# mazouziwissem/improving_yolov8_CBAM_SwinBlock

Measured on AMD Instinct MI355X. Metric: images/sec fwd+bwd YOLOv8s-CBAM-Swin bs=32 640x640, higher is better.
Workload: dtype bf16; 1 GPU; yolov8s.yaml (nc=1) forward + v8 loss + backward + clip + SGD-nesterov + EMA step, bs=32/GPU 640x640 (CBAM + 2x SwinBlock + SPPF5 + SPPF7); global_batch=32, imgsz=640, parallelism=dp1

## Files before the change

### improving_yolov8_cbam_swinblock_amd/_lib.py

```python
import ctypes
import os
import subprocess
import threading
from pathlib import Path

import torch

PKG_DIR = Path(__file__).resolve().parent
CSRC_DIR = PKG_DIR / "csrc"
LIB_PATH = Path(os.environ["YMI_LIB"]).resolve() if os.environ.get("YMI_LIB") else PKG_DIR / "libyolo_mi355.so"

YMI_F32, YMI_BF16 = 0, 1
ACT_NONE, ACT_SILU, ACT_GELU = 0, 1, 2

_c_i64 = ctypes.c_int64
_c_i32 = ctypes.c_int32
_c_f32 = ctypes.c_float
_vp = ctypes.c_void_p
_sz = ctypes.c_size_t


class YmiTensor(ctypes.Structure):
    _fields_ = [
        ("data", _vp),
        ("n", _c_i64),
        ("h", _c_i64),
        ("w", _c_i64),
        ("c", _c_i64),
        ("ld", _c_i64),
        ("dtype", _c_i32),
        ("_pad", _c_i32),
    ]


_TP = ctypes.POINTER(YmiTensor)

_SIGNATURES = {
    "ymi_version": (_c_i32, []),
    "ymi_last_error": (ctypes.c_char_p, []),
    "ymi_set_option": (_c_i32, [ctypes.c_char_p, _c_i64]),
    "ymi_get_option": (_c_i64, [ctypes.c_char_p]),
    "ymi_profile_begin": (_c_i32, [_c_i64]),
    "ymi_profile_end": (_c_i32, [ctypes.POINTER(ctypes.c_double), ctypes.POINTER(ctypes.c_double), ctypes.POINTER(_c_i64)]),
    "ymi_profile_end_ex": (_c_i32, [ctypes.POINTER(ctypes.c_double), ctypes.POINTER(ctypes.c_double), ctypes.POINTER(_c_i64),
                                    ctypes.POINTER(ctypes.c_double), ctypes.POINTER(ctypes.c_double)]),
    "ymi_nchw_to_nhwc": (_c_i32, [_vp, _c_i64, _c_i64, _c_i64, _c_i64, _TP, _vp]),
    "ymi_nhwc_to_nchw": (_c_i32, [_TP, _vp, _vp]),
    "ymi_copy": (_c_i32, [_TP, _TP, _vp]),
    "ymi_upsample2x": (_c_i32, [_TP, _TP, _vp]),
    "ymi_upsample2x_bwd": (_c_i32, [_TP, _TP, _vp]),
    "ymi_upsample2x_bwd_acc": (_c_i32, [_TP, _TP, _vp]),
    "ymi_add_inplace": (_c_i32, [_TP, _TP, _vp]),
    "ymi_pack_conv_weight_fwd": (_c_i32, [_vp, _c_i64, _c_i64, _c_i64, _c_i64, _c_i64, _c_i32, _vp, _vp]),
    "ymi_pack_conv_weight_dgrad": (_c_i32, [_vp, _c_i64, _c_i64, _c_i64, _c_i64, _c_i64, _c_i32, _vp, _vp]),
    "ymi_pack_conv_weight_dgrad_ex": (_c_i32, [_vp, _c_i64, _c_i64, _c_i64, _c_i64, _c_i64, _c_i64, _c_i32, _vp, _vp]),
    "ymi_conv_dgrad_pack_elems": (_c_i64, [_c_i64, _c_i64, _c_i64, _c_i64, _c_i64]),
    "ymi_pack_conv_weights_batch": (_c_i32, [_vp, _vp, _c_i32, _c_i32, _c_i32, _vp]),
    "ymi_pack_matrix": (_c_i32, [_vp, _c_i64, _c_i64, _c_i32, _c_i32, _vp, _vp]),
    "ymi_conv2d_fwd": (_c_i32, [_TP, _vp, _c_i64, _c_i64, _c_i64, _c_i64, _vp, _vp, _c_i32, _TP, _TP, _vp, ctypes.POINTER(_c_i64), _vp]),
    "ymi_conv2d_stat_blocks": (_c_i64, [_c_i64, _c_i64]),
    "ymi_conv2d_fwd_multi": (_c_i32, [_vp, _c_i32, _vp]),
    "ymi_conv2d_bwd_data_multi": (_c_i32, [_vp, _c_i32, _vp]),
    "ymi_bn_finalize_pair": (_c_i32, [_vp, _c_i64, _c_i64, _c_i64, _c_i64, _vp, _vp, _vp, _vp, _vp, _vp, _vp, _vp, _c_f32, _c_f32, _vp, _vp, _vp, _vp, _vp]),
    "ymi_bn_finalize": (_c_i32, [_vp, _c_i64, _c_i64, _c_i64, _vp, _vp, _vp, _vp, _c_f32, _c_f32, _vp, _vp, _vp, _vp, _vp]),
    "ymi_scale_shift_act": (_c_i32, [_TP, _vp, _vp, _c_i32, _TP, _TP, _vp]),
    "ymi_conv2d_bn_silu_fwd": (
        _c_i32,
        [_TP, _vp, _c_i64, _c_i64, _c_i64, _c_i64, _vp, _vp, _vp, _vp, _c_f32, _c_f32, _c_i32, _TP, _TP, _TP, _vp, _vp, _vp, _sz, _vp],
    ),
    "ymi_conv2d_bn_silu_fwd_acc_ok": (_c_i32, [_TP, _TP, _TP]),
    "ymi_conv2d_bn_silu_fwd_acc": (_c_i32, [_TP, _vp, _c_i64, _c_i64, _c_i64, _c_i64, _vp, _vp, _vp, _vp, _c_f32, _c_f32, _c_i32, _TP, _TP, _TP, _vp, _vp, _vp, _vp]),
    "ymi_bn_act_bwd": (_c_i32, [_TP, _TP, _vp, _vp, _vp, _vp, _c_i32, _TP, _vp, _vp, _vp, _sz, _vp]),
    "ymi_conv2d_bn_silu_fwd_pair": (
        _c_i32,
        [_TP, _vp, _c_i64, _c_i64, _c_i64, _c_i64, _c_i64, _vp, _vp, _vp, _vp, _vp, _vp, _vp, _vp, _c_f32, _c_f32, _c_i32, _TP, _TP, _vp, _vp, _vp, _sz, _vp],
    ),
    "ymi_first_conv_stat_blocks": (_c_i64, [_c_i64, _c_i64, _c_i64]),
    "ymi_first_conv_bn_act_fwd": (_c_i32, [_vp, _c_i64, _c_i64, _c_i64, _c_i64, _vp, _c_i64, _vp, _vp, _vp, _vp, _c_f32, _c_f32, _c_i32, _TP, _TP, _vp, _vp,
                                           _vp, _sz, _vp]),
    "ymi_first_conv_bwd_workspace": (_c_i64, [_c_i64, _c_i64, _c_i64, _c_i64]),
    "ymi_first_conv_bn_act_bwd": (_c_i32, [_TP, _vp, _c_i64, _c_i64, _vp, _vp, _vp, _vp, _c_i32, _TP, _vp, _vp, _vp, _vp, _sz, _vp, _vp]),
    "ymi_bn_act_bwd_pair": (_c_i32, [_TP, _TP, _vp, _vp, _vp, _vp, _c_i64, _vp, _vp, _c_i32, _TP, _vp, _vp, _vp, _sz, _vp]),
    "ymi_conv2d_bwd_data": (_c_i32, [_TP, _vp, _c_i64, _c_i64, _c_i64, _c_i64, _TP, _vp]),
    "ymi_conv2d_bwd_data_add": (_c_i32, [_TP, _vp, _c_i64, _c_i64, _c_i64, _c_i64, _TP, _TP, _TP, _vp]),
    "ymi_dwconv2d_fwd": (_c_i32, [_TP, _vp, _c_i64, _c_i64, _vp, _vp, _c_i32, _TP, _TP, _vp, ctypes.POINTER(_c_i64), _vp]),
    "ymi_dwconv2d_stat_blocks": (_c_i64, [_c_i64, _c_i64, _c_i64, _c_i64]),
    "ymi_dwconv2d_bn_act_fwd": (_c_i32, [_TP, _vp, _c_i64, _c_i64, _vp, _vp, _vp, _vp, _c_f32, _c_f32, _c_i32, _TP, _TP, _TP, _vp, _vp, _vp, _sz, _vp]),
    "ymi_dwconv2d_bwd_data": (_c_i32, [_TP, _vp, _c_i64, _c_i64, _TP, _TP, _vp]),
    "ymi_dwconv2d_bwd_weight": (_c_i32, [_TP, _TP, _c_i64, _c_i64, _vp, _vp, _sz, _vp]),
    "ymi_dwconv2d_bwd_weight_workspace": (_sz, [_c_i64, _c_i64, _c_i64, _c_i64, _c_i64]),
    "ymi_swin_mlp_fwd": (_c_i32, [_TP, _vp, _vp, _c_i64, _vp, _vp, _TP, _TP, _TP, _TP, _vp]),
    "ymi_swin_ln_mlp_supported": (_c_i32, [_c_i64, _c_i64, _c_i32]),
    "ymi_swin_ln_mlp_pack_elems": (_c_i64, [_c_i64, _c_i64]),
    "ymi_swin_ln_mlp_pre_elems": (_c_i64, [_c_i64, _c_i64]),
    "ymi_swin_ln_mlp_pack": (_c_i32, [_vp, _vp, _c_i64, _c_i64, _vp, _vp]),
    "ymi_swin_ln_mlp_fwd": (_c_i32, [_TP, _vp, _vp, _c_f32, _vp, _vp, _vp, _c_i64, _TP, _vp, _vp, _vp, _TP, _vp]),
    "ymi_swin_ln_mlp_bwd_data": (_c_i32, [_TP, _vp, _vp, _c_i64, _TP, _TP, _TP, _vp]),
    "ymi_swin_mlp_bwd_data": (_c_i32, [_TP, _vp, _TP, _TP, _vp, _TP, _TP, _TP, _vp]),
    "ymi_conv2d_bwd_weight": (_c_i32, [_TP, _TP, _c_i64, _c_i64, _c_i64, _c_i64, _c_i64, _vp, _vp, _vp, _sz, _vp]),
    "ymi_conv2d_bwd_weight_workspace": (_sz, [_c_i64, _c_i64, _c_i64, _c_i64, _c_i64]),
    "ymi_conv2d_bwd_weight_deferred": (_c_i32, [_TP, _TP, _c_i64, _c_i64, _c_i64, _c_i64, _c_i64, _vp, _vp, _vp, _sz, _vp, _vp]),
    "ymi_wgrad_hold": (_c_i32, [_c_i32]),
    "ymi_wgrad_reduce_batch": (_c_i32, [_vp, _c_i32, _vp, _vp]),
    "ymi_sppf_pool3_fwd": (_c_i32, [_TP, _c_i64, _TP, _TP, _TP, _vp]),
    "ymi_sppf_pool3_bwd_workspace": (_c_i64, [_c_i64, _c_i64, _c_i64, _c_i64, _c_i32]),
    "ymi_sppf_pool3_bwd": (_c_i32, [_TP, _TP, _TP, _c_i64, _TP, _TP, _TP, _TP, _TP, _vp, _c_i64, _vp]),
    "ymi_cbam_fwd": (_c_i32, [_TP, _vp, _vp, _c_i64, _vp, _c_i64, _TP, _vp, _vp, _vp, _vp, _vp, _vp, _vp]),
    "ymi_cbam_bwd": (_c_i32, [_TP, _TP, _vp, _vp, _c_i64, _vp, _c_i64, _vp, _vp, _vp, _vp, _vp, _vp, _TP, _vp, _vp, _vp, _vp, _sz, _vp]),
    "ymi_cbam_bwd_workspace": (_sz, [_c_i64, _c_i64, _c_i64, _c_i64, _c_i64]),
    "ymi_window_partition_index": (_c_i32, [_c_i64, _c_i64, _c_i64, _c_i64, _vp, _vp]),
    "ymi_window_partition": (_c_i32, [_TP, _c_i64, _TP, _vp]),
    "ymi_window_reverse": (_c_i32, [_TP, _c_i64, _TP, _vp]),
    "ymi_layernorm_fwd": (_c_i32, [_TP, _c_i64, _vp, _vp, _c_f32, _TP, _vp, _vp, _vp]),
    "ymi_layernorm_bwd": (_c_i32, [_TP, _c_i64, _TP, _vp, _vp, _vp, _TP, _c_i32, _vp, _vp, _vp, _sz, _vp]),
    "ymi_layernorm_bwd_add": (_c_i32, [_TP, _c_i64, _TP, _vp, _vp, _vp, _TP, _TP, _vp, _vp, _vp, _sz, _vp]),
    "ymi_window_attention_fwd": (_c_i32, [_TP, _c_i64, _c_i64, _TP, _vp, _vp]),
    "ymi_window_attention_bwd": (_c_i32, [_TP, _TP, _TP, _vp, _c_i64, _c_i64, _TP, _vp]),
    "ymi_psa_attention_fwd": (_c_i32, [_TP, _c_i64, _c_i64, _c_i64, _TP, _TP, _vp, _vp]),
    "ymi_psa_attention_bwd": (_c_i32, [_TP, _TP, _TP, _vp, _TP, _c_i64, _c_i64, _c_i64, _TP, _vp]),
    "ymi_colsum":(_c_i32, [_TP, _vp, _vp, _sz, _vp]),
    "ymi_gelu_bwd": (_c_i32, [_TP, _TP, _TP, _vp]),
    "ymi_detect_targets": (_c_i32, [_vp, _vp, _vp, _c_i64, _c_i64, _c_i64, ctypes.c_float, ctypes.c_float, _vp, _vp]),
    "ymi_detect_loss_sizes": (_c_i32, [_c_i64, _c_i64, _c_i64, ctypes.POINTER(ctypes.c_size_t), ctypes.POINTER(ctypes.c_size_t)]),
    "ymi_detect_loss_fwd": (_c_i32, [_c_i32, _TP, _TP, ctypes.POINTER(ctypes.c_float), _vp, _c_i64, _c_i32, ctypes.c_float, ctypes.c_float,
                                     _vp, _vp, _vp, _sz, _vp, _sz, _vp]),
    "ymi_detect_loss_bwd": (_c_i32, [_c_i32, _TP, _TP, ctypes.POINTER(ctypes.c_float), _vp, _sz, _vp, _vp, _TP, _TP, _vp]),
    "ymi_detect_decode": (_c_i32, [_c_i32, _TP, _TP, ctypes.POINTER(ctypes.c_float), _vp, _vp]),
    "ymi_depth_to_space2": (_c_i32, [_TP, _TP, _vp]),
    "ymi_space_to_depth2": (_c_i32, [_TP, _TP, _vp]),
    "ymi_detect_loss_fwd_assign": (_c_i32, [_c_i32, _TP, _TP, ctypes.POINTER(ctypes.c_float), _vp, _c_i64, _c_i32, ctypes.c_float, ctypes.c_float,
                                            _vp, _vp, _vp, _sz, _vp, _sz, _vp, _vp]),
    "ymi_detect_decode_seg": (_c_i32, [_c_i32, _TP, _TP, _TP, ctypes.POINTER(ctypes.c_float), _vp, _vp]),
    "ymi_mask_loss_sizes": (_c_i32, [_c_i64, _c_i64, _c_i64, _c_i32, ctypes.POINTER(ctypes.c_size_t)]),
    "ymi_mask_loss_fwd": (_c_i32, [_c_i32, _TP, _TP, _vp, _c_i32, _c_i64, _c_i64, _vp, _vp, _c_i64, _c_i32, _c_f32, _c_f32, _vp, _vp, _vp, _vp, _sz, _vp]),
    "ymi_mask_loss_bwd": (_c_i32, [_c_i32, _TP, _TP, _vp, _c_i32, _c_i64, _c_i64, _c_i64, _c_i32, _vp, _sz, _vp, _vp, _TP, _TP, _vp]),
    "ymi_detect_nms_sizes": (_c_i32, [_c_i64, _c_i64, _c_i64, _c_i64, _c_i64, ctypes.POINTER(ctypes.c_size_t)]),
    "ymi_detect_nms": (_c_i32, [_vp, _c_i64, _c_i64, _c_i64, _c_f32, _c_f32, _c_i32, _c_i32, ctypes.POINTER(_c_i32), _c_i32, _c_i64, _c_i64, _c_f32,
                                _vp, _vp, _vp, _sz, _vp]),
    "ymi_detect_nms_seg": (_c_i32, [_vp, _c_i64, _c_i64, _c_i64, _c_i64, _c_f32, _c_f32, _c_i32, _c_i32, ctypes.POINTER(_c_i32), _c_i32, _c_i64, _c_i64,
                                    _c_f32, _vp, _vp, _vp, _vp, _sz, _vp]),
    "ymi_process_mask": (_c_i32, [_TP, _vp, _vp, _vp, _c_i64, _c_i64, _c_i64, _c_i32, _vp, _vp, _vp]),
    "ymi_mask_overlap": (_c_i32, [_vp, _vp, _vp, _c_i64, _c_i64, _TP, _c_i64, _c_i64, _vp, _c_i32, _c_i64, _c_i64, _c_i64, _vp, _vp, _vp, _vp]),
    "ymi_scale_image": (_c_i32, [_vp, _c_i32, _c_i64, _c_i64, _c_i64, _vp, _c_i64, _c_i64, _c_i64, _c_i64, _c_f32, _c_i32, _c_i32, _c_i32, _vp]),
    "ymi_tta_merge": (_c_i32, [_c_i32, ctypes.POINTER(_vp), ctypes.POINTER(_c_i64), ctypes.POINTER(_c_i64), ctypes.POINTER(_c_i64), ctypes.POINTER(_c_f32),
                               ctypes.POINTER(_c_i32), ctypes.POINTER(_c_i64), ctypes.POINTER(_c_i64), _c_i64, _c_i64, _vp, _vp]),
    "ymi_letterbox_batch": (_c_i32, [_vp, _c_i64, _vp, _c_i64, _c_i64, _c_i32, _c_i32, _c_i32, _vp]),
    "ymi_scale_boxes": (_c_i32, [_vp, _c_i64, _vp, _vp, _c_i64, _c_i64, _c_i64, _c_i32, _c_i32, _vp, _c_i64, _vp]),
    "ymi_augment_batch": (_c_i32, [_vp, _vp, _c_i64, _vp, _c_i64, _c_i32, _c_i32, _c_i32, _vp]),
    "ymi_augment_boxes": (_c_i32, [_vp, _c_i64, _vp, _c_i64, _c_f32, _vp, _vp, _vp, _vp, _vp, _vp, _vp]),
    "ymi_val_match": (_c_i32, [_vp, _vp, _c_i64, _c_i64, _vp, _vp, _vp, _c_i64, _c_f32, _c_f32, _vp, ctypes.POINTER(_c_f32), _c_i32, _c_i32, _vp, _vp, _c_i64,
                              _c_f32, _c_f32, _vp]),
    "ymi_val_match_masks": (_c_i32, [_vp, _vp, _c_i64, _c_i64, _vp, _vp, _c_i64, _vp, _vp, _vp, _c_i64, ctypes.POINTER(_c_f32), _c_i32, _c_i32, _vp, _vp]),
    "ymi_opt_chunk_elems": (_c_i64, []),
    "ymi_opt_grad_norm": (_c_i32, [_vp, _vp, _c_i32, _c_i32, _c_i64, ctypes.POINTER(_vp), _vp, _vp, _c_i64, _c_i64, _vp, _c_i32, _vp]),
    "ymi_opt_update": (_c_i32, [_vp, _vp, _c_i32, _c_i32, _c_i64, ctypes.POINTER(_vp), _vp, _vp, _c_i32, _vp]),
    "ymi_opt_grad_accumulate": (_c_i32, [_vp, _vp, _c_i32, _c_i32, _c_i64, ctypes.POINTER(_vp), _vp]),
}

OPT_MAX_GRADS = 448


class LetterboxImage(ctypes.Structure):
    _fields_ = [("src", _vp), ("h", _c_i32), ("w", _c_i32), ("hs", _c_i32), ("ws", _c_i32), ("top", _c_i32), ("left", _c_i32)]


AUGMENT_MAX_SRC = 4
VALMATCH_CHUNK, VALMATCH_MAX_LEVELS, VALMATCH_MAX_DET = 1024, 16, 2048


class AugmentSource(ctypes.Structure):
    _fields_ = [("src", _vp), ("h", _c_i32), ("w", _c_i32), ("x1a", _c_i32), ("y1a", _c_i32), ("x2a", _c_i32), ("y2a", _c_i32), ("x1b", _c_i32),
                ("y1b", _c_i32)]


class AugmentImage(ctypes.Structure):
    _fields_ = [("s", AugmentSource * AUGMENT_MAX_SRC), ("A", ctypes.c_double * 6), ("lut", _vp), ("n_src", _c_i32), ("canvas_h", _c_i32),
                ("canvas_w", _c_i32), ("flip_ud", _c_i32), ("flip_lr", _c_i32), ("_pad", _c_i32)]


class AugmentLabelImage(ctypes.Structure):
    _fields_ = [("src_w", _c_f32 * AUGMENT_MAX_SRC), ("src_h", _c_f32 * AUGMENT_MAX_SRC), ("ratio_w", _c_f32 * AUGMENT_MAX_SRC),
                ("ratio_h", _c_f32 * AUGMENT_MAX_SRC), ("padw", _c_f32 * AUGMENT_MAX_SRC), ("padh", _c_f32 * AUGMENT_MAX_SRC), ("M", _c_f32 * 6),
                ("scale", _c_f32), ("size_w", _c_f32), ("size_h", _c_f32), ("canvas", _c_f32), ("flip_ud", _c_i32), ("flip_lr", _c_i32),
                ("row_start", _c_i32), ("row_end", _c_i32)]


class ConvProblem(ctypes.Structure):
    _fields_ = [("x", _TP), ("w_packed", _vp), ("cout", _c_i64), ("kh", _c_i64), ("kw", _c_i64), ("stride", _c_i64), ("scale", _vp), ("bias", _vp),
                ("act", _c_i32), ("_pad", _c_i32), ("residual", _TP), ("y", _TP), ("stat_partials", _vp), ("stat_blocks", _c_i64), ("stat_stride", _c_i64),
                ("stat_offset", _c_i64)]


class DgradProblem(ctypes.Structure):
    _fields_ = [("dy", _TP), ("w_dgrad_packed", _vp), ("cin", _c_i64), ("k", _c_i64), ("add1", _TP), ("add2", _TP), ("dx", _TP)]


class WgradPending(ctypes.Structure):
    _fields_ = [("slab", _vp), ("dw", _vp), ("elems", _c_i64), ("splits", _c_i32), ("ng", _c_i32), ("cin", _c_i32), ("cout_real", _c_i32),
                ("cin_real", _c_i32), ("ntaps", _c_i32), ("lanes", _c_i32), ("first_block", _c_i32), ("blocks", _c_i32), ("slab_bf16", _c_i32),
                ("bias_slab", _vp), ("dbias", _vp)]


class OptEntry(ctypes.Structure):
    _fields_ = [("param", _vp), ("momentum", _vp), ("ema", _vp), ("numel", _c_i64), ("group", _c_i32), ("_pad", _c_i32), ("second", _vp), ("acc", _vp)]


class OptState(ctypes.Structure):
    _fields_ = [("clip", _c_f32), ("norm", _c_f32), ("ema_d", _c_f32), ("ema_1md", _c_f32), ("updates", _c_i64), ("steps", _c_i64), ("inv_bc1", _c_f32),
                ("bc2_sqrt", _c_f32), ("c0", _c_f32), ("c1", _c_f32), ("c2", _c_f32), ("c3", _c_f32), ("mu_product", ctypes.c_double)]


assert ctypes.sizeof(OptState) == 64

_lib = None
_lock = threading.Lock()


def build(verbose=False):
    jobs = str(min(8, os.cpu_count() or 1))
    proc = subprocess.run(["make", "-C", str(CSRC_DIR), "-j", jobs], capture_output=True, text=True)
    if proc.returncode != 0:
        raise RuntimeError(f"building libyolo_mi355.so failed:\n{proc.stdout[-4000:]}\n{proc.stderr[-4000:]}")
    if verbose:
        print(proc.stdout[-2000:])
    return LIB_PATH


def lib():
    global _lib
    if _lib is None:
        with _lock:
            if _lib is None:
                if not LIB_PATH.exists():
                    raise RuntimeError(
                        f"{LIB_PATH} is missing: build it with improving_yolov8_cbam_swinblock_amd._lib.build() "
                        "(make -C csrc); this package has no CPU or PyTorch fallback"
                    )
                handle = ctypes.CDLL(str(LIB_PATH))
                missing = []
                for name, (res, args) in _SIGNATURES.items():
                    try:
                        fn = getattr(handle, name)
                    except AttributeError:
                        missing.append(name)
                        continue
                    fn.restype = res
                    fn.argtypes = args
                if missing:
                    raise RuntimeError(f"{LIB_PATH} is stale, missing symbols {missing}: rebuild with make -C csrc")
                _lib = handle
    return _lib


def exported_symbols():
    return list(_SIGNATURES)


def check(rc, what=""):
    if rc != 0:
        msg = lib().ymi_last_error().decode("utf-8", "replace")
        raise RuntimeError(f"libyolo_mi355 {what} failed ({rc}): {msg}")


def ymi_dtype(dt):
    if dt == torch.float32:
        return YMI_F32
    if dt == torch.bfloat16:
        return YMI_BF16
    raise TypeError(f"libyolo_mi355 computes in float32 or bfloat16, got {dt}")


def chunk_elems(dt):
    return 8 if dt == torch.bfloat16 else 4


def is_nhwc(t):
    if t.dim() != 4:
        return False
    n, c, h, w = t.shape
    sn, sc, sh, sw = t.stride()
    if c > 1 and sc != 1:
        return False
    ld = sw if w > 1 else (sh if h > 1 else (sn if n > 1 else c))
    if w > 1 and h > 1 and sh != w * ld:
        return False
    if (h > 1 or w > 1) and n > 1 and sn != h * w * ld:
        return False
    return ld >= c


def as_ymi(t):
    if not t.is_cuda:
        raise RuntimeError("libyolo_mi355 kernels need tensors on the MI355X (cuda) device; there is no CPU path")
    if t.dim() == 4:
        if not is_nhwc(t):
            raise RuntimeError(f"expected NHWC memory for a logical NCHW tensor, got shape {tuple(t.shape)} strides {t.stride()}")
        n, c, h, w = t.shape
        sn, sc, sh, sw = t.stride()
        ld = sw if w > 1 else (sh if h > 1 else (sn if n > 1 else c))
        return YmiTensor(t.data_ptr(), n, h, w, c, ld, ymi_dtype(t.dtype), 0)
    if t.dim() == 2:
        rows, c = t.shape
        if c > 1 and t.stride(1) != 1:
            raise RuntimeError("token matrix must have unit channel stride")
        ld = t.stride(0) if rows > 1 else c
        return YmiTensor(t.data_ptr(), 1, 1, rows, c, ld, ymi_dtype(t.dtype), 0)
    raise RuntimeError(f"unsupported tensor rank {t.dim()}")


def stream_ptr():
    return ctypes.c_void_p(torch.cuda.current_stream().cuda_stream)


def ptr(t):
    return ctypes.c_void_p(t.data_ptr()) if t is not None else None


def empty_nhwc(n, c, h, w, dtype, device, ld=None):
    ld = c if ld is None else ld
    buf = torch.empty((n, h, w, ld), dtype=dtype, device=device)
    return buf.permute(0, 3, 1, 2)[:, :c]


_workspaces = {}


def workspace(nbytes, device, tag="default"):
    if os.environ.get("YMI_WS_NOCACHE") == "1":
        return torch.empty(max(int(nbytes), 256), dtype=torch.uint8, device=device)
    key = (device.index, torch.cuda.current_stream().cuda_stream, tag)
    buf = _workspaces.get(key)
    if buf is None or buf.numel() < nbytes:
        buf = torch.empty(max(int(nbytes), 1 << 20), dtype=torch.uint8, device=device)
        _workspaces[key] = buf
    return buf


def live_workspaces(device):
    return tuple(buf for (idx, _, _), buf in _workspaces.items() if idx == device.index)


def set_option(name, value):
    check(lib().ymi_set_option(name.encode(), int(value)), "set_option")


def get_option(name):
    v = lib().ymi_get_option(name.encode())
    if v < 0:
        raise RuntimeError(f"unknown option {name!r}")
    return int(v)
```

### improving_yolov8_cbam_swinblock_amd/csrc/common.h

```cpp
#pragma once
#include <hip/hip_runtime.h>
#include <stdint.h>
#include <stdio.h>

#include <type_traits>

#include "../../include/ymi.h"

typedef __bf16 bf16_t;
typedef __attribute__((ext_vector_type(8))) __bf16 bf16x8;
typedef __attribute__((ext_vector_type(4))) __bf16 bf16x4;
typedef __attribute__((ext_vector_type(4))) float f32x4;
typedef __attribute__((ext_vector_type(2))) float f32x2;
typedef __attribute__((ext_vector_type(4))) uint32_t u32x4;
typedef __attribute__((ext_vector_type(2))) uint32_t u32x2;

typedef const __attribute__((address_space(1))) void* gptr_t;
typedef __attribute__((address_space(3))) void* lptr_t;

#define YMI_WAVE 64

void ymi_set_error(const char* fmt, ...);
#define YMI_CHECK_ARG(cond, ...)          \
    do {                                  \
// ... 4 lines not shown
    } while (0)
#define YMI_CHECK_LAUNCH(what)                                                   \
    do {                                                                         \
        hipError_t e_ = hipGetLastError();                                       \
        if (e_ != hipSuccess) {                                                  \
            ymi_set_error("%s: launch failed: %s", what, hipGetErrorString(e_)); \
            return YMI_ELAUNCH;                                                  \
        }                                                                        \
    } while (0)

static inline bool ymi_tensor_ok(const ymi_tensor* t) {
    return t && t->data && t->n > 0 && t->h > 0 && t->w > 0 && t->c > 0 && t->ld >= t->c && (t->dtype == YMI_F32 || t->dtype == YMI_BF16);
}
static inline int64_t ymi_pixels(const ymi_tensor* t) { return t->n * t->h * t->w; }
static inline int ymi_stat_fixed_point_shift(int64_t count) {
    int lg = 0;
    while (((int64_t)1 << lg) < count) ++lg;
    const int sh = 37 - lg;
    return sh < 8 ? 8 : sh > 40 ? 40 : sh;
}
constexpr int BN_STAGE_ROWS = 64;
static inline size_t ymi_esize(int dtype) { return dtype == YMI_BF16 ? 2 : 4; }
static inline bool vec4_ok(const ymi_tensor* t) {
    return t->c % 4 == 0 && t->ld % 4 == 0 && ((uintptr_t)t->data % (4 * ymi_esize(t->dtype))) == 0;
}
static inline bool ymi_same_shape(const ymi_tensor* a, const ymi_tensor* b) {
    return a->n == b->n && a->h == b->h && a->w == b->w && a->c == b->c;
}
enum YmiOpt {
    OPT_EW_PPT,
    OPT_EW_CAP,
    OPT_RED_CAP,
    OPT_XCD_SHIFT,
    OPT_ATTN_TILED,
    OPT_WGRAD_BLOCKS,
    OPT_WGRAD_BLOCKS128,
    OPT_IGEMM_TILE_BM,
    OPT_IGEMM_TILE_BN,
    OPT_BN_TAIL,
    OPT_WGRAD_PATCH,
    OPT_COUNT
};
int ymi_opt(int id);
static inline int ew_ppt() { return ymi_opt(OPT_EW_PPT); }
static inline int ew_cap() { return ymi_opt(OPT_EW_CAP); }
static inline int64_t ew_capped(int64_t gb) {
    if (gb > ew_cap()) gb = ew_cap();
    return (gb + 7) / 8 * 8;
}
static inline int64_t ew_blocks(int64_t P, int rows) {
    int64_t gb = (P + (int64_t)rows * ew_ppt() - 1) / ((int64_t)rows * ew_ppt());
    if (gb < 1024) gb = (P + rows - 1) / rows < 1024 ? (P + rows - 1) / rows : 1024;
    return ew_capped(gb);
}
template <typename T> struct TypeTag {
    typedef T type;
};
template <int ACT> using ActTag = std::integral_constant<int, ACT>;
template <typename F> static inline void dispatch_dtype(int dtype, F&& f) {
    if (dtype == YMI_BF16) f(TypeTag<bf16_t>{});
    else f(TypeTag<float>{});
}
template <typename F> static inline void dispatch_dtype_act(int dtype, int act, F&& f) {
    dispatch_dtype(dtype, [&](auto t) {
        if (act == YMI_ACT_SILU) f(t, ActTag<YMI_ACT_SILU>{});
        else if (act == YMI_ACT_GELU) f(t, ActTag<YMI_ACT_GELU>{});
        else f(t, ActTag<YMI_ACT_NONE>{});
    });
}
const void* ymi_zero_page();

template <typename T> struct ElemTraits;
template <> struct ElemTraits<float> {
    static constexpr int CH = 4;
    static constexpr int DT = YMI_F32;
};
template <> struct ElemTraits<bf16_t> {
    static constexpr int CH = 8;
    static constexpr int DT = YMI_BF16;
};

__device__ __forceinline__ float to_f32(float v) { return v; }
__device__ __forceinline__ float to_f32(bf16_t v) { return (float)v; }
template <typename T> __device__ __forceinline__ T from_f32(float v);
template <> __device__ __forceinline__ float from_f32<float>(float v) { return v; }
template <> __device__ __forceinline__ bf16_t from_f32<bf16_t>(float v) { return (bf16_t)v; }

template <typename T, int G> struct Pack;
template <> struct Pack<float, 4> {
    static __device__ __forceinline__ void load(const float* p, float (&v)[4]) {
        f32x4 t = *reinterpret_cast<const f32x4*>(p);
        v[0] = t[0]; v[1] = t[1]; v[2] = t[2]; v[3] = t[3];
    }
    static __device__ __forceinline__ void store(float* p, const float (&v)[4]) {
        f32x4 t = {v[0], v[1], v[2], v[3]};
        *reinterpret_cast<f32x4*>(p) = t;
    }
};
template <> struct Pack<bf16_t, 4> {
    static __device__ __forceinline__ void load(const bf16_t* p, float (&v)[4]) {
        bf16x4 t = *reinterpret_cast<const bf16x4*>(p);
        v[0] = (float)t[0]; v[1] = (float)t[1]; v[2] = (float)t[2]; v[3] = (float)t[3];
    }
    static __device__ __forceinline__ void store(bf16_t* p, const float (&v)[4]) {
        bf16x4 t = {(bf16_t)v[0], (bf16_t)v[1], (bf16_t)v[2], (bf16_t)v[3]};
        *reinterpret_cast<bf16x4*>(p) = t;
    }
};
template <> struct Pack<bf16_t, 8> {
    static __device__ __forceinline__ void load(const bf16_t* p, float (&v)[8]) {
        bf16x8 t = *reinterpret_cast<const bf16x8*>(p);
#pragma unroll
        for (int i = 0; i < 8; ++i) v[i] = (float)t[i];
    }
    static __device__ __forceinline__ void store(bf16_t* p, const float (&v)[8]) {
        bf16x8 t;
#pragma unroll
        for (int i = 0; i < 8; ++i) t[i] = (bf16_t)v[i];
        *reinterpret_cast<bf16x8*>(p) = t;
    }
};

template <typename T> struct Raw4;
template <> struct Raw4<bf16_t> {
    typedef bf16x4 type;
    static __device__ __forceinline__ void to_f32(const bf16x4& r, float (&v)[4]) {
#pragma unroll
        for (int i = 0; i < 4; ++i) v[i] = (float)r[i];
    }
};
template <> struct Raw4<float> {
    typedef f32x4 type;
    static __device__ __forceinline__ void to_f32(const f32x4& r, float (&v)[4]) {
#pragma unroll
        for (int i = 0; i < 4; ++i) v[i] = r[i];
    }
};

__host__ __device__ __forceinline__ int64_t ymi_xcd_span(int64_t P) { return (((P + 63) >> 6) + 7) >> 3 << 6; }
struct XcdRange {
    int64_t lo, hi;
    int bi, nbx;
};
int64_t ymi_xcd_span_arg(int64_t P);
__device__ __forceinline__ XcdRange xcd_range(int64_t P, int64_t span_arg) {
    const int id = blockIdx.x, x = ((id & 7) + (int)(span_arg >> 56)) & 7;
    const int64_t span = span_arg & ((1ll << 56) - 1);
    XcdRange r;
    r.lo = x * span;
    r.hi = r.lo + span < P ? r.lo + span : P;
    if (r.lo > P) r.lo = P;
    r.bi = id >> 3;
    r.nbx = gridDim.x >> 3;
    return r;
}

__device__ __forceinline__ int xcd_unit(int flat, int total) { return (total & 7) ? flat : (flat & 7) * (total >> 3) + (flat >> 3); }
__device__ __forceinline__ int flat_block_id() { return blockIdx.x + gridDim.x * (blockIdx.y + gridDim.y * blockIdx.z); }

template <int U, typename T, typename F>
__device__ __forceinline__ void pixel_walk(const T* ap, int64_t lda, const T* bp, int64_t ldb, bool two, int coff, int64_t p, int64_t step, int64_t end, F&& use) {
    typedef typename Raw4<T>::type R4;
    R4 ra[U], rb[U];
    bool have = p + (U - 1) * step < end;
    if (have) {
#pragma unroll
        for (int u = 0; u < U; ++u) {
            ra[u] = *reinterpret_cast<const R4*>(ap + (p + u * step) * lda + coff);
            if (two) rb[u] = *reinterpret_cast<const R4*>(bp + (p + u * step) * ldb + coff);
        }
    }
    while (have) {
        float va[U][4], vb[U][4] = {};
#pragma unroll
        for (int u = 0; u < U; ++u) {
            Raw4<T>::to_f32(ra[u], va[u]);
            if (two) Raw4<T>::to_f32(rb[u], vb[u]);
        }
        const int64_t pc = p;
        p += U * step;
        have = p + (U - 1) * step < end;
        if (have) {
#pragma unroll
            for (int u = 0; u < U; ++u) {
                ra[u] = *reinterpret_cast<const R4*>(ap + (p + u * step) * lda + coff);
                if (two) rb[u] = *reinterpret_cast<const R4*>(bp + (p + u * step) * ldb + coff);
            }
        }
#pragma unroll
        for (int u = 0; u < U; ++u) use(va[u], vb[u], pc + u * step);
    }
    for (; p < end; p += step) {
        float va[4], vb[4] = {0.f, 0.f, 0.f, 0.f};
        Pack<T, 4>::load(ap + p * lda + coff, va);
        if (two) Pack<T, 4>::load(bp + p * ldb + coff, vb);
        use(va, vb, p);
    }
}

__device__ __forceinline__ float fast_exp(float x) { return __builtin_amdgcn_exp2f(x * 1.44269504088896340736f); }
__device__ __forceinline__ float sigmoidf_(float x) { return __builtin_amdgcn_rcpf(1.0f + fast_exp(-x)); }
__device__ __forceinline__ float silu_f(float x) { return x * sigmoidf_(x); }
__device__ __forceinline__ float silu_grad_f(float x) {
    float s = sigmoidf_(x);
    return s * (1.0f + x * (1.0f - s));
}
__device__ __forceinline__ float erf_as(float z, float* e2 = nullptr) {
    const float az = fabsf(z);
    const float t = __builtin_amdgcn_rcpf(1.0f + 0.3275911f * az);
    const float e = fast_exp(-az * az);
    float p = 1.061405429f;
    p = p * t - 1.453152027f;
    p = p * t + 1.421413741f;
    p = p * t - 0.284496736f;
    p = p * t + 0.254829592f;
    if (e2) *e2 = e;
    return copysignf(1.0f - p * t * e, z);
}
__device__ __forceinline__ float gelu_f(float x) { return 0.5f * x * (1.0f + erf_as(x * 0.70710678118654752440f)); }
__device__ __forceinline__ float gelu_grad_f(float x) {
    const float c = 0.39894228040143267794f;
    float e;
    const float er = erf_as(x * 0.70710678118654752440f, &e);
    return 0.5f * (1.0f + er) + x * c * e;
}
template <int ACT> __device__ __forceinline__ float apply_act(float x) {
    if (ACT == YMI_ACT_SILU) return silu_f(x);
    if (ACT == YMI_ACT_GELU) return gelu_f(x);
    return x;
}
__device__ __forceinline__ float apply_act_rt(float x, int act) {
    return act == YMI_ACT_SILU ? silu_f(x) : act == YMI_ACT_GELU ? gelu_f(x) : x;
}
template <int ACT> __device__ __forceinline__ float act_grad(float x) {
    if (ACT == YMI_ACT_SILU) return silu_grad_f(x);
    if (ACT == YMI_ACT_GELU) return gelu_grad_f(x);
    return 1.0f;
}
__device__ __forceinline__ float act_grad_rt(float x, int act) {
    return act == YMI_ACT_SILU ? silu_grad_f(x) : act == YMI_ACT_GELU ? gelu_grad_f(x) : 1.0f;
}

__device__ __forceinline__ float unit_of_byte(uint32_t u) {
    const float f = (float)u, rc = 1.0f / 255.0f;
    const float q = f * rc;
    const float r = __builtin_fmaf(-q, 255.0f, f);
    return __builtin_fmaf(r, rc, q);
}

struct Tap {
    int i0, i1;
    float l0, l1;
};
__device__ __forceinline__ Tap tap_of(int dst, float scale, int in) {
    float s = ((float)dst + 0.5f) * scale - 0.5f;
    s = s < 0.0f ? 0.0f : s;
    Tap t;
    t.i0 = (int)s;
    t.i0 = t.i0 > in - 1 ? in - 1 : t.i0;
    t.i1 = t.i0 + (t.i0 < in - 1 ? 1 : 0);
    t.l1 = s - (float)t.i0;
    t.l0 = 1.0f - t.l1;
    return t;
}

__device__ __forceinline__ void st_wt(float* p, float v) { __hip_atomic_store(p, v, __ATOMIC_RELAXED, __HIP_MEMORY_SCOPE_AGENT); }
__device__ __forceinline__ void st_wt2(float* p, float a, float b) {
    const uint64_t v = (uint64_t)__builtin_bit_cast(uint32_t, a) | ((uint64_t)__builtin_bit_cast(uint32_t, b) << 32);
    __hip_atomic_store(reinterpret_cast<uint64_t*>(p), v, __ATOMIC_RELAXED, __HIP_MEMORY_SCOPE_AGENT);
}
__device__ __forceinline__ void st_wt(double* p, double v) { __hip_atomic_store(p, v, __ATOMIC_RELAXED, __HIP_MEMORY_SCOPE_AGENT); }
__device__ __forceinline__ float ld_wt(const float* p) { return __hip_atomic_load(p, __ATOMIC_RELAXED, __HIP_MEMORY_SCOPE_AGENT); }
__device__ __forceinline__ double ld_wt(const double* p) { return __hip_atomic_load(p, __ATOMIC_RELAXED, __HIP_MEMORY_SCOPE_AGENT); }
__device__ __forceinline__ void ld_wt2(const float* p, float& a, float& b) {
    const uint64_t v = __hip_atomic_load(reinterpret_cast<const uint64_t*>(p), __ATOMIC_RELAXED, __HIP_MEMORY_SCOPE_AGENT);
    a = __builtin_bit_cast(float, (uint32_t)v);
    b = __builtin_bit_cast(float, (uint32_t)(v >> 32));
}
__device__ __forceinline__ bool ticket_is_last(unsigned* counter, unsigned last, int* flag) {
    asm volatile("s_waitcnt vmcnt(0)" ::: "memory");
    __syncthreads();
    if (threadIdx.x == 0) {
        const unsigned t = __hip_atomic_fetch_add(counter, 1u, __ATOMIC_RELAXED, __HIP_MEMORY_SCOPE_AGENT);
        if (t == last) __hip_atomic_store(counter, 0u, __ATOMIC_RELAXED, __HIP_MEMORY_SCOPE_AGENT);
        *flag = t == last;
    }
    __syncthreads();
    return *flag != 0;
}
struct GammaBeta2 {
    const float* gamma;
    const float* beta;
    int split;
};
struct BnCoefArgs {
    const float* gamma;
    const float* beta;
    const float* mean;
    const float* inv;
    float inv_count;
    float* coef;
    GammaBeta2 g2;
};
struct BnFinal {
    const float* part;
    int blocks, C;
    float* out0;
    float* out1;
    BnCoefArgs bn;
};
__device__ __forceinline__ void bn_affine_of(const float* gamma, const float* beta, const GammaBeta2& g2, int c, float& ga, float& be) {
    const bool second = g2.split > 0 && c >= g2.split;
    const float* gp = second ? g2.gamma : gamma;
    const float* bp = second ? g2.beta : beta;
    const int pc = second ? c - g2.split : c;
    ga = gp ? gp[pc] : 1.0f;
    be = bp ? bp[pc] : 0.0f;
}
struct BnChan {
    float ga, be, inv, mean;
};
__device__ __forceinline__ void bn_chan_fetch(const BnCoefArgs& bn, int c, BnChan& p) {
    bn_affine_of(bn.gamma, bn.beta, bn.g2, c, p.ga, p.be);
    p.inv = bn.inv[c];
    p.mean = bn.mean[c];
}
__device__ __forceinline__ void bn_coef_write(const BnCoefArgs& bn, int C, int c, const BnChan& p, float s0, float s1) {
    const float ga = p.ga, be = p.be;
    const float p0 = p.inv, p1 = -p.mean * p0;
    const float k1 = s0 * bn.inv_count, k2 = s1 * bn.inv_count;
    bn.coef[0 * C + c] = p0 * ga;
    bn.coef[1 * C + c] = p1 * ga + be;
    bn.coef[2 * C + c] = ga * p0;
    bn.coef[3 * C + c] = ga * p0 * p0 * k2;
    bn.coef[4 * C + c] = ga * p0 * (k1 + p1 * k2);
}
struct BnStat {
    double mean, var;
    float inv;
};
__device__ __forceinline__ BnStat bn_stat_of(double sum, double sumsq, double count, float eps) {
    BnStat s;
    s.mean = sum / count;
    s.var = sumsq / count - s.mean * s.mean;
    if (s.var < 0.0) s.var = 0.0;
    s.inv = (float)(1.0 / sqrt(s.var + (double)eps));
    return s;
}
constexpr int BN_FINAL_RED = 2 * 32 * 33;
template <int NT, bool PREFETCH = true> __device__ __forceinline__ void bn_final_block(const BnFinal& f, int w, double* red) {
    static_assert(NT == 1024 || NT == 256, "32 channels x 32 or 8 thread rows");
    constexpr int SPT = 1024 / NT;
    const int cl = threadIdx.x & 31, grp = threadIdx.x >> 5;
    const int c = w * 32 + cl, C = f.C;
    BnChan p{1.0f, 0.0f, 0.f, 0.f};
    if (PREFETCH && grp == 0 && c < C && f.bn.coef) bn_chan_fetch(f.bn, c, p);
    int es = 0;
#pragma unroll
    do {
        const int slice = grp * SPT + es;
        double s0 = 0.0, s1 = 0.0;
        if (c < C) {
            float a0 = 0.f, a1 = 0.f, b0 = 0.f, b1 = 0.f, c0 = 0.f, c1 = 0.f, d0 = 0.f, d1 = 0.f;
            int b = slice;
            for (; b + 96 < f.blocks; b += 128) {
                a0 += f.part[((int64_t)b * 2 + 0) * C + c];
                a1 += f.part[((int64_t)b * 2 + 1) * C + c];
                b0 += f.part[((int64_t)(b + 32) * 2 + 0) * C + c];
                b1 += f.part[((int64_t)(b + 32) * 2 + 1) * C + c];
                c0 += f.part[((int64_t)(b + 64) * 2 + 0) * C + c];
                c1 += f.part[((int64_t)(b + 64) * 2 + 1) * C + c];
                d0 += f.part[((int64_t)(b + 96) * 2 + 0) * C + c];
                d1 += f.part[((int64_t)(b + 96) * 2 + 1) * C + c];
            }
            for (; b < f.blocks; b += 32) {
                a0 += f.part[((int64_t)b * 2 + 0) * C + c];
                a1 += f.part[((int64_t)b * 2 + 1) * C + c];
            }
            s0 = ((double)a0 + (double)b0) + ((double)c0 + (double)d0);
            s1 = ((double)a1 + (double)b1) + ((double)c1 + (double)d1);
        }
        red[(0 * 32 + slice) * 33 + cl] = s0;
        red[(1 * 32 + slice) * 33 + cl] = s1;
    } while (++es < SPT);
    __syncthreads();
    if (grp == 0 && c < C) {
        double a0 = 0.0, a1 = 0.0;
#pragma unroll
        for (int q = 0; q < 32; ++q) {
            a0 += red[(0 * 32 + q) * 33 + cl];
            a1 += red[(1 * 32 + q) * 33 + cl];
        }
        if (f.out0) f.out0[c] = (float)a0;
        if (f.out1) f.out1[c] = (float)a1;
        if (f.bn.coef) {
            if (!PREFETCH) bn_chan_fetch(f.bn, c, p);
            bn_coef_write(f.bn, C, c, p, (float)a0, (float)a1);
        }
    }
}
struct BnRider {
    BnFinal f;
    int nwg;
};
bool ymi_wgrad_issue_held(const BnFinal* f, hipStream_t stream);

bool ymi_prof_enabled();
int ymi_prof_start(hipStream_t stream, int family, double flop, double bytes, double peak_tflops);
void ymi_prof_stop(hipStream_t stream, int idx);
struct IgemmArgs;
int ymi_launch_igemm(const IgemmArgs& a, int dtype, bool stats, int* host_blocks, hipStream_t stream);
int ymi_conv2d_fwd_statacc(const ymi_tensor* x, const void* w_packed, int64_t cout, int64_t kh, int64_t kw, int64_t stride, const ymi_tensor* y,
                           long long* stat_acc, void* stream);

int ymi_chan_reduce_final(const float* part, int blocks, int C, float* out0, float* out1, hipStream_t stream);
int ymi_bn_bwd_final(const float* part, int blocks, int C, const float* gamma, const float* beta, const float* mean, const float* inv, float inv_count,
                     float* dgamma, float* dbeta, float* coef, hipStream_t stream);

ymi_wgrad_pending ymi_wgrad_record(const void* slab, float* dw, int64_t elems, int splits, int ng, int cin, int cout_real, int cin_real, int ntaps,
                                   bool slab_bf16, const float* bias_slab, float* dbias);

unsigned* ymi_ticket_slot();

template <int N> __device__ __forceinline__ void wait_vmcnt_barrier() {
    asm volatile("s_waitcnt vmcnt(%0)\n\ts_barrier" ::"n"(N) : "memory");
}

constexpr int tr_swz_mode(int row_bytes) { return row_bytes >= 256 ? 1 : row_bytes == 64 ? 2 : 0; }
template <int SW> __device__ __forceinline__ int tr_swz(int row) {
    return SW == 1 ? ((row & 3) | (((row >> 3) & 1) << 2)) : SW == 2 ? ((row >> 3) & 1) : (((row >> 1) & 1) | (((row >> 3) & 1) << 1));
}
struct TrFragAddr {
    lptr_t lo, hi;
};
template <int SW> __device__ __forceinline__ TrFragAddr tr_frag_addr(const char* img, int rowb, int c0, int lane) {
    const int g = lane >> 4, i = lane & 15, q = i >> 2, p = i & 3;
    const int r_lo = 8 * g + q, r_hi = r_lo + 4;
    const int u = (c0 >> 2) + p;
    const int u_lo = u ^ (tr_swz<SW>(r_lo) << 2), u_hi = u ^ (tr_swz<SW>(r_hi) << 2);
    return TrFragAddr{(lptr_t)(img + r_lo * rowb + u_lo * 8), (lptr_t)(img + r_hi * rowb + u_hi * 8)};
}

template <int CTRL> __device__ __forceinline__ float dpp_add(float v) {
    return v + __builtin_bit_cast(float, __builtin_amdgcn_update_dpp(0, __builtin_bit_cast(int, v), CTRL, 0xF, 0xF, true));
}
__device__ __forceinline__ float row16_sum(float v) {
    v = dpp_add<0xB1>(v);
    v = dpp_add<0x4E>(v);
    v = dpp_add<0x141>(v);
    v = dpp_add<0x140>(v);
    return v;
}
__device__ __forceinline__ uint32_t pack_bf16x2(float a, float b) {
    typedef __attribute__((ext_vector_type(2))) __bf16 bf16x2;
    const bf16x2 v = {(bf16_t)a, (bf16_t)b};
    return __builtin_bit_cast(uint32_t, v);
}

__device__ __forceinline__ float wave_sum(float v) {
#pragma unroll
    for (int o = 32; o > 0; o >>= 1) v += __shfl_xor(v, o, 64);
    return v;
}
__device__ __forceinline__ float wave_max(float v) {
#pragma unroll
    for (int o = 32; o > 0; o >>= 1) v = fmaxf(v, __shfl_xor(v, o, 64));
    return v;
}
```

### improving_yolov8_cbam_swinblock_amd/csrc/reduce_bwd.hip

```cpp
#include <stdlib.h>

#include "common.h"

struct RV {
    const void* p;
    int64_t ld;
};

struct ReduceTail {
    unsigned* tickets;
    int ncls;
    double* xrows;
    float* out0;
    float* out1;
    BnCoefArgs bn;
};
constexpr int RED_U = 4;
constexpr int APPLY_U = 4;
template <typename T, int FN, int ACT>
__global__ void chan_reduce_kernel(RV a, RV b, int64_t P, int64_t span, int C, int TG, const float* __restrict__ gamma, const float* __restrict__ beta,
                                   const float* __restrict__ mean, const float* __restrict__ inv, float* __restrict__ part, GammaBeta2 g2, ReduceTail tail) {
    extern __shared__ float red[];
    const int rows = 256 / TG;
    const int tx = threadIdx.x % TG, ty = threadIdx.x / TG;
    const int c0 = blockIdx.y * 1024;
    const int groups = ((C - c0 < 1024) ? C - c0 : 1024) / 4;
    const XcdRange xr = xcd_range(P, span);
    const int64_t per = (xr.hi - xr.lo + xr.nbx - 1) / xr.nbx;
    const int64_t p0 = (xr.lo + xr.bi * per < xr.hi) ? xr.lo + xr.bi * per : xr.hi, p1 = (p0 + per < xr.hi) ? p0 + per : xr.hi;
    const T* ap = reinterpret_cast<const T*>(a.p) + c0;
    const T* bp = reinterpret_cast<const T*>(b.p) + c0;
    float s0[4] = {0.f, 0.f, 0.f, 0.f}, s1[4] = {0.f, 0.f, 0.f, 0.f};
    if (tx < groups) {
        float g[4], be[4], mu[4], iv[4];
#pragma unroll
        for (int r = 0; r < 4; ++r) {
            const int c = c0 + tx * 4 + r;
            g[r] = 1.0f;
            be[r] = 0.0f;
            if (FN == 1) bn_affine_of(gamma, beta, g2, c, g[r], be[r]);
            mu[r] = (FN == 1) ? mean[c] : 0.0f;
            iv[r] = (FN == 1) ? inv[c] : 1.0f;
        }
        auto accum = [&](const float (&va)[4], const float (&vb)[4], int64_t p) {
            if (FN == 0) {
#pragma unroll
                for (int r = 0; r < 4; ++r) s0[r] += va[r];
            } else if (FN == 1) {
#pragma unroll
                for (int r = 0; r < 4; ++r) {
                    const float xh = (vb[r] - mu[r]) * iv[r];
                    const float dz = va[r] * act_grad<ACT>(xh * g[r] + be[r]);
                    s0[r] += dz;
                    s1[r] += dz * xh;
                }
            } else {
                const float m = mean[p], rs = inv[p];
#pragma unroll
                for (int r = 0; r < 4; ++r) {
                    s0[r] += va[r];
                    s1[r] += va[r] * (vb[r] - m) * rs;
                }
            }
        };
        pixel_walk<RED_U>(ap, a.ld, bp, b.ld, FN != 0, tx * 4, p0 + ty, (int64_t)rows, p1, accum);
    }
    float* my = red + ((size_t)ty * TG + tx) * 8;
#pragma unroll
    for (int r = 0; r < 4; ++r) {
        my[r] = s0[r];
        my[4 + r] = s1[r];
    }
    __syncthreads();
    if (ty == 0 && tx < groups) {
        for (int q = 1; q < rows; ++q) {
            const float* o = red + ((size_t)q * TG + tx) * 8;
#pragma unroll
            for (int r = 0; r < 4; ++r) {
                s0[r] += o[r];
                s1[r] += o[4 + r];
            }
        }
        float* r0 = part + ((int64_t)blockIdx.x * 2 + 0) * C + c0 + tx * 4;
        float* r1 = part + ((int64_t)blockIdx.x * 2 + 1) * C + c0 + tx * 4;
        if (tail.tickets) {
            st_wt2(r0, s0[0], s0[1]);
            st_wt2(r0 + 2, s0[2], s0[3]);
            st_wt2(r1, s1[0], s1[1]);
            st_wt2(r1 + 2, s1[2], s1[3]);
        } else {
#pragma unroll
            for (int r = 0; r < 4; ++r) {
                r0[r] = s0[r];
                r1[r] = s1[r];
            }
        }
    }
    if (tail.tickets == nullptr) return;
    int* flag = reinterpret_cast<int*>(red);
    const int NC = tail.ncls;
    const int xg = blockIdx.x % NC, nbx = gridDim.x / NC;
    if (!ticket_is_last(&tail.tickets[xg], (unsigned)nbx - 1u, flag)) return;
    for (int col = threadIdx.x * 2; col < 2 * C; col += 512) {
        const float* src = part + (int64_t)xg * 2 * C + col;
        const int64_t rs = (int64_t)NC * 2 * C;
        double a0 = 0.0, a1 = 0.0;
        int j = 0;
        for (; j + 15 < nbx; j += 16) {
            float x[16], y[16];
#pragma unroll
            for (int u = 0; u < 16; ++u) ld_wt2(src + (int64_t)(j + u) * rs, x[u], y[u]);
#pragma unroll
            for (int u = 0; u < 16; ++u) {
                a0 += (double)x[u];
                a1 += (double)y[u];
            }
        }
        for (; j < nbx; ++j) {
            float x, y;
            ld_wt2(src + (int64_t)j * rs, x, y);
            a0 += (double)x;
            a1 += (double)y;
        }
        st_wt(&tail.xrows[(int64_t)xg * 2 * C + col], a0);
        st_wt(&tail.xrows[(int64_t)xg * 2 * C + col + 1], a1);
    }
    if (!ticket_is_last(&tail.tickets[32], (unsigned)NC - 1u, flag)) return;
    for (int c = threadIdx.x; c < C; c += 256) {
        double sa = 0.0, sb = 0.0;
        for (int x0 = 0; x0 < NC; x0 += 8) {
            double v0[8], v1[8];
#pragma unroll
            for (int x = 0; x < 8; ++x) {
                v0[x] = ld_wt(&tail.xrows[((int64_t)(x0 + x) * 2 + 0) * C + c]);
                v1[x] = ld_wt(&tail.xrows[((int64_t)(x0 + x) * 2 + 1) * C + c]);
            }
#pragma unroll
            for (int x = 0; x < 8; ++x) {
                sa += v0[x];
                sb += v1[x];
            }
        }
        if (tail.out0) tail.out0[c] = (float)sa;
        if (tail.out1) tail.out1[c] = (float)sb;
        if (tail.bn.coef) {
            BnChan p;
            bn_chan_fetch(tail.bn, c, p);
            bn_coef_write(tail.bn, C, c, p, (float)sa, (float)sb);
        }
    }
}

__global__ __launch_bounds__(1024) void chan_reduce_final_kernel(BnFinal f) {
    __shared__ double red[BN_FINAL_RED];
    bn_final_block<1024>(f, (int)blockIdx.x, red);
}
static int launch_final(const BnFinal& f, hipStream_t stream, const char* what) {
    hipLaunchKernelGGL(chan_reduce_final_kernel, dim3((f.C + 31) / 32), dim3(1024), 0, stream, f);
    YMI_CHECK_LAUNCH(what);
    return YMI_OK;
}

static bool bn_tail_on() { return ymi_opt(OPT_BN_TAIL) != 0; }

static int pow2_ge(int v) {
    int p = 1;
    while (p < v) p <<= 1;
    return p;
}

static int reduce_blocks(int64_t P, int C) {
    const int tg = pow2_ge(C / 4) > 256 ? 256 : pow2_ge(C / 4);
    int64_t ppb = (int64_t)(256 / tg) * 4;
    if (ppb < 16) ppb = 16;
    if (ppb > 64) ppb = 64;
    int64_t b = (P + ppb - 1) / ppb;
    const int rcap = ymi_opt(OPT_RED_CAP);
    if (b > rcap) b = rcap;
    if (b < 1) b = 1;
    return (int)((b + 7) / 8 * 8);
}

template <int FN>
static int launch_chan_reduce(const ymi_tensor* a, const ymi_tensor* b, const float* gamma, const float* beta, const float* mean,
                              const float* inv, int act, float* part, int* blocks_out, hipStream_t stream, const char* what,
                              GammaBeta2 g2 = GammaBeta2{nullptr, nullptr, 0}, ReduceTail tail = ReduceTail{}) {
    const int64_t P = ymi_pixels(a);
    const int C = (int)a->c;
    YMI_CHECK_ARG(C % 4 == 0 && a->ld % 4 == 0 && (!b || (b->ld % 4 == 0)), "%s: channels must be a multiple of 4", what);
    const int TG = pow2_ge(C / 4) > 256 ? 256 : pow2_ge(C / 4);
    const int crows = (C + 1023) / 1024;
    const int blocks = reduce_blocks(P, C);
    YMI_CHECK_ARG(!tail.tickets || crows == 1, "%s: the in-kernel final pass covers at most 1024 channels", what);
    const size_t lds = (size_t)256 * 8 * sizeof(float);
    RV ra{a->data, a->ld}, rb{b ? b->data : nullptr, b ? b->ld : 0};
    dispatch_dtype_act(a->dtype, act, [&](auto t, auto ac) {
        typedef typename decltype(t)::type T;
        constexpr int ACT = FN == 1 ? decltype(ac)::value : YMI_ACT_NONE;
        hipLaunchKernelGGL((chan_reduce_kernel<T, FN, ACT>), dim3(blocks, crows), dim3(256), lds, stream, ra, rb, P, ymi_xcd_span_arg(P), C, TG, gamma, beta, mean,
                           inv, part, g2, tail);
    });
    YMI_CHECK_LAUNCH(what);
    *blocks_out = blocks;
    return YMI_OK;
}

int ymi_chan_reduce_final(const float* part, int blocks, int C, float* out0, float* out1, hipStream_t stream) {
    return launch_final(BnFinal{part, blocks, C, out0, out1, BnCoefArgs{}}, stream, "chan_reduce_final");
}

int ymi_bn_bwd_final(const float* part, int blocks, int C, const float* gamma, const float* beta, const float* mean, const float* inv, float inv_count,
                     float* dgamma, float* dbeta, float* coef, hipStream_t stream) {
    return launch_final(BnFinal{part, blocks, C, dbeta, dgamma, BnCoefArgs{gamma, beta, mean, inv, inv_count, coef, GammaBeta2{nullptr, nullptr, 0}}}, stream,
                        "bn_bwd_final");
}

extern "C" int ymi_colsum(const ymi_tensor* x, float* out, void* workspace, size_t workspace_bytes, void* stream) {
    YMI_CHECK_ARG(ymi_tensor_ok(x) && out && workspace, "colsum: args");
    const size_t need = (size_t)reduce_blocks(ymi_pixels(x), (int)x->c) * 2 * x->c * sizeof(float);
    if (workspace_bytes < need) {
        ymi_set_error("colsum: workspace %zu < %zu", workspace_bytes, need);
        return YMI_EWORKSPACE;
    }
    int blocks = 0;
    int rc = launch_chan_reduce<0>(x, nullptr, nullptr, nullptr, nullptr, nullptr, 0, (float*)workspace, &blocks, (hipStream_t)stream, "colsum");
    if (rc) return rc;
    return ymi_chan_reduce_final((const float*)workspace, blocks, (int)x->c, out, nullptr, (hipStream_t)stream);
}

int ymi_ln_param_grads(const ymi_tensor* dy, const ymi_tensor* x, const float* mean, const float* rstd, float* dgamma, float* dbeta,
                       void* workspace, size_t workspace_bytes, hipStream_t stream) {
    const size_t need = (size_t)reduce_blocks(ymi_pixels(dy), (int)dy->c) * 2 * dy->c * sizeof(float);
    if (workspace_bytes < need) {
        ymi_set_error("layernorm_bwd: workspace %zu < %zu", workspace_bytes, need);
        return YMI_EWORKSPACE;
    }
    int blocks = 0;
    int rc = launch_chan_reduce<2>(dy, x, nullptr, nullptr, mean, rstd, 0, (float*)workspace, &blocks, stream, "layernorm_bwd(param)");
    if (rc) return rc;
    return ymi_chan_reduce_final((const float*)workspace, blocks, (int)dy->c, dbeta, dgamma, stream);
}

template <typename T, bool FIXED, int ACT>
__global__ __launch_bounds__(256) void bn_act_bwd_apply_kernel(RV dout, RV raw, RV draw, int64_t Pall, int64_t span, int C, const float* __restrict__ coef) {
    constexpr int G = 4;
    const int groups = C / G;
    const T* dp = reinterpret_cast<const T*>(dout.p);
    const T* rp = reinterpret_cast<const T*>(raw.p);
    T* op = reinterpret_cast<T*>(const_cast<void*>(draw.p));
    if constexpr (FIXED) {
        const int g = threadIdx.x % groups, rows = 256 / groups;
        if ((int)threadIdx.x >= rows * groups) return;
        float a0[G], a1[G], c0[G], c1[G], c2[G];
#pragma unroll
        for (int r = 0; r < G; ++r) {
            const int c = g * G + r;
            a0[r] = coef[c];
            a1[r] = coef[C + c];
            c0[r] = coef[2 * C + c];
            c1[r] = coef[3 * C + c];
            c2[r] = coef[4 * C + c];
        }
        auto one = [&](const float (&d)[G], const float (&x)[G], int64_t p) {
            float o[G];
#pragma unroll
            for (int r = 0; r < G; ++r) {
                const float dz = d[r] * act_grad<ACT>(x[r] * a0[r] + a1[r]);
                o[r] = dz * c0[r] - (x[r] * c1[r] + c2[r]);
            }
            Pack<T, G>::store(op + p * draw.ld + g * G, o);
        };
        const XcdRange xr = xcd_range(Pall, span);
        const int64_t step = (int64_t)xr.nbx * rows;
        pixel_walk<APPLY_U>(dp, dout.ld, rp, raw.ld, true, g * G, xr.lo + (int64_t)xr.bi * rows + threadIdx.x / groups, step, xr.hi, one);
    } else {
        const uint32_t total = (uint32_t)(Pall * groups), ugroups = (uint32_t)groups;
        for (uint32_t i = blockIdx.x * blockDim.x + threadIdx.x; i < total; i += gridDim.x * blockDim.x) {
            const uint32_t pu = i / ugroups;
            const int g = (int)(i - pu * ugroups);
            const int64_t p = pu;
            float d[G], x[G], o[G];
            Pack<T, G>::load(dp + p * dout.ld + g * G, d);
            Pack<T, G>::load(rp + p * raw.ld + g * G, x);
#pragma unroll
            for (int r = 0; r < G; ++r) {
                const int c = g * G + r;
                const float dz = d[r] * act_grad<ACT>(x[r] * coef[c] + coef[C + c]);
                o[r] = dz * coef[2 * C + c] - (x[r] * coef[3 * C + c] + coef[4 * C + c]);
            }
            Pack<T, G>::store(op + p * draw.ld + g * G, o);
        }
    }
}

static int launch_bn_apply(const ymi_tensor* dout, const ymi_tensor* raw, const ymi_tensor* draw, int act, const float* coef, hipStream_t s) {
    const int64_t P = ymi_pixels(dout);
    const int C = (int)dout->c;
    const int groups = C / 4;
    const bool fixed = groups <= 256;
    const int64_t total = P * groups;
    YMI_CHECK_ARG(total < (1ll << 31), "bn_act_bwd: tensor too large for 32-bit indexing");
    const dim3 gb((unsigned)(fixed ? ew_blocks(P, 256 / groups) : ew_capped((total + 255) / 256)));
    const int64_t span = ymi_xcd_span_arg(P);
    RV a{dout->data, dout->ld}, b{raw->data, raw->ld}, o{draw->data, draw->ld};
    dispatch_dtype_act(dout->dtype, act, [&](auto t, auto ac) {
        typedef typename decltype(t)::type T;
        constexpr int ACT = decltype(ac)::value;
        if (fixed) hipLaunchKernelGGL((bn_act_bwd_apply_kernel<T, true, ACT>), gb, dim3(256), 0, s, a, b, o, P, span, C, coef);
        else hipLaunchKernelGGL((bn_act_bwd_apply_kernel<T, false, ACT>), gb, dim3(256), 0, s, a, b, o, P, span, C, coef);
    });
    YMI_CHECK_LAUNCH("bn_act_bwd(apply)");
    return YMI_OK;
}

static int bn_act_bwd_impl(const ymi_tensor* dout, const ymi_tensor* raw, const float* gamma, const float* save_mean,
                           const float* save_invstd, const float* beta, GammaBeta2 g2, int32_t act, const ymi_tensor* draw, float* dgamma,
                           float* dbeta, void* workspace, size_t workspace_bytes, void* stream);
extern "C" int ymi_bn_act_bwd(const ymi_tensor* dout, const ymi_tensor* raw, const float* gamma, const float* save_mean,
                              const float* save_invstd, const float* beta, int32_t act, const ymi_tensor* draw, float* dgamma,
                              float* dbeta, void* workspace, size_t workspace_bytes, void* stream) {
    return bn_act_bwd_impl(dout, raw, gamma, save_mean, save_invstd, beta, GammaBeta2{nullptr, nullptr, 0}, act, draw, dgamma, dbeta, workspace, workspace_bytes, stream);
}
extern "C" int ymi_bn_act_bwd_pair(const ymi_tensor* dout, const ymi_tensor* raw, const float* gamma, const float* beta, const float* gamma2,
                                   const float* beta2, int64_t split, const float* save_mean, const float* save_invstd, int32_t act,
                                   const ymi_tensor* draw, float* dgamma, float* dbeta, void* workspace, size_t workspace_bytes, void* stream) {
    YMI_CHECK_ARG(dout && split > 0 && split < dout->c && split % 4 == 0 && gamma2 && beta2, "bn_act_bwd_pair: split");
    return bn_act_bwd_impl(dout, raw, gamma, save_mean, save_invstd, beta, GammaBeta2{gamma2, beta2, (int)split}, act, draw, dgamma, dbeta, workspace, workspace_bytes, stream);
}
static int bn_act_bwd_impl(const ymi_tensor* dout, const ymi_tensor* raw, const float* gamma, const float* save_mean,
                           const float* save_invstd, const float* beta, GammaBeta2 g2, int32_t act, const ymi_tensor* draw, float* dgamma,
                           float* dbeta, void* workspace, size_t workspace_bytes, void* stream) {
    YMI_CHECK_ARG(ymi_tensor_ok(dout) && ymi_tensor_ok(raw) && ymi_tensor_ok(draw) && ymi_same_shape(dout, raw) && ymi_same_shape(dout, draw),
                  "bn_act_bwd: shapes");
    YMI_CHECK_ARG(dout->dtype == raw->dtype && raw->dtype == draw->dtype, "bn_act_bwd: dtypes");
    YMI_CHECK_ARG(save_mean && save_invstd && dgamma && dbeta && workspace, "bn_act_bwd: null argument");
    YMI_CHECK_ARG(draw->ld % 4 == 0, "bn_act_bwd: draw ld");
    const int64_t P = ymi_pixels(dout);
    const int C = (int)dout->c;
    const int rblocks = reduce_blocks(P, C);
    const size_t need = ((size_t)rblocks * 2 * C + 6 * (size_t)C) * sizeof(float) + 64 * (size_t)C * sizeof(double);
    if (workspace_bytes < need) {
        ymi_set_error("bn_act_bwd: workspace %zu < %zu", workspace_bytes, need);
        return YMI_EWORKSPACE;
    }
    hipStream_t s = (hipStream_t)stream;
    int blocks = 0;
    float* coef = (float*)workspace + (size_t)rblocks * 2 * C;
    double* xrows = reinterpret_cast<double*>(coef + 6 * (size_t)C);
    const BnCoefArgs bn{gamma, beta, save_mean, save_invstd, 1.0f / (float)P, coef, g2};
    if (bn_tail_on() && C <= 1024) {
        unsigned* tickets = ymi_ticket_slot();
        YMI_CHECK_ARG(tickets, "bn_act_bwd: ticket counters");
        int rc = launch_chan_reduce<1>(dout, raw, gamma, beta, save_mean, save_invstd, act, (float*)workspace, &blocks, s, "bn_act_bwd(reduce)", g2,
                                       ReduceTail{tickets, rblocks % 32 == 0 ? 32 : 8, xrows, dbeta, dgamma, bn});
        if (rc) return rc;
        return launch_bn_apply(dout, raw, draw, act, coef, s);
    }
    int rc = launch_chan_reduce<1>(dout, raw, gamma, beta, save_mean, save_invstd, act, (float*)workspace, &blocks, s, "bn_act_bwd(reduce)", g2);
    if (rc) return rc;
    const BnFinal f{(const float*)workspace, blocks, C, dbeta, dgamma, bn};
    if (C <= 1024 && ymi_wgrad_issue_held(&f, s)) YMI_CHECK_LAUNCH("bn_act_bwd(final, riding)");
    else if ((rc = launch_final(f, s, "bn_act_bwd(final)")) != YMI_OK) return rc;
    return launch_bn_apply(dout, raw, draw, act, coef, s);
}

template <typename T>
__global__ void gelu_bwd_kernel(RV pre, RV dy, RV dx, int64_t P, int C) {
    const int groups = C / 4;
    const uint32_t total = (uint32_t)(P * groups), ugroups = (uint32_t)groups;
    const T* pp = reinterpret_cast<const T*>(pre.p);
    const T* dp = reinterpret_cast<const T*>(dy.p);
    T* op = reinterpret_cast<T*>(const_cast<void*>(dx.p));
    for (uint32_t i = blockIdx.x * blockDim.x + threadIdx.x; i < total; i += gridDim.x * blockDim.x) {
        const uint32_t pu = i / ugroups;
        const int g = (int)(i - pu * ugroups);
        const int64_t p = pu;
        float a[4], d[4];
        Pack<T, 4>::load(pp + p * pre.ld + g * 4, a);
        Pack<T, 4>::load(dp + p * dy.ld + g * 4, d);
#pragma unroll
        for (int r = 0; r < 4; ++r) d[r] *= gelu_grad_f(a[r]);
        Pack<T, 4>::store(op + p * dx.ld + g * 4, d);
    }
}

extern "C" int ymi_gelu_bwd(const ymi_tensor* pre, const ymi_tensor* dy, const ymi_tensor* dx, void* stream) {
    YMI_CHECK_ARG(ymi_tensor_ok(pre) && ymi_tensor_ok(dy) && ymi_tensor_ok(dx) && ymi_same_shape(pre, dy) && ymi_same_shape(pre, dx), "gelu_bwd: shapes");
    YMI_CHECK_ARG(pre->dtype == dy->dtype && dy->dtype == dx->dtype && pre->c % 4 == 0 && pre->ld % 4 == 0 && dy->ld % 4 == 0 && dx->ld % 4 == 0, "gelu_bwd: dtype/alignment");
    const int64_t P = ymi_pixels(pre), total = P * (pre->c / 4);
    YMI_CHECK_ARG(total < (1ll << 31), "gelu_bwd: tensor too large for 32-bit indexing");
    int64_t gb = (total + 255) / 256;
    if (gb > 4096) gb = 4096;
    RV a{pre->data, pre->ld}, b{dy->data, dy->ld}, o{dx->data, dx->ld};
    dispatch_dtype(pre->dtype, [&](auto t) {
        hipLaunchKernelGGL(gelu_bwd_kernel<typename decltype(t)::type>, dim3((unsigned)gb), dim3(256), 0, (hipStream_t)stream, a, b, o, P, (int)pre->c);
    });
    YMI_CHECK_LAUNCH("gelu_bwd");
    return YMI_OK;
}
```

### improving_yolov8_cbam_swinblock_amd/csrc/wgrad.hip

```cpp
#include <stdlib.h>

#include <mutex>
#include <type_traits>

#include "common.h"

struct WgradArgs {
    const void* x;
    const void* dy;
    void* slab;
    int slab_bf16;
    float* bias_slab;
    const void* zero;
    int64_t ldx, ldy;
    int Mpix, H, W, Ho, Wo;
    int stride, pad, KW;
    int CoutP, Cin, NG;
    int pix_per_split;
    int nx, ny, splits, xcd_map;
    int pw_shift;
    uint32_t x_bytes, y_bytes;
    uint32_t wo_mul, wo_shr, ho_mul, ho_shr;
};

// ... 4 lines not shown
constexpr int WG_NS = 2;
constexpr int WG_WAVES = 5;

template <typename T, int BM> constexpr size_t wgrad_lds_bytes() { return (size_t)WG_NS * WG_BK * (BM + WG_BN) * sizeof(T); }

__device__ __forceinline__ void wg_buffer_to_lds(const void* base, uint32_t bytes, lptr_t dst, uint32_t voff, uint32_t soff) {
#if defined(__HIP_DEVICE_COMPILE__)
    __builtin_amdgcn_raw_ptr_buffer_load_lds(__builtin_amdgcn_make_buffer_rsrc(const_cast<void*>(base), 0, bytes, 0x00020000), dst, 16, voff, soff, 0, 0);
#endif
}
__device__ __forceinline__ void wg_global_to_lds(const void* src, lptr_t dst) {
#if defined(__HIP_DEVICE_COMPILE__)
    __builtin_amdgcn_global_load_lds((gptr_t)src, dst, 16, 0, 0);
#endif
}
template <typename T> struct WFrag;

template <> struct WFrag<bf16_t> {
    static __device__ __forceinline__ void read2(bf16x8& f, const TrFragAddr& ad) {
        typedef __attribute__((ext_vector_type(2))) uint32_t u2;
        u2 lo, hi;
        asm volatile("ds_read_b64_tr_b16 %0, %1" : "=v"(lo) : "v"((uint32_t)(uintptr_t)ad.lo));
        asm volatile("ds_read_b64_tr_b16 %0, %1" : "=v"(hi) : "v"((uint32_t)(uintptr_t)ad.hi));
        const u32x4 v = {lo[0], lo[1], hi[0], hi[1]};
        f = __builtin_bit_cast(bf16x8, v);
    }
    template <int BM, int TR, int TC, bool BIAS>
    static __device__ __forceinline__ void step(const char* Ys, const char* Xs, int r0, int c0, int lane, f32x4 (&acc)[TR][TC], bool bias, f32x4 (&accb)[BIAS ? TR : 1]) {
        static_assert(WG_BK == 32, "one 32-deep sub-step");
        bf16x8 af[TR], bfr[TC];
        TrFragAddr ay[TR], ax[TC];
#pragma unroll
        for (int t = 0; t < TR; ++t) ay[t] = tr_frag_addr<tr_swz_mode(BM * 2)>(Ys, BM * 2, r0 + t * 16, lane);
#pragma unroll
        for (int t = 0; t < TC; ++t) ax[t] = tr_frag_addr<tr_swz_mode(WG_BN * 2)>(Xs, WG_BN * 2, c0 + t * 16, lane);
        __builtin_amdgcn_sched_barrier(0);
#pragma unroll
        for (int t = 0; t < TC; ++t) read2(bfr[t], ax[t]);
#pragma unroll
        for (int t = 0; t < TR; ++t) read2(af[t], ay[t]);
#pragma unroll
        for (int a = 0; a < TR; ++a) {
            __builtin_amdgcn_sched_barrier(0);
            if (a == 0) asm volatile("s_waitcnt lgkmcnt(%0)" ::"n"(2 * (TR - 1)) : "memory");
            else if (a == 1) asm volatile("s_waitcnt lgkmcnt(%0)" ::"n"(TR > 2 ? 2 * (TR - 2) : 0) : "memory");
            else if (a == 2) asm volatile("s_waitcnt lgkmcnt(%0)" ::"n"(TR > 3 ? 2 * (TR - 3) : 0) : "memory");
            else asm volatile("s_waitcnt lgkmcnt(0)" ::: "memory");
            asm volatile("" : "+v"(af[a]));
            if (a == 0) {
#pragma unroll
                for (int b = 0; b < TC; ++b) asm volatile("" : "+v"(bfr[b]));
            }
#pragma unroll
            for (int b = 0; b < TC; ++b)
                acc[a][b] = __builtin_amdgcn_mfma_f32_16x16x32_bf16(bfr[b], af[a], acc[a][b], 0, 0, 0);
            if (BIAS && bias) {
                typedef __attribute__((ext_vector_type(8))) short s16x8;
                const s16x8 one8 = {0x3F80, 0x3F80, 0x3F80, 0x3F80, 0x3F80, 0x3F80, 0x3F80, 0x3F80};
                const bf16x8 ones = __builtin_bit_cast(bf16x8, one8);
                if constexpr (BIAS) accb[a] = __builtin_amdgcn_mfma_f32_16x16x32_bf16(ones, af[a], accb[a], 0, 0, 0);
            }
        }
        __builtin_amdgcn_sched_barrier(0);
    }
};
template <> struct WFrag<float> {
    template <int BM, int TR, int TC, bool BIAS>
    static __device__ __forceinline__ void step(const char* Ys, const char* Xs, int r0, int c0, int lane, f32x4 (&acc)[TR][TC], bool bias, f32x4 (&accb)[BIAS ? TR : 1]) {
        const int kq = lane >> 4, i = lane & 15;
#pragma unroll
        for (int ks = 0; ks < WG_BK / 4; ++ks) {
            float af[TR], bfr[TC];
#pragma unroll
            for (int t = 0; t < TR; ++t) af[t] = *reinterpret_cast<const float*>(Ys + ((4 * ks + kq) * BM + r0 + t * 16 + i) * 4);
#pragma unroll
            for (int t = 0; t < TC; ++t) bfr[t] = *reinterpret_cast<const float*>(Xs + ((4 * ks + kq) * WG_BN + c0 + t * 16 + i) * 4);
#pragma unroll
            for (int a = 0; a < TR; ++a)
#pragma unroll
                for (int b = 0; b < TC; ++b) acc[a][b] = __builtin_amdgcn_mfma_f32_16x16x4f32(bfr[b], af[a], acc[a][b], 0, 0, 0);
            if (BIAS && bias) {
#pragma unroll
                for (int a = 0; a < (BIAS ? TR : 1); ++a) accb[a] = __builtin_amdgcn_mfma_f32_16x16x4f32(1.0f, af[a], accb[a], 0, 0, 0);
            }
        }
    }
};

template <typename T, int BM> struct WgTile {
    static constexpr int NT = 256;
    static constexpr int CH = ElemTraits<T>::CH, ES = (int)sizeof(T);
    static constexpr int YCW = BM * ES / 16, XCW = WG_BN * ES / 16;
    static constexpr int YT = WG_BK * YCW < NT ? WG_BK * YCW : NT;
    static constexpr int NY = (WG_BK * YCW + NT - 1) / NT, NX = WG_BK * XCW / NT;
    static constexpr int WCOLS = WG_BN / 64, WROWS = (NT / 64) / WCOLS;
    static constexpr int WM = BM / WROWS, TR = WM / 16, TC = 4;
    static constexpr int YBYTES = WG_BK * BM * ES, XBYTES = WG_BK * WG_BN * ES, STAGE = YBYTES + XBYTES;
    static_assert(NY >= 1 && NX >= 1, "tile too small");
    static constexpr bool SWZ = std::is_same<T, bf16_t>::value;
    static_assert(NT / XCW >= 16 || !SWZ, "bf16: a block-wide load covers >= 16 rows, so a thread's rows share the row bits the swizzle uses");
    int yrow0, ych;
    bool y_cok, x_cok;
    int xrow0, ci, dh, dw;
    __device__ __forceinline__ WgTile(const WgradArgs& a, int tid, int j0, int co0) {
        const int ytid = tid % YT;
        yrow0 = ytid / YCW;
        const int ycc = SWZ ? ((ytid % YCW) ^ (tr_swz<tr_swz_mode(YCW * 16)>(yrow0) << 1)) : (ytid % YCW);
        ych = co0 + ycc * CH;
        y_cok = ych < a.CoutP;
        xrow0 = tid / XCW;
        const int xcc = SWZ ? ((tid % XCW) ^ (tr_swz<tr_swz_mode(XCW * 16)>(xrow0) << 1)) : (tid % XCW);
        const int j = j0 + xcc * CH;
        x_cok = j < a.NG;
        const int tap = x_cok ? j / a.Cin : 0;
        ci = x_cok ? j - tap * a.Cin : 0;
        dh = tap / a.KW - a.pad;
        dw = tap % a.KW - a.pad;
    }
    __device__ __forceinline__ int y_row(int i) const { return yrow0 + i * (NT / YCW); }
    __device__ __forceinline__ int x_row(int i) const { return xrow0 + i * (NT / XCW); }
    static __device__ __forceinline__ lptr_t y_slot(char* Ys, int i, int wave) { return (lptr_t)(Ys + (i * NT + (wave * 64) % YT) * 16); }
    static __device__ __forceinline__ lptr_t x_slot(char* Xs, int i, int wave) { return (lptr_t)(Xs + (i * NT + wave * 64) * 16); }
};

template <typename T, int BM> struct WgRasterWalk {
    using G = WgTile<T, BM>;
    const WgradArgs& a;
    const G& ld;
    const int wave, m_end;
    const int s_ = a.stride, ldx32 = (int)a.ldx, ldy32 = (int)a.ldy;
    const int q_ = WG_BK / a.Wo, r_ = WG_BK - q_ * a.Wo;
    const uint32_t d_step = (uint32_t)((q_ * s_ * a.W + r_ * s_) * ldx32);
    const uint32_t d_wwrap = (uint32_t)((s_ * a.W - a.Wo * s_) * ldx32);
    const uint32_t d_hwrap = (uint32_t)((a.H * a.W - a.Ho * s_ * a.W) * ldx32);
    const uint32_t y_step = (uint32_t)(WG_BK * ldy32);
    const int ws_lim = a.Wo * s_, hs_lim = a.Ho * s_;
    int x_ws[G::NX], x_hs[G::NX];
    uint32_t x_off[G::NX], y_off[G::NY];
    __device__ __forceinline__ WgRasterWalk(const WgradArgs& a_, const G& ld_, int wave_, int m_begin)
        : a(a_), ld(ld_), wave(wave_), m_end(min(a_.Mpix, m_begin + a_.pix_per_split)) {
#pragma unroll
        for (int i = 0; i < G::NX; ++i) {
            const int m = m_begin + ld.x_row(i);
            const int t = wg_fast_div(m, a.wo_mul, a.wo_shr);
            const int wo = m - t * a.Wo;
            const int n = wg_fast_div(t, a.ho_mul, a.ho_shr);
            const int ho = t - n * a.Ho;
            x_ws[i] = wo * s_;
            x_hs[i] = ho * s_;
            x_off[i] = (uint32_t)(((n * a.H + ho * s_ + ld.dh) * a.W + wo * s_ + ld.dw) * ldx32 + ld.ci);
        }
#pragma unroll
        for (int i = 0; i < G::NY; ++i) y_off[i] = (uint32_t)((m_begin + ld.y_row(i)) * ldy32 + ld.ych);
    }
    __device__ __forceinline__ void issue(char* Ys, int mk) {
        const T* __restrict__ xg = reinterpret_cast<const T*>(a.x);
        const T* __restrict__ yg = reinterpret_cast<const T*>(a.dy);
        const T* zero = reinterpret_cast<const T*>(a.zero);
        char* Xs = Ys + G::YBYTES;
        const int left = m_end - mk;
#pragma unroll
        for (int i = 0; i < G::NY; ++i) {
            const bool ok = ld.y_cok && ld.y_row(i) < left;
            const T* src = ok ? yg + y_off[i] : zero;
            wg_global_to_lds(src, ld.y_slot(Ys, i, wave));
            y_off[i] += y_step;
        }
#pragma unroll
        for (int i = 0; i < G::NX; ++i) {
            const bool ok = ld.x_cok && ld.x_row(i) < left && (unsigned)(x_hs[i] + ld.dh) < (unsigned)a.H && (unsigned)(x_ws[i] + ld.dw) < (unsigned)a.W;
            const T* src = ok ? xg + x_off[i] : zero;
            wg_global_to_lds(src, ld.x_slot(Xs, i, wave));
            x_ws[i] += r_ * s_;
            x_hs[i] += q_ * s_;
            x_off[i] += d_step;
            if (x_ws[i] >= ws_lim) {
                x_ws[i] -= ws_lim;
                x_hs[i] += s_;
                x_off[i] += d_wwrap;
            }
            while (x_hs[i] >= hs_lim) {
                x_hs[i] -= hs_lim;
                x_off[i] += d_hwrap;
            }
        }
    }
};

template <typename T, int BM> struct WgPatchWalk {
    using G = WgTile<T, BM>;
    static constexpr uint32_t OOR = 0x80000000u;
    static constexpr int ES = G::ES;
    const WgradArgs& a;
    const int wave;
    const int s_ = a.stride, ldx32 = (int)a.ldx, ldy32 = (int)a.ldy;
    const int pw = 1 << a.pw_shift, ph = WG_BK >> a.pw_shift;
    const uint32_t xbias = (uint32_t)((a.W + 1) * ldx32 * ES);
    uint32_t pvx[G::NX], pvy[G::NY];
    int pch[G::NX], pcw[G::NX];
    int p_wo, p_ho;
    uint32_t p_sx, p_sy;
    __device__ __forceinline__ WgPatchWalk(const WgradArgs& a_, const G& ld, int wave_, int m_begin) : a(a_), wave(wave_) {
#pragma unroll
        for (int i = 0; i < G::NX; ++i) {
            const int row = ld.x_row(i);
            const int pr = row >> a.pw_shift, pc = row & (pw - 1);
            pch[i] = pr * s_ + ld.dh;
            pcw[i] = pc * s_ + ld.dw;
            pvx[i] = ld.x_cok ? (uint32_t)(((pch[i] * a.W + pcw[i]) * ldx32 + ld.ci) * ES) + xbias : OOR;
        }
#pragma unroll
        for (int i = 0; i < G::NY; ++i) {
            const int row = ld.y_row(i);
            const int pr = row >> a.pw_shift, pc = row & (pw - 1);
            pvy[i] = ld.y_cok ? (uint32_t)(((pr * a.Wo + pc) * ldy32 + ld.ych) * ES) : OOR;
        }
        const int pidx = __builtin_amdgcn_readfirstlane(m_begin / WG_BK);
        const int npw = a.Wo >> a.pw_shift, nph = a.Ho / ph;
        const int t = pidx / npw, wp = pidx - t * npw;
        const int n = t / nph, hp = t - n * nph;
        p_wo = wp * pw;
        p_ho = hp * ph;
        p_sx = (uint32_t)(((n * a.H + p_ho * s_) * a.W + p_wo * s_) * ldx32 * ES);
        p_sy = (uint32_t)(((n * a.Ho + p_ho) * a.Wo + p_wo) * ldy32 * ES);
    }
    __device__ __forceinline__ void issue(char* Ys, int) {
        char* Xs = Ys + G::YBYTES;
        const char* xbase = reinterpret_cast<const char*>(a.x) - xbias;
        const uint32_t sx = __builtin_amdgcn_readfirstlane(p_sx), sy = __builtin_amdgcn_readfirstlane(p_sy);
#pragma unroll
        for (int i = 0; i < G::NY; ++i) wg_buffer_to_lds(a.dy, a.y_bytes, G::y_slot(Ys, i, wave), pvy[i], sy);
        const int hs0 = __builtin_amdgcn_readfirstlane(p_ho * s_), ws0 = __builtin_amdgcn_readfirstlane(p_wo * s_);
#pragma unroll
        for (int i = 0; i < G::NX; ++i) {
            const bool ok = (unsigned)(hs0 + pch[i]) < (unsigned)a.H && (unsigned)(ws0 + pcw[i]) < (unsigned)a.W;
            wg_buffer_to_lds(xbase, a.x_bytes + xbias, G::x_slot(Xs, i, wave), ok ? pvx[i] : OOR, sx);
        }
        p_wo += pw;
        p_sx += (uint32_t)(pw * s_ * ldx32 * ES);
        p_sy += (uint32_t)(pw * ldy32 * ES);
        if (p_wo == a.Wo) {
            p_wo = 0;
            p_ho += ph;
            p_sx += (uint32_t)((ph * s_ * a.W - a.Wo * s_) * ldx32 * ES);
            p_sy += (uint32_t)((ph * a.Wo - a.Wo) * ldy32 * ES);
            if (p_ho == a.Ho) {
                p_ho = 0;
                p_sx += (uint32_t)((a.H * a.W - a.Ho * s_ * a.W) * ldx32 * ES);
            }
        }
    }
};

template <typename S, int TR> struct SlabStage {
    static constexpr int ES = (int)sizeof(S);
    static constexpr int SROW = 64 * ES + 16;
    static constexpr int CPR = 64 * ES / 16;
    static constexpr int RPI = 64 / CPR;
    static constexpr int RP = TR < 4 / ES ? TR : 4 / ES;
    static constexpr int BYTES = RP * 16 * SROW;
    static_assert(TR % RP == 0, "whole passes");
};
template <typename S, int TR, int TC>
__device__ __forceinline__ void wg_store_slab_staged(char* ring, int wave, int lane, const f32x4 (&acc)[TR][TC], S* slab, int row0, int col0, int CoutP, int NG) {
    using St = SlabStage<S, TR>;
    constexpr int ES = St::ES, SROW = St::SROW, RP = St::RP;
    static_assert(TC * 16 == 64, "a wave's tile is 64 columns wide");
    __syncthreads();
    asm volatile("" : "+v"(lane));
    char* st = ring + wave * St::BYTES;
    const int l15 = lane & 15, l4 = lane >> 4;
    const int srow = lane / St::CPR, sch = lane % St::CPR;
    const int col = col0 + sch * (16 / ES);
#pragma unroll
    for (int r0 = 0; r0 < TR; r0 += RP) {
#pragma unroll
        for (int rr = 0; rr < RP; ++rr)
#pragma unroll
            for (int c = 0; c < TC; ++c) {
                char* p = st + (rr * 16 + l15) * SROW + (c * 16 + 4 * l4) * ES;
                if constexpr (std::is_same<S, float>::value) {
                    *reinterpret_cast<f32x4*>(p) = acc[r0 + rr][c];
                } else {
                    const bf16x4 v = {(bf16_t)acc[r0 + rr][c][0], (bf16_t)acc[r0 + rr][c][1], (bf16_t)acc[r0 + rr][c][2], (bf16_t)acc[r0 + rr][c][3]};
                    *reinterpret_cast<bf16x4*>(p) = v;
                }
            }
        __builtin_amdgcn_fence(__ATOMIC_RELEASE, "wavefront");
        __builtin_amdgcn_wave_barrier();
        __builtin_amdgcn_fence(__ATOMIC_ACQUIRE, "wavefront");
#pragma unroll
        for (int k = 0; k < RP * 16 / St::RPI; ++k) {
            const int row = k * St::RPI + srow;
            const u32x4 u = *reinterpret_cast<const u32x4*>(st + row * SROW + sch * 16);
            const int co = row0 + r0 * 16 + row;
            if (co < CoutP && col < NG) *reinterpret_cast<u32x4*>(slab + (int64_t)co * NG + col) = u;
        }
        __builtin_amdgcn_fence(__ATOMIC_RELEASE, "wavefront");
        __builtin_amdgcn_wave_barrier();
        __builtin_amdgcn_fence(__ATOMIC_ACQUIRE, "wavefront");
    }
}

template <typename T, int BM, bool BIAS, bool PATCH>
__global__ __launch_bounds__(256, (BM == 128 ? 3 : WG_WAVES)) void wgrad_kernel(WgradArgs a, BnRider rider) {
    using G = WgTile<T, BM>;
    constexpr int NT = G::NT, TR = G::TR, TC = G::TC, WM = G::WM, STAGE = G::STAGE, NS = WG_NS;
    constexpr int LDS = (int)wgrad_lds_bytes<T, BM>();
    static_assert(LDS == NS * STAGE, "the launcher's LDS bytes are the ring");
    static_assert(LDS >= (NT / 64) * SlabStage<bf16_t, TR>::BYTES && LDS >= (NT / 64) * SlabStage<float, TR>::BYTES, "the staged slab stores use the ring");
    static_assert(LDS >= BN_FINAL_RED * (int)sizeof(double), "a rider workgroup sums its slices in the ring");
    extern __shared__ __attribute__((aligned(16))) char smem[];

    const int tid = threadIdx.x, lane = tid & 63;
    const int wave = __builtin_amdgcn_readfirstlane(tid >> 6);
    const int wr = wave / G::WCOLS, wc = wave % G::WCOLS;
    int bx, by, bz;
    if (rider.nwg && (int)blockIdx.x < rider.nwg) {
        if ((int)blockIdx.x * 32 < rider.f.C) bn_final_block<NT, false>(rider.f, (int)blockIdx.x, reinterpret_cast<double*>(smem));
        return;
    }
    if (a.xcd_map) {
        const int id = (int)blockIdx.x - rider.nwg, xcd = id & 7, seq = id >> 3, nxy = a.nx * a.ny;
        const int zi = seq / nxy, t = seq - zi * nxy;
        const int spx = (a.splits + 7) >> 3;
        bz = xcd * spx + zi;
        if (zi >= spx || bz >= a.splits) return;
        by = t / a.nx;
        bx = t - by * a.nx;
    } else {
        bx = blockIdx.x; by = blockIdx.y; bz = blockIdx.z;
    }
    const int j0 = bx * WG_BN, co0 = by * BM;
    const int m_begin = bz * a.pix_per_split;
    const int m_end = min(a.Mpix, m_begin + a.pix_per_split);
    const G ld(a, tid, j0, co0);
    typename std::conditional<PATCH, WgPatchWalk<T, BM>, WgRasterWalk<T, BM>>::type walk(a, ld, wave, m_begin);

    f32x4 acc[TR][TC];
#pragma unroll
    for (int r = 0; r < TR; ++r)
#pragma unroll
        for (int c = 0; c < TC; ++c) acc[r][c] = f32x4{0.f, 0.f, 0.f, 0.f};

    const bool do_bias = BIAS && bx == 0 && wc == 0;
    f32x4 accb[BIAS ? TR : 1];
#pragma unroll
    for (int r = 0; r < (BIAS ? TR : 1); ++r) accb[r] = f32x4{0.f, 0.f, 0.f, 0.f};
    const int nk = (m_end - m_begin + WG_BK - 1) / WG_BK;
    constexpr int LPT = G::NY + G::NX;
#pragma unroll
    for (int s = 0; s < NS - 1; ++s)
        if (s < nk) walk.issue(smem + s * STAGE, m_begin + s * WG_BK);
    for (int kt = 0; kt < nk; ++kt) {
        if (kt + NS - 2 < nk) wait_vmcnt_barrier<LPT * (NS - 2)>();
        else wait_vmcnt_barrier<0>();
        if (kt + NS - 1 < nk) walk.issue(smem + ((kt + NS - 1) % NS) * STAGE, m_begin + (kt + NS - 1) * WG_BK);
        const char* Ys = smem + (kt % NS) * STAGE;
        WFrag<T>::template step<BM, TR, TC, BIAS>(Ys, Ys + G::YBYTES, wr * WM, wc * 64, lane, acc, do_bias, accb);
    }

    const int64_t slab_off = (int64_t)bz * a.CoutP * a.NG;
    const int row0 = co0 + wr * WM, col0 = j0 + wc * 64;
    const int l15 = lane & 15, l4 = lane >> 4;
    if (BIAS && do_bias && l4 == 0) {
#pragma unroll
        for (int r = 0; r < (BIAS ? TR : 1); ++r) {
            const int co = row0 + r * 16 + l15;
            if (co < a.CoutP) a.bias_slab[(int64_t)bz * a.CoutP + co] = accb[r][0];
        }
    }
    if constexpr (std::is_same<T, bf16_t>::value) {
        if (a.slab_bf16) wg_store_slab_staged<bf16_t>(smem, wave, lane, acc, reinterpret_cast<bf16_t*>(a.slab) + slab_off, row0, col0, a.CoutP, a.NG);
        else wg_store_slab_staged<float>(smem, wave, lane, acc, reinterpret_cast<float*>(a.slab) + slab_off, row0, col0, a.CoutP, a.NG);
    } else {
#pragma unroll
        for (int r = 0; r < TR; ++r) {
            const int co = row0 + r * 16 + l15;
#pragma unroll
            for (int c = 0; c < TC; ++c) {
                const int col = col0 + c * 16 + 4 * l4;
                if (co < a.CoutP && col < a.NG) *reinterpret_cast<f32x4*>(reinterpret_cast<float*>(a.slab) + slab_off + (int64_t)co * a.NG + col) = acc[r][c];
            }
        }
    }
}


template <typename S> __device__ __forceinline__ float wg_split_sum(const S* __restrict__ p, int64_t e, int64_t stride, int splits) {
    float s0 = 0.f, s1 = 0.f, s2 = 0.f, s3 = 0.f;
    int k = 0;
    for (; k + 3 < splits; k += 4) {
        s0 += (float)p[e + (int64_t)k * stride];
        s1 += (float)p[e + (int64_t)(k + 1) * stride];
        s2 += (float)p[e + (int64_t)(k + 2) * stride];
        s3 += (float)p[e + (int64_t)(k + 3) * stride];
    }
    for (; k < splits; ++k) s0 += (float)p[e + (int64_t)k * stride];
    return (s0 + s1) + (s2 + s3);
}

template <bool BF>
__global__ void wgrad_reduce_kernel(const void* __restrict__ slab, int splits, int CoutP, int NG, int Cin, int cout_real, int cin_real, int ntaps,
                                    float* __restrict__ dw) {
    typedef typename std::conditional<BF, bf16_t, float>::type S;
    const uint32_t total = (uint32_t)cout_real * (uint32_t)ntaps * (uint32_t)cin_real;
    const int64_t sstride = (int64_t)CoutP * NG;
    for (uint32_t idx = blockIdx.x * blockDim.x + threadIdx.x; idx < total; idx += gridDim.x * blockDim.x) {
        const uint32_t t = idx / (uint32_t)cin_real;
        const uint32_t ci = idx - t * (uint32_t)cin_real;
        const uint32_t co = t / (uint32_t)ntaps;
        const uint32_t tap = t - co * (uint32_t)ntaps;
        const int64_t e = (int64_t)co * NG + tap * Cin + ci;
        dw[((int64_t)co * cin_real + ci) * ntaps + tap] = wg_split_sum(reinterpret_cast<const S*>(slab), e, sstride, splits);
    }
}

__device__ __forceinline__ void bias_slab_sum(const float* __restrict__ bs, int splits, int coutp, float* __restrict__ db, int tid, int nthr) {
    for (int co = tid; co < coutp; co += nthr) db[co] = wg_split_sum(bs, co, coutp, splits);
}
__global__ void wgrad_bias_reduce_kernel(const float* __restrict__ bs, int splits, int coutp, float* __restrict__ db) {
    bias_slab_sum(bs, splits, coutp, db, (int)(blockIdx.x * blockDim.x + threadIdx.x), (int)(gridDim.x * blockDim.x));
}
template <bool BF> __device__ __forceinline__ void reduce_batch_body(const ymi_wgrad_pending& e, f32x4* red) {
    if (e.bias_slab && (int)blockIdx.x == e.first_block) bias_slab_sum(e.bias_slab, e.splits, (int)(e.elems / e.ng), e.dbias, (int)threadIdx.x, 256);
    constexpr int EPT = BF ? 8 : 4, Q = EPT / 4;
    const int SL = e.lanes, OUTS = 256 / SL;
    const int ol = threadIdx.x % OUTS, lane = threadIdx.x / OUTS;
    const int64_t el = ((int64_t)((int)blockIdx.x - e.first_block) * OUTS + ol) * EPT;
    f32x4 s0[Q], s1[Q], s2[Q], s3[Q];
#pragma unroll
    for (int q = 0; q < Q; ++q) s0[q] = s1[q] = s2[q] = s3[q] = f32x4{0.f, 0.f, 0.f, 0.f};
    auto add_split = [&](f32x4 (&acc)[Q], int k) {
        const int64_t off = el + (int64_t)k * e.elems;
        if constexpr (BF) {
            const bf16x8 v = *reinterpret_cast<const bf16x8*>(reinterpret_cast<const bf16_t*>(e.slab) + off);
            acc[0] += f32x4{(float)v[0], (float)v[1], (float)v[2], (float)v[3]};
            acc[1] += f32x4{(float)v[4], (float)v[5], (float)v[6], (float)v[7]};
        } else {
            acc[0] += *reinterpret_cast<const f32x4*>(reinterpret_cast<const float*>(e.slab) + off);
        }
    };
    if (el < e.elems) {
        int k = lane;
        for (; k + 3 * SL < e.splits; k += 4 * SL) {
            add_split(s0, k);
            add_split(s1, k + SL);
            add_split(s2, k + 2 * SL);
            add_split(s3, k + 3 * SL);
        }
        for (; k < e.splits; k += SL) add_split(s0, k);
    }
#pragma unroll
    for (int q = 0; q < Q; ++q) red[(q * SL + lane) * OUTS + ol] = (s0[q] + s1[q]) + (s2[q] + s3[q]);
    __syncthreads();
    if (lane == 0 && el < e.elems) {
#pragma unroll
        for (int q = 0; q < Q; ++q) {
            f32x4 s = {0.f, 0.f, 0.f, 0.f};
            for (int c = 0; c < SL; ++c) s += red[(q * SL + c) * OUTS + ol];
            const uint32_t eu = (uint32_t)el + 4u * q;
            const int co = (int)(eu / (uint32_t)e.ng), col = (int)(eu - (uint32_t)co * (uint32_t)e.ng);
            const int tap = (int)((uint32_t)col / (uint32_t)e.cin), ci = col - tap * e.cin;
            if (co < e.cout_real) {
#pragma unroll
                for (int r = 0; r < 4; ++r)
                    if (ci + r < e.cin_real) e.dw[((int64_t)co * e.cin_real + ci + r) * e.ntaps + tap] = s[r];
            }
        }
    }
}
__global__ __launch_bounds__(256) void wgrad_reduce_batch_kernel(const ymi_wgrad_pending* __restrict__ tab, int n) {
    __shared__ f32x4 red[512];
    int lo = 0, hi = n - 1;
    while (lo < hi) {
        const int mid = (lo + hi + 1) >> 1;
        if (tab[mid].first_block <= (int)blockIdx.x) lo = mid;
        else hi = mid - 1;
    }
    const ymi_wgrad_pending e = tab[lo];
    if (e.slab_bf16) reduce_batch_body<true>(e, red);
    else reduce_batch_body<false>(e, red);
}

static void wg_find_divisor(int d, uint32_t* mul, uint32_t* shr) {
    int lg = 0;
    while ((1 << lg) < d) ++lg;
    *mul = (uint32_t)((((uint64_t)1 << 32) * (((uint64_t)1 << lg) - (uint64_t)d)) / (uint64_t)d + 1);
    *shr = (uint32_t)lg;
}

struct WgradPlan {
    int splits, pix_per_split;
    size_t slab_bytes;
};
static int wgrad_bm(int64_t coutp, bool bf16) {
    if (!bf16) return 64;
    if (coutp <= 32) return 32;
    return (coutp >= 128 && coutp % 128 == 0) || coutp >= 256 ? 128 : 64;
}
static WgradPlan wgrad_plan(int64_t mpix, int64_t coutp, int64_t ng, int bm, size_t slab_esize) {
    const int64_t tiles = ((ng + WG_BN - 1) / WG_BN) * ((coutp + bm - 1) / bm);
    const int target64 = ymi_opt(OPT_WGRAD_BLOCKS);
    const int target128 = ymi_opt(OPT_WGRAD_BLOCKS128);
    const int target = bm == 128 ? target128 : target64;
    int64_t s = (target + tiles - 1) / tiles;
    const int64_t smax = (mpix + 255) / 256;
    if (s > smax) s = smax;
    if (s < 1) s = 1;
    if (s >= 8) s = (s + 7) / 8 * 8 <= smax ? (s + 7) / 8 * 8 : s / 8 * 8;
    int64_t pps = (mpix + s - 1) / s;
    pps = (pps + WG_BK - 1) / WG_BK * WG_BK;
    s = (mpix + pps - 1) / pps;
    WgradPlan p;
    p.splits = (int)s;
    p.pix_per_split = (int)pps;
    p.slab_bytes = ((size_t)s * coutp * ng * slab_esize + 255) / 256 * 256;
    return p;
}

static int64_t pad_to(int64_t v, int64_t m) { return (v + m - 1) / m * m; }
constexpr int64_t WG_BIAS_ROWS = 2048 * 2 + 1;

extern "C" size_t ymi_conv2d_bwd_weight_workspace(int64_t m_rows, int64_t cout, int64_t cin, int64_t kh, int64_t kw) {
    const int64_t coutp = pad_to(cout, 8), cinp = pad_to(cin, 8);
    WgradPlan p = wgrad_plan(m_rows, coutp, kh * kw * cinp, 64, 4);
    const WgradPlan p128 = wgrad_plan(m_rows, coutp, kh * kw * cinp, 128, 4);
    if (p128.slab_bytes > p.slab_bytes) p = p128;
    return p.slab_bytes + (size_t)WG_BIAS_ROWS * coutp * sizeof(float) + 256;
}

static int wgrad_impl(const ymi_tensor* x, const ymi_tensor* dy, int64_t cout_real, int64_t cin_real, int64_t kh, int64_t kw, int64_t stride,
                      float* dw_oihw, float* dbias, void* workspace, size_t workspace_bytes, ymi_wgrad_pending* pending, void* stream);

struct WgradLaunch {
    WgradArgs a;
    dim3 grid;
    int bm;
    bool bf16;
    hipStream_t s;
    double flop, bytes;
};
template <typename T, int BM> static void wgrad_launch_tile(const WgradArgs& a, const BnRider& r, dim3 grid, hipStream_t s) {
    constexpr size_t lds = wgrad_lds_bytes<T, BM>();
    static_assert(lds <= 64 * 1024, "a larger ring needs hipFuncAttributeMaxDynamicSharedMemorySize");
    void (*kernel)(WgradArgs, BnRider) = a.bias_slab ? wgrad_kernel<T, BM, true, false> : wgrad_kernel<T, BM, false, false>;
    if constexpr (std::is_same<T, bf16_t>::value) {
        if (a.pw_shift >= 0) kernel = a.bias_slab ? wgrad_kernel<T, BM, true, true> : wgrad_kernel<T, BM, false, true>;
    }
    hipLaunchKernelGGL(kernel, grid, dim3(256), lds, s, a, r);
}
static void wgrad_launch(const WgradLaunch& h, const BnFinal* rider) {
    BnRider r{};
    dim3 grid = h.grid;
    if (rider && h.a.xcd_map) {
        r.f = *rider;
        r.nwg = ((rider->C + 31) / 32 + 7) / 8 * 8;
        grid.x += (unsigned)r.nwg;
    }
    int prof = -1;
    if (ymi_prof_enabled()) prof = ymi_prof_start(h.s, 1, h.flop, h.bytes, h.bf16 ? 2500.0 : 157.3);
    if (!h.bf16) wgrad_launch_tile<float, 64>(h.a, r, grid, h.s);
    else if (h.bm == 128) wgrad_launch_tile<bf16_t, 128>(h.a, r, grid, h.s);
    else if (h.bm == 32) wgrad_launch_tile<bf16_t, 32>(h.a, r, grid, h.s);
    else wgrad_launch_tile<bf16_t, 64>(h.a, r, grid, h.s);
    ymi_prof_stop(h.s, prof);
}
static struct WgradHeld {
    std::mutex mu;
    bool on = false;
    bool valid = false;
    WgradLaunch launch;
    int device = 0;
} g_held;
static int wgrad_current_device() {
    int d = 0;
    (void)hipGetDevice(&d);
    return d;
}
static void wgrad_flush_held_locked(const BnFinal* rider = nullptr) {
    if (!g_held.valid) return;
    g_held.valid = false;
    const int cur = wgrad_current_device();
    if (cur != g_held.device) (void)hipSetDevice(g_held.device);
    wgrad_launch(g_held.launch, rider);
    if (cur != g_held.device) (void)hipSetDevice(cur);
}
bool ymi_wgrad_issue_held(const BnFinal* f, hipStream_t stream) {
    std::lock_guard<std::mutex> lk(g_held.mu);
    if (!g_held.valid || g_held.launch.s != stream || g_held.device != wgrad_current_device()) return false;
    wgrad_flush_held_locked(f);
    return true;
}
extern "C" int ymi_wgrad_hold(int32_t mode) {
    std::lock_guard<std::mutex> lk(g_held.mu);
    if (mode == 2) {
        g_held.valid = false;
        return YMI_OK;
    }
    YMI_CHECK_ARG(mode == 0 || mode == 1, "wgrad_hold: mode 0, 1 or 2");
    if (mode == 0) wgrad_flush_held_locked();
    g_held.on = mode == 1;
    return hipGetLastError() == hipSuccess ? YMI_OK : YMI_ELAUNCH;
}

extern "C" int ymi_conv2d_bwd_weight(const ymi_tensor* x, const ymi_tensor* dy, int64_t cout_real, int64_t cin_real, int64_t kh, int64_t kw,
                                     int64_t stride, float* dw_oihw, float* dbias, void* workspace, size_t workspace_bytes, void* stream) {
    return wgrad_impl(x, dy, cout_real, cin_real, kh, kw, stride, dw_oihw, dbias, workspace, workspace_bytes, nullptr, stream);
}

extern "C" int ymi_conv2d_bwd_weight_deferred(const ymi_tensor* x, const ymi_tensor* dy, int64_t cout_real, int64_t cin_real, int64_t kh, int64_t kw,
                                              int64_t stride, float* dw_oihw, float* dbias, void* workspace, size_t workspace_bytes,
                                              ymi_wgrad_pending* pending, void* stream) {
    YMI_CHECK_ARG(pending, "conv2d_bwd_weight_deferred: null pending record");
    return wgrad_impl(x, dy, cout_real, cin_real, kh, kw, stride, dw_oihw, dbias, workspace, workspace_bytes, pending, stream);
}

ymi_wgrad_pending ymi_wgrad_record(const void* slab, float* dw, int64_t elems, int splits, int ng, int cin, int cout_real, int cin_real, int ntaps,
                                   bool slab_bf16, const float* bias_slab, float* dbias) {
    const int lanes = splits > 128 ? 32 : splits > 32 ? 16 : splits > 8 ? 8 : 4;
    const int outs = 256 / lanes, ept = slab_bf16 ? 8 : 4;
    return ymi_wgrad_pending{slab, dw, elems, splits, ng, cin, cout_real, cin_real, ntaps, lanes, 0, (int32_t)((elems / ept + outs - 1) / outs), slab_bf16 ? 1 : 0,
                             bias_slab, dbias};
}

constexpr int WG_TABLE_CHUNK = 48;
static_assert(sizeof(ymi_wgrad_pending) == 80, "ymi_wgrad_pending layout (mirrored in _lib.py)");
struct WgradTableChunk {
    ymi_wgrad_pending e[WG_TABLE_CHUNK];
};
__global__ void wgrad_table_write_kernel(WgradTableChunk c, int n, ymi_wgrad_pending* __restrict__ table) {
    const int i = threadIdx.x;
    if (i < n) table[i] = c.e[i];
}

extern "C" int ymi_wgrad_reduce_batch(const ymi_wgrad_pending* host_records, int32_t n, ymi_wgrad_pending* device_table, void* stream) {
    YMI_CHECK_ARG(host_records && device_table && n > 0, "wgrad_reduce_batch: args");
    hipStream_t s = (hipStream_t)stream;
    {
        std::lock_guard<std::mutex> lk(g_held.mu);
        wgrad_flush_held_locked();
    }
    int64_t total = 0;
    for (int base = 0; base < n; base += WG_TABLE_CHUNK) {
        WgradTableChunk c{};
        const int m = n - base < WG_TABLE_CHUNK ? n - base : WG_TABLE_CHUNK;
        for (int i = 0; i < m; ++i) {
            c.e[i] = host_records[base + i];
            YMI_CHECK_ARG(c.e[i].slab && c.e[i].dw && c.e[i].blocks > 0 && (c.e[i].lanes == 4 || c.e[i].lanes == 8 || c.e[i].lanes == 16 || c.e[i].lanes == 32),
                          "wgrad_reduce_batch: record %d", base + i);
            c.e[i].first_block = (int32_t)total;
            total += c.e[i].blocks;
        }
        hipLaunchKernelGGL(wgrad_table_write_kernel, dim3(1), dim3(64), 0, s, c, m, device_table + base);
    }
    YMI_CHECK_ARG(total < (1ll << 31), "wgrad_reduce_batch: too many workgroups");
    hipLaunchKernelGGL(wgrad_reduce_batch_kernel, dim3((unsigned)total), dim3(256), 0, s, (const ymi_wgrad_pending*)device_table, (int)n);
    YMI_CHECK_LAUNCH("wgrad_reduce_batch");
    return YMI_OK;
}

static int wgrad_impl(const ymi_tensor* x, const ymi_tensor* dy, int64_t cout_real, int64_t cin_real, int64_t kh, int64_t kw, int64_t stride,
                      float* dw_oihw, float* dbias, void* workspace, size_t workspace_bytes, ymi_wgrad_pending* pending, void* stream) {
    YMI_CHECK_ARG(ymi_tensor_ok(x) && ymi_tensor_ok(dy) && dw_oihw && workspace, "conv2d_bwd_weight: bad argument");
    YMI_CHECK_ARG(x->dtype == dy->dtype, "conv2d_bwd_weight: dtype mismatch");
    const int ch = x->dtype == YMI_BF16 ? 8 : 4;
    YMI_CHECK_ARG(x->c % ch == 0 && x->ld % ch == 0 && dy->c % ch == 0 && dy->ld % ch == 0, "conv2d_bwd_weight: channels must be multiples of %d", ch);
    YMI_CHECK_ARG(kh == kw && (kh == 1 || kh == 3) && (stride == 1 || stride == 2), "conv2d_bwd_weight: k in {1,3}, stride in {1,2}");
    const int64_t pad = kh / 2;
    YMI_CHECK_ARG(dy->n == x->n && dy->h == (x->h + 2 * pad - kh) / stride + 1 && dy->w == (x->w + 2 * pad - kw) / stride + 1, "conv2d_bwd_weight: shapes");
    YMI_CHECK_ARG(cout_real <= dy->c && cin_real <= x->c, "conv2d_bwd_weight: real channel counts");
    YMI_CHECK_ARG(ymi_pixels(x) * x->ld < (1ll << 31) && ymi_pixels(dy) * dy->ld < (1ll << 31), "conv2d_bwd_weight: too large");
    const int64_t mpix = ymi_pixels(dy);
    const int64_t ng = kh * kw * x->c;
    const bool bf16 = x->dtype == YMI_BF16;
    const int bm = wgrad_bm(dy->c, bf16), bn = WG_BN;
    WgradPlan p = wgrad_plan(mpix, dy->c, ng, bm, bf16 ? 2 : 4);
    const bool slab_bf16 = bf16 && p.splits >= 16;
    if (bf16 && !slab_bf16) p = wgrad_plan(mpix, dy->c, ng, bm, 4);
    size_t need = p.slab_bytes + (dbias ? (size_t)WG_BIAS_ROWS * dy->c * sizeof(float) : 0);
    if (workspace_bytes < need) {
        ymi_set_error("conv2d_bwd_weight: workspace %zu < %zu bytes", workspace_bytes, need);
        return YMI_EWORKSPACE;
    }
    WgradArgs a{};
    a.x = x->data; a.dy = dy->data; a.slab = workspace; a.slab_bf16 = slab_bf16 ? 1 : 0; a.zero = ymi_zero_page();
    a.bias_slab = dbias ? reinterpret_cast<float*>(reinterpret_cast<char*>(workspace) + p.slab_bytes) : nullptr;
    YMI_CHECK_ARG(!dbias || p.splits <= WG_BIAS_ROWS, "conv2d_bwd_weight: too many splits for the bias partials");
    a.ldx = x->ld; a.ldy = dy->ld;
    a.Mpix = (int)mpix; a.H = (int)x->h; a.W = (int)x->w; a.Ho = (int)dy->h; a.Wo = (int)dy->w;
    a.stride = (int)stride; a.pad = (int)pad; a.KW = (int)kw;
    a.CoutP = (int)dy->c; a.Cin = (int)x->c; a.NG = (int)ng; a.pix_per_split = p.pix_per_split;
    wg_find_divisor(a.Wo, &a.wo_mul, &a.wo_shr);
    wg_find_divisor(a.Ho, &a.ho_mul, &a.ho_shr);
    a.nx = (int)((ng + bn - 1) / bn); a.ny = (int)((dy->c + bm - 1) / bm); a.splits = p.splits;
    a.pw_shift = -1;
    {
        const int64_t xb = ymi_pixels(x) * x->ld * ymi_esize(x->dtype), yb = ymi_pixels(dy) * dy->ld * ymi_esize(dy->dtype);
        const int64_t margin = (x->w + 2) * x->ld * (int64_t)ymi_esize(x->dtype);
        if (bf16 && ymi_opt(OPT_WGRAD_PATCH) && xb + margin < (1ll << 31) && yb < (1ll << 31) && mpix % WG_BK == 0) {
            for (int sh = 5; sh >= 0; --sh) {
                const int pw = 1 << sh, ph = WG_BK >> sh;
                if (dy->w % pw == 0 && dy->h % ph == 0) {
                    a.pw_shift = sh;
                    break;
                }
            }
            a.x_bytes = (uint32_t)xb;
            a.y_bytes = (uint32_t)yb;
        }
    }
    a.xcd_map = p.splits >= 8 ? 1 : 0;
    dim3 grid((unsigned)a.nx, (unsigned)a.ny, (unsigned)p.splits);
    if (a.xcd_map) grid = dim3((unsigned)(8 * ((p.splits + 7) / 8) * a.nx * a.ny), 1, 1);
    hipStream_t s = (hipStream_t)stream;
    const double es = (double)ymi_esize(x->dtype);
    WgradLaunch h{a, grid, bm, bf16, s, 2.0 * (double)mpix * (double)dy->c * (double)ng,
                  ((double)ymi_pixels(x) * x->c + (double)mpix * dy->c) * es + (double)dy->c * ng * 4.0};
    {
        std::lock_guard<std::mutex> lk(g_held.mu);
        wgrad_flush_held_locked();
        if (pending && g_held.on && a.xcd_map) {
            g_held.launch = h;
            g_held.device = wgrad_current_device();
            g_held.valid = true;
        } else {
            wgrad_launch(h, nullptr);
        }
    }
    YMI_CHECK_LAUNCH("wgrad");
    if (pending) {
        *pending = ymi_wgrad_record(a.slab, dw_oihw, (int64_t)a.CoutP * a.NG, p.splits, a.NG, a.Cin, (int)cout_real, (int)cin_real, (int)(kh * kw), slab_bf16,
                                    a.bias_slab, dbias);
    } else {
        const int64_t total = cout_real * kh * kw * cin_real;
        int64_t gb = (total + 255) / 256;
        if (gb > 2048) gb = 2048;
        hipLaunchKernelGGL(slab_bf16 ? wgrad_reduce_kernel<true> : wgrad_reduce_kernel<false>, dim3((unsigned)gb), dim3(256), 0, s, (const void*)a.slab, p.splits,
                           a.CoutP, a.NG, a.Cin, (int)cout_real, (int)cin_real, (int)(kh * kw), dw_oihw);
    }
    YMI_CHECK_LAUNCH("wgrad_reduce");
    if (dbias && !pending) {
        hipLaunchKernelGGL(wgrad_bias_reduce_kernel, dim3((unsigned)((dy->c + 255) / 256)), dim3(256), 0, s, (const float*)a.bias_slab, p.splits, (int)dy->c, dbias);
        YMI_CHECK_LAUNCH("wgrad_bias_reduce");
    }
    return YMI_OK;
}
```

### improving_yolov8_cbam_swinblock_amd/ops/base.py

```python
import ctypes
import os

import torch

from .. import _lib
from .._lib import ACT_GELU, ACT_NONE, ACT_SILU, ConvProblem, DgradProblem, as_ymi, check, chunk_elems, empty_nhwc, is_nhwc, ptr, stream_ptr, workspace, ymi_dtype

_byref = ctypes.byref


def L():
    return _lib.lib()


HOOKS = {
    "fused_swin_mlp": True,
    "detect_pair": True,
    "detect_multi": True,
    "first_conv": True,
    "stat_atomics": True,
    "wgrad_rider": True,
}


def compute_dtype(x):
    if torch.is_autocast_enabled("cuda") if hasattr(torch, "is_autocast_enabled") else False:
        dt = torch.get_autocast_dtype("cuda")
        if dt != torch.bfloat16:
            raise RuntimeError(f"libyolo_mi355 supports bfloat16 autocast only (got {dt}); fp16 has no kernels here")
        return dt
    return x.dtype if x.dtype in (torch.float32, torch.bfloat16) else torch.float32


def round_up(v, m):
    return (v + m - 1) // m * m


def _dense_ok(t, dtype):
    ch = chunk_elems(dtype)
    if t.dtype != dtype or not is_nhwc(t):
        return False
    n, c, h, w = t.shape
    ld = as_ymi(t).ld
    return c % ch == 0 and ld % ch == 0 and t.data_ptr() % 16 == 0


class _ToInternal(torch.autograd.Function):

    @staticmethod
    def forward(ctx, x, dtype):
        n, c, h, w = x.shape
        cp = round_up(c, chunk_elems(dtype))
        src = x.detach()
        if src.dtype != torch.float32 or not src.is_contiguous():
            src = src.float().contiguous()
        out = empty_nhwc(n, cp, h, w, dtype, x.device)
        check(L().ymi_nchw_to_nhwc(ptr(src), n, c, h, w, _byref(as_ymi(out)), stream_ptr()), "nchw_to_nhwc")
        ctx.c = c
        ctx.in_dtype = x.dtype
        return out

    @staticmethod
    def backward(ctx, g):
        g = grad_nhwc(g, g.dtype if g.dtype in (torch.float32, torch.bfloat16) else torch.float32)
        n, cp, h, w = g.shape
        full = torch.empty((n, cp, h, w), dtype=torch.float32, device=g.device)
        check(L().ymi_nhwc_to_nchw(_byref(as_ymi(g)), ptr(full), stream_ptr()), "nhwc_to_nchw")
        return full[:, : ctx.c].to(ctx.in_dtype), None


def to_internal(x, dtype=None):
    dtype = dtype or compute_dtype(x)
    if not x.is_cuda:
        raise RuntimeError("improving_yolov8_cbam_swinblock_amd runs on the MI355X only: move the input to 'cuda' (no CPU path)")
    if _dense_ok(x, dtype):
        return x
    return _ToInternal.apply(x, dtype)


def grad_nhwc(g, dtype):
    if g.dtype != dtype:
        g = g.to(dtype)
    if g.dim() == 4:
        if not _dense_ok(g, dtype):
            n, c, h, w = g.shape
            buf = empty_nhwc(n, c, h, w, dtype, g.device)
            buf.copy_(g)
            g = buf
    elif g.dim() == 2:
        if g.stride(1) != 1 or g.stride(0) % 4 != 0 or g.data_ptr() % 16 != 0:
            g = g.contiguous()
    return g


def to_nchw_float(x):
    n, c, h, w = x.shape
    out = torch.empty((n, c, h, w), dtype=torch.float32, device=x.device)
    check(L().ymi_nhwc_to_nchw(_byref(as_ymi(x.detach())), ptr(out), stream_ptr()), "nhwc_to_nchw")
    return out


def _as4d(w):
    return w if w.dim() == 4 else w.view(w.shape[0], w.shape[1], 1, 1)


def _conv_out_hw(h, w, k, s):
    p = k // 2
    return (h + 2 * p - k) // s + 1, (w + 2 * p - k) // s + 1


class RunState:

    def __init__(self):
        self.model = None
        self.arena = None
        self.defer = False
        self.records, self.keep, self.owners, self.bias = [], [], [], []
        self.task = None
        self.table = None
        self.side = False
        self.side_pending, self.side_keep = False, []
        self.side_streams = {}
        self.grad_views = None
        self.riders = False
        self.padded = {}


RUN = RunState()


def _note_use(*params):
    m = RUN.model
    epoch = (id(m), m.epoch) if m is not None else None
    for w in params:
        if w is None:
            continue
        st = getattr(w, "_ymi_use", None)
        if st is None or (epoch is not None and st[0] != epoch):
            w._ymi_use = [epoch, 1]
        else:
            st[1] += 1


def _stat_acc(cout, device):
    n = 8 * cout
    m = RUN.model
    if m is not None:
        m.need += n
        if m.acc is not None and m.acc.device == device and m.cursor + n <= m.acc.numel():
            m.cursor += n
            return m.acc[m.cursor - n : m.cursor]
    return torch.zeros(n, dtype=torch.int64, device=device)


def _count_batch(bn):
    if bn.num_batches_tracked is None:
        return
    if RUN.model is not None:
        RUN.model.counters.append(bn.num_batches_tracked)
    else:
        bn.num_batches_tracked.add_(1)


def _deferred_twice(params):
    for p in params:
        st = getattr(p, "_ymi_use", None) if p is not None else None
        if st is not None and st[1] > 1:
            return True
    return False


def _in_backward():
    try:
        return torch._C._current_graph_task_id() != -1
    except AttributeError:
        return False


class GradJoin:

    __slots__ = ("n", "seen", "pending", "out", "dst")

    def __init__(self, n):
        self.n, self.seen, self.pending = int(n), 0, []
        self.dst = None
        self.out = None

    def arrive(self):
        self.seen += 1
        if self.seen < self.n:
            return None
        out, self.pending, self.seen = self.pending, [], 0
        return out

    def deposit(self, g):
        self.pending.append(g)


def mark_join(t, consumers, force=False):
    if (consumers > 1 or force) and torch.is_grad_enabled() and t.requires_grad:
        t._ymi_join = GradJoin(consumers)
    return t


def join_of(t):
    return getattr(t, "_ymi_join", None) if torch.is_grad_enabled() else None


def _accumulate(total, adds):
    for a in adds:
        a = grad_nhwc(a, total.dtype) if a.dim() == 4 else a.to(total.dtype)
        check(L().ymi_add_inplace(_byref(as_ymi(a)), _byref(as_ymi(total)), stream_ptr()), "add_inplace")
    return total


def _join_plain(join, g):
    if join is None:
        return g
    adds = join.arrive()
    if adds is None:
        join.deposit(g)
        return None
    if not adds:
        return g
    total = empty_nhwc(*g.shape, g.dtype, g.device) if g.dim() == 4 else torch.empty_like(g)
    total.copy_(g)
    return _accumulate(total, adds)


def _prep_adds(adds, dtype):
    out = []
    for a in adds or ():
        if a.dtype != dtype:
            a = a.to(dtype)
        a = grad_nhwc(a, dtype)
        out.append(a)
    return out


class OutSlot:

    def __init__(self, buf, off, lazy=None):
        self.buf, self.off, self.lazy = buf, int(off), lazy

    def view(self, n, c, h, w, dtype):
        if self.buf is None and self.lazy is not None:
            self.buf = self.lazy.get(n, h, w, dtype)
        b = self.buf
        if b.dtype != dtype or b.shape[0] != n or b.shape[2] != h or b.shape[3] != w or self.off + c > b.shape[1]:
            raise RuntimeError(f"output slot [{self.off}:{self.off + c}] of {tuple(b.shape)} {b.dtype} does not fit a {(n, c, h, w)} {dtype} result")
        return b[:, self.off : self.off + c]


class LazyConcatBuffer:

    def __init__(self, channels, device):
        self.channels, self.device, self.buf = int(channels), device, None

    def get(self, n, h, w, dtype):
        if self.buf is None:
            self.buf = empty_nhwc(n, self.channels, h, w, dtype, self.device)
        return self.buf


class _GradBuffer:

    def __init__(self, shape, device):
        self.shape, self.device, self.buf = tuple(shape), device, None

    def get(self, dtype):
        if self.buf is None:
            n, c, h, w = self.shape
            self.buf = empty_nhwc(n, c, h, w, dtype, self.device)
        return self.buf if self.buf.dtype == dtype else None


class _GradSlot:
    __slots__ = ("gb", "lo", "hi")

    def __init__(self, gb, lo, hi):
        self.gb, self.lo, self.hi = gb, lo, hi

    def view(self, dtype):
        b = self.gb.get(dtype)
        return None if b is None else b[:, self.lo : self.hi]
```

### improving_yolov8_cbam_swinblock_amd/ops/conv.py

```python
import ctypes
from collections import namedtuple
from dataclasses import make_dataclass

import torch

from .. import _lib
from .._lib import ACT_NONE, ACT_SILU, ConvProblem, DgradProblem, as_ymi, check, chunk_elems, empty_nhwc, is_nhwc, ptr, stream_ptr, workspace
from .base import (
    HOOKS, RUN, L, _GradBuffer, _GradSlot, _accumulate, _as4d, _byref, _conv_out_hw, _count_batch, _deferred_twice, _dense_ok, _in_backward,
    _join_plain, _note_use, _prep_adds, _stat_acc, compute_dtype, grad_nhwc, join_of, mark_join, round_up,
)
from .weights import (
    _adoptable, _defer_wgrad, _new_dw, _wgrad_maybe_async, pack_conv_dgrad, pack_conv_dgrad_pair, pack_conv_fwd, pack_conv_fwd_pair,
)

DgradJob = namedtuple("DgradJob", "dy ty wd cin k stride fused rest dx dxv")
FwdProblem = make_dataclass("FwdProblem", ["x", "wp", "cout", "k", "y", ("bias", object, None), ("part", object, None), ("pstride", int, 0), ("poff", int, 0),
                                           ("blocks", int, 0)])


def _dgrad_prepare(dy, weight4, k, stride, in_shape, dtype, adds=None, out=None, packed=None):
    shape = tuple(in_shape)
    cp = shape[1]
    ty = as_ymi(dy)
    if packed is not None:
        wd, cin = packed
    else:
        cin = weight4.shape[1]
        wd = pack_conv_dgrad(weight4, ty.c, stride, dtype)
    dx = out if (out is not None and tuple(out.shape) == shape and cp == cin) else None
    if dx is None:
        dx = empty_nhwc(*shape, dtype, dy.device) if len(shape) == 4 else torch.empty(shape, dtype=dtype, device=dy.device)
    dxv = dx
    if cp != cin:
        dx.zero_()
        dxv = dx[:, :cin]
    adds = _prep_adds(adds, dtype)
    sparse = k == 1 and stride > 1
    if sparse and cp == cin:
        dx.zero_()
    fused = adds[:2] if (cp == cin and not sparse) else []
    return DgradJob(dy, ty, wd, cin, k, stride, fused, adds[len(fused):], dx, dxv)


def _dgrad_finish(job):
    if job.rest:
        _accumulate(job.dxv, job.rest)
    return job.dx


def _dgrad(dy, weight4, k, stride, in_shape, dtype, adds=None, out=None, packed=None):
    return _dgrad_launch(_dgrad_prepare(dy, weight4, k, stride, in_shape, dtype, adds, out, packed))


def _dgrad_launch(j):
    a1 = _byref(as_ymi(j.fused[0])) if len(j.fused) > 0 else None
    a2 = _byref(as_ymi(j.fused[1])) if len(j.fused) > 1 else None
    check(L().ymi_conv2d_bwd_data_add(_byref(j.ty), ptr(j.wd), j.cin, j.k, j.k, j.stride, a1, a2, _byref(as_ymi(j.dxv)), stream_ptr()), "conv2d_bwd_data")
    return _dgrad_finish(j)


def _width_class(c, dtype):
    cpt = int(c) // chunk_elems(dtype)
    return (cpt % 4 == 0, cpt % 8 == 0)


def _launch_grouped(items, key, struct, fill, entry, what):
    groups = {}
    for it in items:
        groups.setdefault(key(it), []).append(it)
    done = []
    for g in groups.values():
        for s in range(0, len(g), 8):
            chunk = g[s : s + 8]
            arr = (struct * len(chunk))()
            keep = [fill(q, it) for q, it in zip(arr, chunk)]
            check(entry(arr, len(chunk), stream_ptr()), what)
            done += zip(chunk, arr)
    return done


def _fill_dgrad(q, j):
    ts = [j.ty, as_ymi(j.dxv)] + [as_ymi(a) for a in j.fused]
    for name, t in zip(("dy", "dx", "add1", "add2"), ts):
        setattr(q, name, ctypes.pointer(t))
    q.w_dgrad_packed, q.cin, q.k = j.wd.data_ptr(), j.cin, j.k
    return ts


def _fill_fwd(q, p):
    ts = [as_ymi(p.x), as_ymi(p.y)]
    q.x, q.y = ctypes.pointer(ts[0]), ctypes.pointer(ts[1])
    q.w_packed, q.cout, q.kh, q.kw, q.stride, q.act = p.wp.data_ptr(), p.cout, p.k, p.k, 1, ACT_NONE
    if p.bias is not None:
        q.bias = p.bias.data_ptr()
    if p.part is not None:
        q.stat_partials, q.stat_stride, q.stat_offset = p.part.data_ptr(), p.pstride, p.poff
    return ts


def _dgrad_multi(jobs, dtype):
    if any(j.stride != 1 for j in jobs):
        raise RuntimeError("_dgrad_multi: stride 1 only")
    _launch_grouped(jobs, lambda j: _width_class(j.ty.c, dtype), DgradProblem, _fill_dgrad, L().ymi_conv2d_bwd_data_multi, "conv2d_bwd_data_multi")
    return [_dgrad_finish(j) for j in jobs]


def _conv_fwd_multi(problems, dtype):
    for p, q in _launch_grouped(problems, lambda p: (_width_class(p.x.shape[1], dtype), p.part is not None), ConvProblem, _fill_fwd,
                                L().ymi_conv2d_fwd_multi, "conv2d_fwd_multi"):
        p.blocks = int(q.stat_blocks)


def _dgrad_joined_prepare(join, dy, weight4, k, stride, in_shape, dtype, packed=None):
    adds = join.arrive() if join is not None else []
    out = None
    if adds is not None and join is not None and join.dst is not None:
        cand = join.dst.view(dtype)
        join.dst = None
        if cand is not None and tuple(cand.shape) == tuple(in_shape) and _dense_ok(cand, dtype) and not (k == 1 and stride > 1):
            out = cand
    elif adds is not None and join is not None and join.out is not None:
        out, join.out = join.out, None
        if len(adds) < 2 and _dense_ok(out, dtype) and tuple(out.shape) == tuple(in_shape) and not (k == 1 and stride > 1):
            adds = list(adds) + [out]
        else:
            out = None
    return _dgrad_prepare(dy, weight4, k, stride, in_shape, dtype, adds, out, packed), adds is None


def _dgrad_joined_finish(join, dx, deposit):
    if deposit:
        join.deposit(dx)
        return None
    return dx


def _dgrad_joined(join, dy, weight4, k, stride, in_shape, dtype, packed=None):
    job, deposit = _dgrad_joined_prepare(join, dy, weight4, k, stride, in_shape, dtype, packed)
    return _dgrad_joined_finish(join, _dgrad_launch(job), deposit)


def _stat_ws_bytes(m, o):
    return (L().ymi_conv2d_stat_blocks(m, o) * 2 * o + 2 * o) * 4


def _bn_act_bwd(dout, raw, stats, act, gamma, beta, second=None):
    o, dev = raw.shape[1], raw.device
    draw = empty_nhwc(*raw.shape, raw.dtype, dev)
    dgamma = torch.empty(o, dtype=torch.float32, device=dev)
    dbeta = torch.empty(o, dtype=torch.float32, device=dev)
    ws = workspace(2048 * 2 * o * 4 + 256, dev, "bnbwd")
    if second is None:
        check(L().ymi_bn_act_bwd(_byref(as_ymi(dout)), _byref(as_ymi(raw)), ptr(gamma), ptr(stats[0]), ptr(stats[1]), ptr(beta), act,
                                 _byref(as_ymi(draw)), ptr(dgamma), ptr(dbeta), ptr(ws), ws.numel(), stream_ptr()), "bn_act_bwd")
    else:
        gamma_b, beta_b, oa = second
        check(L().ymi_bn_act_bwd_pair(_byref(as_ymi(dout)), _byref(as_ymi(raw)), ptr(gamma), ptr(beta), ptr(gamma_b), ptr(beta_b), oa, ptr(stats[0]), ptr(stats[1]),
                                      act, _byref(as_ymi(draw)), ptr(dgamma), ptr(dbeta), ptr(ws), ws.numel(), stream_ptr()), "bn_act_bwd_pair")
    return draw, dgamma, dbeta


class _ConvBnAct(torch.autograd.Function):

    @staticmethod
    def forward(ctx, x, weight, gamma, beta, running_mean, running_var, stride, eps, momentum, act, residual, slot=None, join=None, res_join=None):
        dtype = x.dtype
        o, i, k, _ = weight.shape
        n, cp, h, w = x.shape
        ho, wo = _conv_out_hw(h, w, k, stride)
        dev = x.device
        _note_use(weight)
        wp = pack_conv_fwd(weight, cp, dtype)
        raw = empty_nhwc(n, o, ho, wo, dtype, dev)
        out = slot.view(n, o, ho, wo, dtype) if slot is not None else empty_nhwc(n, o, ho, wo, dtype, dev)
        stats = torch.empty((2, o), dtype=torch.float32, device=dev)
        ws = workspace(_stat_ws_bytes(n * ho * wo, o), dev, "conv")
        res = residual
        tres = _byref(as_ymi(res)) if res is not None else None
        if (HOOKS["stat_atomics"] and o % 4 == 0 and L().ymi_conv2d_bn_silu_fwd_acc_ok(_byref(as_ymi(raw)), _byref(as_ymi(out)), tres)
                and all(t is None or t.data_ptr() % 16 == 0 for t in (gamma, beta, running_mean, running_var))):
            acc = _stat_acc(o, dev)
            check(
                L().ymi_conv2d_bn_silu_fwd_acc(
                    _byref(as_ymi(x)), ptr(wp), o, k, k, stride, ptr(gamma), ptr(beta), ptr(running_mean), ptr(running_var),
                    momentum, eps, act, tres, _byref(as_ymi(raw)), _byref(as_ymi(out)), ptr(stats[0]), ptr(stats[1]), ptr(acc), stream_ptr(),
                ),
                "conv2d_bn_silu_fwd_acc",
            )
        else:
            check(
                L().ymi_conv2d_bn_silu_fwd(
                    _byref(as_ymi(x)), ptr(wp), o, k, k, stride, ptr(gamma), ptr(beta), ptr(running_mean), ptr(running_var),
                    momentum, eps, act, tres, _byref(as_ymi(raw)), _byref(as_ymi(out)), ptr(stats[0]), ptr(stats[1]), ptr(ws), ws.numel(), stream_ptr(),
                ),
                "conv2d_bn_silu_fwd",
            )
        ctx.save_for_backward(x, weight, gamma, beta, raw, stats)
        ctx.cfg = (stride, act, i, residual is not None)
        ctx.joins = (join, res_join)
        return out

    @staticmethod
    def backward(ctx, dout):
        x, weight, gamma, beta, raw, stats = ctx.saved_tensors
        stride, act, cin, has_res = ctx.cfg
        dtype = x.dtype
        o, _, k, _ = weight.shape
        dout = grad_nhwc(dout, dtype)
        draw, dgamma, dbeta = _bn_act_bwd(dout, raw, stats, act, gamma, beta)
        join, res_join = ctx.joins
        dres = _join_plain(res_join, dout) if (has_res and ctx.needs_input_grad[10]) else None
        dx = None
        if ctx.needs_input_grad[0]:
            dx = _dgrad_joined(join, draw, weight, k, stride, x.shape, dtype)
        dw = None
        if ctx.needs_input_grad[1]:
            dw, _ = _wgrad_maybe_async(x, draw, o, cin, k, stride, False, (weight,))
        return dx, dw, dgamma, dbeta, None, None, None, None, None, None, dres, None, None, None


def conv_bn_act(x, weight, bn, stride, act=ACT_SILU, residual=None, slot=None):
    if bn.momentum is None:
        raise RuntimeError("BatchNorm with cumulative moving average (momentum=None) is not supported")
    if torch.is_grad_enabled() and weight.shape[0] % chunk_elems(x.dtype) != 0 and (x.requires_grad or weight.requires_grad):
        raise NotImplementedError(f"training a Conv with {weight.shape[0]} output channels in {x.dtype}: the backward kernels need channel counts in "
                                  f"whole 16-byte chunks (multiples of {chunk_elems(x.dtype)}); every standard YOLOv8 width is - use float32 for this width")
    out = _ConvBnAct.apply(x, weight, bn.weight, bn.bias, bn.running_mean, bn.running_var, int(stride), float(bn.eps), float(bn.momentum), int(act), residual, slot,
                           join_of(x), join_of(residual) if residual is not None else None)
    _count_batch(bn)
    return out


class _FirstConvBnAct(torch.autograd.Function):

    @staticmethod
    def forward(ctx, img, weight, gamma, beta, running_mean, running_var, eps, momentum, act):
        n, c, h, w = img.shape
        o = weight.shape[0]
        dt = torch.bfloat16
        dev = img.device
        ho, wo = _conv_out_hw(h, w, 3, 2)
        _note_use(weight)
        x4 = torch.empty((n, h, w, 4), dtype=dt, device=dev).permute(0, 3, 1, 2)
        out = empty_nhwc(n, o, ho, wo, dt, dev)
        stats = torch.empty((2, o), dtype=torch.float32, device=dev)
        need = (2 * o + (L().ymi_first_conv_stat_blocks(n, h, w) + 64) * 2 * o) * 4
        ws = workspace(need, dev, "conv")
        check(
            L().ymi_first_conv_bn_act_fwd(ptr(img), n, c, h, w, ptr(weight.detach()), o, ptr(gamma), ptr(beta), ptr(running_mean), ptr(running_var), momentum, eps,
                                          act, _byref(as_ymi(x4)), _byref(as_ymi(out)), ptr(stats[0]), ptr(stats[1]), ptr(ws), ws.numel(), stream_ptr()),
            "first_conv_bn_act_fwd",
        )
        ctx.save_for_backward(x4, weight, gamma, beta, stats)
        ctx.act = act
        return out

    @staticmethod
    def backward(ctx, dout):
        x4, weight, gamma, beta, stats = ctx.saved_tensors
        o, cin, k, _ = weight.shape
        dev = x4.device
        dout = grad_nhwc(dout, torch.bfloat16)
        dgamma = torch.empty(o, dtype=torch.float32, device=dev)
        dbeta = torch.empty(o, dtype=torch.float32, device=dev)
        n, _, h, w = x4.shape
        need = int(L().ymi_first_conv_bwd_workspace(n, h, w, o))
        defer = (ctx.needs_input_grad[1] and RUN.defer and _in_backward() and _adoptable((weight,)) and not _deferred_twice((weight,)))
        dw = _new_dw(o, cin, k, dev, (weight,), None)
        ws = torch.empty(need, dtype=torch.uint8, device=dev) if defer else workspace(need, dev, "firstconv")
        rec = _lib.WgradPending() if defer else None
        if defer:
            _defer_wgrad(rec, (ws, x4, dout), weight)
        check(
            L().ymi_first_conv_bn_act_bwd(_byref(as_ymi(x4)), ptr(weight.detach()), cin, o, ptr(gamma), ptr(beta), ptr(stats[0]), ptr(stats[1]), ctx.act,
                                          _byref(as_ymi(dout)), ptr(dgamma), ptr(dbeta), ptr(dw), ptr(ws), ws.numel(), _byref(rec) if defer else None, stream_ptr()),
            "first_conv_bn_act_bwd",
        )
        return None, (dw if ctx.needs_input_grad[1] else None), dgamma, dbeta, None, None, None, None, None


def first_conv_ok(x, conv, residual, slot):
    return (residual is None and slot is None and torch.is_tensor(x) and x.is_cuda and x.dim() == 4 and x.dtype == torch.float32 and x.is_contiguous()
            and x.shape[1] <= 4 and not x.requires_grad and conv.kernel_size == (3, 3) and conv.stride == (2, 2) and conv.in_channels == x.shape[1]
            and conv.out_channels in (16, 32, 48, 64) and x.shape[2] % 2 == 0 and x.shape[3] % 4 == 0 and x.data_ptr() % 16 == 0 and compute_dtype(x) == torch.bfloat16
            and HOOKS["first_conv"])


def first_conv_bn_act(img, weight, bn, act=ACT_SILU):
    if bn.momentum is None:
        raise RuntimeError("BatchNorm with cumulative moving average (momentum=None) is not supported")
    out = _FirstConvBnAct.apply(img, weight, bn.weight, bn.bias, bn.running_mean, bn.running_var, float(bn.eps), float(bn.momentum), int(act))
    _count_batch(bn)
    return out


class _ChanSplit2(torch.autograd.Function):

    @staticmethod
    def forward(ctx, t, c):
        ctx.c, ctx.shape = c, tuple(t.shape)
        ctx.gb = _ChanSplit2.last = _GradBuffer(t.shape, t.device)
        return t[:, :c], t[:, c:]

    @staticmethod
    def backward(ctx, ga, gb):
        c = ctx.c
        buf = ctx.gb.buf
        ctx.gb.buf = None
        n, ctot, h, w = ctx.shape
        g0 = ga if ga is not None else gb
        if buf is None or buf.dtype != g0.dtype:
            buf = empty_nhwc(n, ctot, h, w, g0.dtype, g0.device)
        for g, dst in ((ga, buf[:, :c]), (gb, buf[:, c:])):
            if g is None:
                dst.zero_()
            elif not (g.data_ptr() == dst.data_ptr() and g.stride() == dst.stride() and g.dtype == dst.dtype):
                check(L().ymi_copy(_byref(as_ymi(grad_nhwc(g, buf.dtype))), _byref(as_ymi(dst)), stream_ptr()), "copy")
        return buf, None


def chan_split2(t, c):
    a, b = _ChanSplit2.apply(t, int(c))
    if torch.is_grad_enabled() and t.requires_grad:
        gb, _ChanSplit2.last = getattr(_ChanSplit2, "last", None), None
        if gb is not None:
            for v, lo, hi in ((a, 0, int(c)), (b, int(c), t.shape[1])):
                mark_join(v, 1, force=True)
                j = join_of(v)
                if j is not None:
                    j.dst = _GradSlot(gb, lo, hi)
    return a, b


class _ConvBnActPair(torch.autograd.Function):

    @staticmethod
    def forward(ctx, x, wa, ga, ba, rma, rva, wb, gb, bb, rmb, rvb, stride, eps, momentum, act, join):
        dtype = x.dtype
        oa, i, k, _ = wa.shape
        ob = wb.shape[0]
        o = oa + ob
        n, cp, h, w = x.shape
        ho, wo = _conv_out_hw(h, w, k, stride)
        dev = x.device
        _note_use(wa, wb)
        wp = pack_conv_fwd_pair(wa, wb, cp, dtype)
        raw = empty_nhwc(n, o, ho, wo, dtype, dev)
        out = empty_nhwc(n, o, ho, wo, dtype, dev)
        stats = torch.empty((2, o), dtype=torch.float32, device=dev)
        ws = workspace(_stat_ws_bytes(n * ho * wo, o), dev, "conv")
        check(
            L().ymi_conv2d_bn_silu_fwd_pair(
                _byref(as_ymi(x)), ptr(wp), o, oa, k, k, stride, ptr(ga), ptr(ba), ptr(rma), ptr(rva), ptr(gb), ptr(bb), ptr(rmb), ptr(rvb),
                momentum, eps, act, _byref(as_ymi(raw)), _byref(as_ymi(out)), ptr(stats[0]), ptr(stats[1]), ptr(ws), ws.numel(), stream_ptr(),
            ),
            "conv2d_bn_silu_fwd_pair",
        )
        ctx.save_for_backward(x, wa, wb, ga, ba, gb, bb, raw, stats)
        ctx.cfg = (stride, act, i)
        ctx.join = join
        return out

    @staticmethod
    def backward(ctx, dout):
        x, wa, wb, ga, ba, gb, bb, raw, stats = ctx.saved_tensors
        stride, act, cin = ctx.cfg
        dtype = x.dtype
        oa, _, k, _ = wa.shape
        o = oa + wb.shape[0]
        dout = grad_nhwc(dout, dtype)
        draw, dgamma, dbeta = _bn_act_bwd(dout, raw, stats, act, ga, ba, (gb, bb, oa))
        dx = None
        if ctx.needs_input_grad[0]:
            wd = pack_conv_dgrad_pair(wa, wb, stride, dtype)
            dx = _dgrad_joined(ctx.join, draw, None, k, stride, x.shape, dtype, packed=(wd, cin))
        nig = ctx.needs_input_grad
        dwa = dwb = None
        if nig[1] or nig[6]:
            dw, _ = _wgrad_maybe_async(x, draw, o, cin, k, stride, False, (wa, wb), pair_rows=oa)
            dwa, dwb = (dw[:oa] if nig[1] else None), (dw[oa:] if nig[6] else None)
        return (dx, dwa, dgamma[:oa], dbeta[:oa], None, None, dwb, dgamma[oa:], dbeta[oa:], None, None, None, None, None, None, None)


def conv_bn_act_pair(x, conv_a, bn_a, conv_b, bn_b, act=ACT_SILU):
    wa, wb = conv_a.weight, conv_b.weight
    if wa.shape[1:] != wb.shape[1:] or conv_a.stride != conv_b.stride:
        raise RuntimeError("conv_bn_act_pair: the two convolutions must share kernel size, stride and input width")
    if bn_a.momentum is None or bn_b.momentum is None or bn_a.eps != bn_b.eps or bn_a.momentum != bn_b.momentum:
        raise RuntimeError("conv_bn_act_pair: the two BatchNorms must share eps and momentum (initialize_weights sets them alike)")
    ch = chunk_elems(x.dtype)
    if wa.shape[0] % ch or wb.shape[0] % ch:
        raise NotImplementedError(f"conv_bn_act_pair: output widths {wa.shape[0]} / {wb.shape[0]} must be multiples of {ch} in {x.dtype}")
    out = _ConvBnActPair.apply(x, wa, bn_a.weight, bn_a.bias, bn_a.running_mean, bn_a.running_var, wb, bn_b.weight, bn_b.bias, bn_b.running_mean,
                               bn_b.running_var, int(conv_a.stride[0]), float(bn_a.eps), float(bn_a.momentum), int(act), join_of(x))
    _count_batch(bn_a)
    _count_batch(bn_b)
    return out


_Level = namedtuple("_Level", """x
    a0_w a0_gamma a0_beta a0_mean a0_var
    b0_w b0_gamma b0_beta b0_mean b0_var
    a1_w a1_gamma a1_beta a1_mean a1_var
    b1_w b1_gamma b1_beta b1_mean b1_var
    oa_w oa_bias ob_w ob_bias""")
_SAVED_ARGS = "x a0_w b0_w a0_gamma a0_beta b0_gamma b0_beta a1_w b1_w a1_gamma a1_beta b1_gamma b1_beta oa_w ob_w".split()
_Saved = namedtuple("_Saved", _SAVED_ARGS + "raw1 st1 h1 raw2 st2 h2".split())
_Geo = namedtuple("_Geo", "n cp h w c2 c3 o m ws_off stat_bytes")


def _per_level(rec, flat, nl):
    n = len(rec._fields)
    return [rec._make(flat[l * n : (l + 1) * n]) for l in range(nl)]


def _detect_args(xs, levels):
    t = []
    for x, (a0, b0, a1, b1, oa, ob) in zip(xs, levels):
        t.append(x)
        for m in (a0, b0, a1, b1):
            t += [m.conv.weight, m.bn.weight, m.bn.bias, m.bn.running_mean, m.bn.running_var]
        t += [oa.weight, oa.bias, ob.weight, ob.bias]
    return t


def _detect_grads(per_level):
    return (None,) + tuple(g for d in per_level for g in _Level(**{**dict.fromkeys(_Level._fields), **d}))


class _DetectTrain(torch.autograd.Function):

    @staticmethod
    def forward(ctx, meta, *t):
        nl, eps, momentum, joins, ncpad = meta
        lv = _per_level(_Level, t, nl)
        dtype, dev = lv[0].x.dtype, lv[0].x.device
        lib = L()
        geo = []
        need = 0
        for v in lv:
            n, cp, h, w = v.x.shape
            c2, c3 = v.a0_w.shape[0], v.b0_w.shape[0]
            g = _Geo(n, cp, h, w, c2, c3, c2 + c3, n * h * w, need, _stat_ws_bytes(n * h * w, c2 + c3))
            geo.append(g)
            need += 2 * g.stat_bytes
            _note_use(v.a0_w, v.b0_w, v.a1_w, v.b1_w, v.oa_w, v.ob_w)
        ws = workspace(need, dev, "detect").view(torch.float32)

        def region(g, stage):
            base, o = (g.ws_off + stage * g.stat_bytes) // 4, g.o
            return ws[base : base + o], ws[base + o : base + 2 * o], ws[base + 2 * o : base + g.stat_bytes // 4]

        def bn_stage(probs_of_level, stage, raws, bns):
            _conv_fwd_multi([p for ps in probs_of_level for p in ps], dtype)
            outs, stats = [], []
            for g, ps, raw, bn in zip(geo, probs_of_level, raws, bns):
                blocks = ps[0].blocks
                if any(p.blocks != blocks for p in ps):
                    raise RuntimeError("_DetectTrain: the convolutions of one BatchNorm group ran with different row tiles")
                scale, shift, part = region(g, stage)
                st = torch.empty((2, g.o), dtype=torch.float32, device=dev)
                out = empty_nhwc(g.n, g.o, g.h, g.w, dtype, dev)
                check(lib.ymi_bn_finalize_pair(ptr(part), blocks, g.m, g.o, g.c2, *map(ptr, bn), momentum, eps, ptr(scale), ptr(shift), ptr(st[0]), ptr(st[1]),
                                               stream_ptr()), "bn_finalize_pair")
                check(lib.ymi_scale_shift_act(_byref(as_ymi(raw)), ptr(scale), ptr(shift), ACT_SILU, None, _byref(as_ymi(out)), stream_ptr()), "scale_shift_act")
                outs.append(out)
                stats.append(st)
            return outs, stats

        raw1 = [empty_nhwc(g.n, g.o, g.h, g.w, dtype, dev) for g in geo]
        probs = [[FwdProblem(v.x, pack_conv_fwd_pair(v.a0_w, v.b0_w, g.cp, dtype), g.o, v.a0_w.shape[2], r, part=region(g, 0)[2], pstride=g.o)]
                 for v, g, r in zip(lv, geo, raw1)]
        h1, st1 = bn_stage(probs, 0, raw1, [(v.a0_gamma, v.a0_beta, v.a0_mean, v.a0_var, v.b0_gamma, v.b0_beta, v.b0_mean, v.b0_var) for v in lv])
        raw2 = [empty_nhwc(g.n, g.o, g.h, g.w, dtype, dev) for g in geo]
        probs = []
        for v, g, hh, r in zip(lv, geo, h1, raw2):
            c2, c3 = g.c2, g.c3
            part = region(g, 1)[2]
            probs.append([FwdProblem(hh[:, :c2], pack_conv_fwd(v.a1_w, c2, dtype), c2, v.a1_w.shape[2], r[:, :c2], part=part, pstride=g.o, poff=0),
                          FwdProblem(hh[:, c2:], pack_conv_fwd(v.b1_w, c3, dtype), c3, v.b1_w.shape[2], r[:, c2:], part=part, pstride=g.o, poff=c2)])
        h2, st2 = bn_stage(probs, 1, raw2, [(v.a1_gamma, v.a1_beta, v.a1_mean, v.a1_var, v.b1_gamma, v.b1_beta, v.b1_mean, v.b1_var) for v in lv])
        outs, probs = [], []
        for v, g, hh in zip(lv, geo, h2):
            c2, c3 = g.c2, g.c3
            ob, nc = v.oa_w.shape[0], v.ob_w.shape[0]
            box = empty_nhwc(g.n, ob, g.h, g.w, dtype, dev)
            cls = empty_nhwc(g.n, ncpad, g.h, g.w, dtype, dev)
            probs += [FwdProblem(hh[:, :c2], pack_conv_fwd(v.oa_w, c2, dtype), ob, 1, box, bias=v.oa_bias),
                      FwdProblem(hh[:, c2:], pack_conv_fwd(v.ob_w, c3, dtype), nc, 1, cls[:, :nc] if ncpad != nc else cls, bias=v.ob_bias)]
            outs += [box, cls]
        _conv_fwd_multi(probs, dtype)
        saved = []
        for v, r1, s1, a1, r2, s2, a2 in zip(lv, raw1, st1, h1, raw2, st2, h2):
            saved += _Saved(*[getattr(v, f) for f in _SAVED_ARGS], r1, s1, a1, r2, s2, a2)
        ctx.save_for_backward(*saved)
        ctx.bias_params = [(v.oa_bias if v.oa_bias.requires_grad else None, v.ob_bias if v.ob_bias.requires_grad else None) for v in lv]
        ctx.meta = (nl, joins, ncpad, geo)
        return tuple(outs)

    @staticmethod
    def backward(ctx, *gout):
        nl, joins, ncpad, geo = ctx.meta
        sv = _per_level(_Saved, ctx.saved_tensors, nl)
        need = [v._asdict() for v in _per_level(_Level, ctx.needs_input_grad[1:], nl)]
        grads = [{} for _ in range(nl)]
        dtype, dev = sv[0].x.dtype, sv[0].x.device

        def dgrad_halves(branches):
            jobs, bufs = [], []
            for l, g in enumerate(geo):
                pair = branches(l)
                buf = empty_nhwc(g.n, g.o, g.h, g.w, dtype, dev)
                for (dy, wt), lo, hi in zip(pair, (0, g.c2), (g.c2, g.o)):
                    jobs.append(_dgrad_prepare(dy, None, wt.shape[2], 1, (g.n, hi - lo, g.h, g.w), dtype, [], buf[:, lo:hi],
                                               (pack_conv_dgrad(wt, dy.shape[1], 1, dtype), hi - lo)))
                bufs.append(buf)
            _dgrad_multi(jobs, dtype)
            return bufs

# ... 201 lines not shown
```

### include/ymi.h

```cpp
#ifndef YMI_H
#define YMI_H

#include <stddef.h>
#include <stdint.h>

#ifdef __cplusplus
extern "C" {
#endif

#define YMI_VERSION 1

enum { YMI_F32 = 0, YMI_BF16 = 1 };
enum { YMI_ACT_NONE = 0, YMI_ACT_SILU = 1, YMI_ACT_GELU = 2 };
enum { YMI_OK = 0, YMI_EINVAL = -1, YMI_EALIGN = -2, YMI_ELAUNCH = -3, YMI_EWORKSPACE = -4 };

typedef struct ymi_tensor {
    void* data;
    int64_t n, h, w, c;
    int64_t ld;
    int32_t dtype;
    int32_t _pad;
} ymi_tensor;

int ymi_version(void);
const char* ymi_last_error(void);
int ymi_set_option(const char* name, int64_t value);
int64_t ymi_get_option(const char* name);

int ymi_profile_begin(int64_t capacity);
int ymi_profile_end(double* ms_by_family, double* flop_by_family, int64_t* launches_by_family);
int ymi_profile_end_ex(double* ms_by_family, double* flop_by_family, int64_t* launches_by_family, double* bytes_by_family,
                       double* bound_ms_by_family);


int ymi_nchw_to_nhwc(const float* src, int64_t n, int64_t c, int64_t h, int64_t w, const ymi_tensor* dst, void* stream);
int ymi_nhwc_to_nchw(const ymi_tensor* src, float* dst, void* stream);
int ymi_copy(const ymi_tensor* src, const ymi_tensor* dst, void* stream);
int ymi_upsample2x(const ymi_tensor* src, const ymi_tensor* dst, void* stream);
int ymi_upsample2x_bwd(const ymi_tensor* src, const ymi_tensor* dst, void* stream);
int ymi_upsample2x_bwd_acc(const ymi_tensor* src, const ymi_tensor* dst, void* stream);
int ymi_add_inplace(const ymi_tensor* src, const ymi_tensor* dst, void* stream);


int ymi_pack_conv_weight_fwd(const float* w_oihw, int64_t o, int64_t i, int64_t kh, int64_t kw, int64_t ipad, int32_t dtype, void* dst, void* stream);
int ymi_pack_conv_weight_dgrad(const float* w_oihw, int64_t o, int64_t i, int64_t kh, int64_t kw, int64_t stride, int32_t dtype, void* dst, void* stream);
int ymi_pack_conv_weight_dgrad_ex(const float* w_oihw, int64_t o_real, int64_t o_pad, int64_t i, int64_t kh, int64_t kw, int64_t stride, int32_t dtype, void* dst, void* stream);
int64_t ymi_conv_dgrad_pack_elems(int64_t o, int64_t i, int64_t kh, int64_t kw, int64_t stride);
typedef struct ymi_pack_desc {
    const float* src;
    void* dst_fwd;
    void* dst_dgrad;
    int32_t o, i, kh, kw, ipad, opad, stride;
    int32_t ostride;
    int32_t o_off;
    int32_t _pad;
} ymi_pack_desc;
int ymi_pack_conv_weights_batch(const void* descs_device, const int32_t* block_start_device, int32_t count, int32_t total_blocks,
                                int32_t dtype, void* stream);
int ymi_pack_matrix(const float* src, int64_t rows, int64_t cols, int32_t transpose, int32_t dtype, void* dst, void* stream);


int ymi_conv2d_fwd(const ymi_tensor* x, const void* w_packed, int64_t cout, int64_t kh, int64_t kw, int64_t stride,
                   const float* scale, const float* bias, int32_t act, const ymi_tensor* residual, const ymi_tensor* y,
                   float* stat_partials, int64_t* host_stat_blocks, void* stream);
int64_t ymi_conv2d_stat_blocks(int64_t m_rows, int64_t cout);
typedef struct ymi_conv_problem {
    const ymi_tensor* x;
    const void* w_packed;
    int64_t cout, kh, kw, stride;
    const float* scale;
    const float* bias;
    int32_t act, _pad;
    const ymi_tensor* residual;
    const ymi_tensor* y;
    float* stat_partials;
    int64_t stat_blocks;
    int64_t stat_stride, stat_offset;
} ymi_conv_problem;
int ymi_conv2d_fwd_multi(const ymi_conv_problem* problems, int32_t n, void* stream);

int ymi_bn_finalize(const float* stat_partials, int64_t blocks, int64_t count, int64_t c, const float* gamma, const float* beta,
                    float* running_mean, float* running_var, float momentum, float eps, float* scale, float* shift,
                    float* save_mean, float* save_invstd, void* stream);
int ymi_bn_finalize_pair(const float* stat_partials, int64_t blocks, int64_t count, int64_t c, int64_t split, const float* gamma, const float* beta,
                         float* running_mean, float* running_var, const float* gamma2, const float* beta2, float* running_mean2, float* running_var2,
                         float momentum, float eps, float* scale, float* shift, float* save_mean, float* save_invstd, void* stream);
int ymi_scale_shift_act(const ymi_tensor* raw, const float* scale, const float* shift, int32_t act, const ymi_tensor* residual,
                        const ymi_tensor* out, void* stream);

int ymi_conv2d_bn_silu_fwd(const ymi_tensor* x, const void* w_packed, int64_t cout, int64_t kh, int64_t kw, int64_t stride,
                           const float* gamma, const float* beta, float* running_mean, float* running_var, float momentum,
                           float eps, int32_t act, const ymi_tensor* residual, const ymi_tensor* raw, const ymi_tensor* out,
                           float* save_mean, float* save_invstd, void* workspace, size_t workspace_bytes, void* stream);

int ymi_conv2d_bn_silu_fwd_acc_ok(const ymi_tensor* raw, const ymi_tensor* out, const ymi_tensor* residual);
int ymi_conv2d_bn_silu_fwd_acc(const ymi_tensor* x, const void* w_packed, int64_t cout, int64_t kh, int64_t kw, int64_t stride,
                               const float* gamma, const float* beta, float* running_mean, float* running_var, float momentum,
                               float eps, int32_t act, const ymi_tensor* residual, const ymi_tensor* raw, const ymi_tensor* out,
                               float* save_mean, float* save_invstd, void* stat_acc, void* stream);

int ymi_bn_act_bwd(const ymi_tensor* dout, const ymi_tensor* raw, const float* gamma, const float* save_mean,
                   const float* save_invstd, const float* beta, int32_t act, const ymi_tensor* draw, float* dgamma, float* dbeta,
                   void* workspace, size_t workspace_bytes, void* stream);

int ymi_conv2d_bn_silu_fwd_pair(const ymi_tensor* x, const void* w_packed, int64_t cout, int64_t split, int64_t kh, int64_t kw, int64_t stride,
                                const float* gamma, const float* beta, float* running_mean, float* running_var, const float* gamma2,
                                const float* beta2, float* running_mean2, float* running_var2, float momentum, float eps, int32_t act,
                                const ymi_tensor* raw, const ymi_tensor* out, float* save_mean, float* save_invstd, void* workspace,
                                size_t workspace_bytes, void* stream);
int ymi_bn_act_bwd_pair(const ymi_tensor* dout, const ymi_tensor* raw, const float* gamma, const float* beta, const float* gamma2,
                        const float* beta2, int64_t split, const float* save_mean, const float* save_invstd, int32_t act,
                        const ymi_tensor* draw, float* dgamma, float* dbeta, void* workspace, size_t workspace_bytes, void* stream);
int ymi_conv2d_bwd_data(const ymi_tensor* dy, const void* w_dgrad_packed, int64_t cin, int64_t kh, int64_t kw, int64_t stride,
                        const ymi_tensor* dx, void* stream);
int ymi_conv2d_bwd_data_add(const ymi_tensor* dy, const void* w_dgrad_packed, int64_t cin, int64_t kh, int64_t kw, int64_t stride,
                            const ymi_tensor* add1, const ymi_tensor* add2, const ymi_tensor* dx, void* stream);
typedef struct ymi_dgrad_problem {
    const ymi_tensor* dy;
    const void* w_dgrad_packed;
    int64_t cin, k;
    const ymi_tensor* add1;
    const ymi_tensor* add2;
    const ymi_tensor* dx;
} ymi_dgrad_problem;
int ymi_conv2d_bwd_data_multi(const ymi_dgrad_problem* problems, int32_t n, void* stream);
int ymi_conv2d_bwd_weight(const ymi_tensor* x, const ymi_tensor* dy, int64_t cout_real, int64_t cin_real, int64_t kh, int64_t kw,
                          int64_t stride, float* dw_oihw, float* dbias, void* workspace, size_t workspace_bytes, void* stream);
size_t ymi_conv2d_bwd_weight_workspace(int64_t m_rows, int64_t cout, int64_t cin, int64_t kh, int64_t kw);
typedef struct ymi_wgrad_pending {
    const void* slab;
    float* dw;
    int64_t elems;
    int32_t splits, ng, cin, cout_real, cin_real, ntaps;
    int32_t lanes;
    int32_t first_block;
    int32_t blocks;
    int32_t slab_bf16;
    const float* bias_slab;
    float* dbias;
} ymi_wgrad_pending;
int ymi_conv2d_bwd_weight_deferred(const ymi_tensor* x, const ymi_tensor* dy, int64_t cout_real, int64_t cin_real, int64_t kh, int64_t kw,
                                   int64_t stride, float* dw_oihw, float* dbias, void* workspace, size_t workspace_bytes,
                                   ymi_wgrad_pending* pending, void* stream);
int ymi_wgrad_hold(int32_t mode);
int ymi_wgrad_reduce_batch(const ymi_wgrad_pending* host_records, int32_t n, ymi_wgrad_pending* device_table, void* stream);

int64_t ymi_first_conv_stat_blocks(int64_t n, int64_t h, int64_t w);
int ymi_first_conv_bn_act_fwd(const float* img_nchw, int64_t n, int64_t c, int64_t h, int64_t w, const float* weight_oihw, int64_t cout,
                              const float* gamma, const float* beta, float* running_mean, float* running_var, float momentum, float eps,
                              int32_t act, const ymi_tensor* x4, const ymi_tensor* out, float* save_mean, float* save_invstd,
                              void* workspace, size_t workspace_bytes, void* stream);
int64_t ymi_first_conv_bwd_workspace(int64_t n, int64_t h, int64_t w, int64_t cout);
int ymi_first_conv_bn_act_bwd(const ymi_tensor* x4, const float* weight_oihw, int64_t c, int64_t cout, const float* gamma, const float* beta,
                              const float* save_mean, const float* save_invstd, int32_t act, const ymi_tensor* dout, float* dgamma, float* dbeta,
                              float* dw_oihw, void* workspace, size_t workspace_bytes, ymi_wgrad_pending* pending, void* stream);

int ymi_dwconv2d_fwd(const ymi_tensor* x, const float* w, int64_t k, int64_t stride, const float* scale, const float* bias, int32_t act,
                     const ymi_tensor* residual, const ymi_tensor* y, float* stat_partials, int64_t* host_stat_blocks, void* stream);
int64_t ymi_dwconv2d_stat_blocks(int64_t n, int64_t ho, int64_t wo, int64_t c);
int ymi_dwconv2d_bn_act_fwd(const ymi_tensor* x, const float* w, int64_t k, int64_t stride, const float* gamma, const float* beta,
                            float* running_mean, float* running_var, float momentum, float eps, int32_t act, const ymi_tensor* residual,
                            const ymi_tensor* raw, const ymi_tensor* out, float* save_mean, float* save_invstd, void* workspace,
                            size_t workspace_bytes, void* stream);
int ymi_dwconv2d_bwd_data(const ymi_tensor* dy, const float* w, int64_t k, int64_t stride, const ymi_tensor* add, const ymi_tensor* dx, void* stream);
int ymi_dwconv2d_bwd_weight(const ymi_tensor* x, const ymi_tensor* dy, int64_t k, int64_t stride, float* dw, void* workspace,
                            size_t workspace_bytes, void* stream);
size_t ymi_dwconv2d_bwd_weight_workspace(int64_t n, int64_t ho, int64_t wo, int64_t c, int64_t k);


int ymi_sppf_pool3_fwd(const ymi_tensor* y0, int64_t k, const ymi_tensor* y1, const ymi_tensor* y2, const ymi_tensor* y3, void* stream);
int64_t ymi_sppf_pool3_bwd_workspace(int64_t n, int64_t h, int64_t w, int64_t c, int dtype);
int ymi_sppf_pool3_bwd(const ymi_tensor* y0, const ymi_tensor* y1, const ymi_tensor* y2, int64_t k, const ymi_tensor* dy0,
                       const ymi_tensor* dy1, const ymi_tensor* dy2, const ymi_tensor* dy3, const ymi_tensor* dx, void* workspace,
                       int64_t workspace_bytes, void* stream);


int ymi_cbam_fwd(const ymi_tensor* x, const float* w1, const float* w2, int64_t hidden, const float* wsa, int64_t ksa,
                 const ymi_tensor* out, float* ca, float* pooled , int32_t* pool_argmax , float* smap,
                 int32_t* smap_argmax , float* sa, void* stream);
int ymi_cbam_bwd(const ymi_tensor* x, const ymi_tensor* dout, const float* w1, const float* w2, int64_t hidden, const float* wsa,
                 int64_t ksa, const float* ca, const float* pooled, const int32_t* pool_argmax, const float* smap,
                 const int32_t* smap_argmax, const float* sa, const ymi_tensor* dx, float* dw1, float* dw2, float* dwsa,
                 void* workspace, size_t workspace_bytes, void* stream);
size_t ymi_cbam_bwd_workspace(int64_t n, int64_t h, int64_t w, int64_t c, int64_t hidden);


int ymi_window_partition_index(int64_t n, int64_t hp, int64_t wp, int64_t ws, int32_t* index, void* stream);
int ymi_window_partition(const ymi_tensor* x, int64_t ws, const ymi_tensor* tokens , void* stream);
int ymi_window_reverse(const ymi_tensor* tokens, int64_t ws, const ymi_tensor* x, void* stream);
int ymi_layernorm_fwd(const ymi_tensor* x, int64_t ws, const float* gamma, const float* beta, float eps, const ymi_tensor* out,
                      float* mean, float* rstd, void* stream);
int ymi_layernorm_bwd(const ymi_tensor* x, int64_t ws, const ymi_tensor* dout, const float* gamma, const float* mean,
                      const float* rstd, const ymi_tensor* dx, int32_t accumulate, float* dgamma, float* dbeta, void* workspace,
                      size_t workspace_bytes, void* stream);
int ymi_layernorm_bwd_add(const ymi_tensor* x, int64_t ws, const ymi_tensor* dout, const float* gamma, const float* mean, const float* rstd,
                          const ymi_tensor* add, const ymi_tensor* dx, float* dgamma, float* dbeta, void* workspace, size_t workspace_bytes,
                          void* stream);
int ymi_window_attention_fwd(const ymi_tensor* qkv, int64_t wlen, int64_t heads, const ymi_tensor* out, float* lse, void* stream);
int ymi_window_attention_bwd(const ymi_tensor* qkv, const ymi_tensor* out, const ymi_tensor* dout, const float* lse, int64_t wlen,
                             int64_t heads, const ymi_tensor* dqkv, void* stream);
int ymi_psa_attention_fwd(const ymi_tensor* qkv, int64_t tokens, int64_t heads, int64_t kd, const ymi_tensor* out, const ymi_tensor* v_out,
                          float* lse, void* stream);
int ymi_psa_attention_bwd(const ymi_tensor* qkv, const ymi_tensor* out, const ymi_tensor* dout, const float* lse, const ymi_tensor* dv_add,
                          int64_t tokens, int64_t heads, int64_t kd, const ymi_tensor* dqkv, void* stream);
int ymi_colsum(const ymi_tensor* x, float* out , void* workspace, size_t workspace_bytes, void* stream);
int ymi_gelu_bwd(const ymi_tensor* pre, const ymi_tensor* dy, const ymi_tensor* dx, void* stream);


int ymi_detect_targets(const float* batch_idx, const float* cls, const float* bboxes_xywhn, int64_t n, int64_t batch, int64_t max_boxes,
                       float img_w, float img_h, float* out, void* stream);
int ymi_detect_loss_sizes(int64_t batch, int64_t anchors, int64_t max_boxes, size_t* state_bytes, size_t* workspace_bytes);
int ymi_detect_loss_fwd(int32_t nl, const ymi_tensor* box_maps, const ymi_tensor* cls_maps, const float* strides, const float* targets,
                        int64_t max_boxes, int32_t topk, float alpha, float beta, const float* out_scale, float* loss_out, void* state,
                        size_t state_bytes, void* workspace, size_t workspace_bytes, void* stream);
int ymi_detect_loss_bwd(int32_t nl, const ymi_tensor* box_maps, const ymi_tensor* cls_maps, const float* strides, const void* state,
                        size_t state_bytes, const float* grad_loss, const float* grad_scale, const ymi_tensor* dbox_maps,
                        const ymi_tensor* dcls_maps, void* stream);

int ymi_detect_decode(int32_t nl, const ymi_tensor* box_maps, const ymi_tensor* cls_maps, const float* strides, float* y, void* stream);


int ymi_depth_to_space2(const ymi_tensor* src, const ymi_tensor* dst, void* stream);
int ymi_space_to_depth2(const ymi_tensor* src, const ymi_tensor* dst, void* stream);
int ymi_detect_loss_fwd_assign(int32_t nl, const ymi_tensor* box_maps, const ymi_tensor* cls_maps, const float* strides, const float* targets,
                               int64_t max_boxes, int32_t topk, float alpha, float beta, const float* out_scale, float* loss_out, void* state,
                               size_t state_bytes, void* workspace, size_t workspace_bytes, int32_t* gidx_out, void* stream);
int ymi_detect_decode_seg(int32_t nl, const ymi_tensor* box_maps, const ymi_tensor* cls_maps, const ymi_tensor* mc_maps, const float* strides,
                          float* y, void* stream);
int ymi_mask_loss_sizes(int64_t batch, int64_t anchors, int64_t max_boxes, int32_t topk, size_t* state_bytes);
int ymi_mask_loss_fwd(int32_t nl, const ymi_tensor* mc_maps, const ymi_tensor* proto, const void* masks, int32_t masks_f32, int64_t masks_h,
                      int64_t masks_w, const int32_t* gidx, const float* targets, int64_t max_boxes, int32_t topk, float img_w, float img_h,
                      const float* det_out6, const float* scale6, float* out8, void* state, size_t state_bytes, void* stream);
int ymi_mask_loss_bwd(int32_t nl, const ymi_tensor* mc_maps, const ymi_tensor* proto, const void* masks, int32_t masks_f32, int64_t masks_h,
                      int64_t masks_w, int64_t max_boxes, int32_t topk, const void* state, size_t state_bytes, const float* grad_out8,
                      const float* scale6, const ymi_tensor* dmc_maps, const ymi_tensor* dproto, void* stream);

int ymi_detect_nms_sizes(int64_t batch, int64_t anchors, int64_t nc, int64_t max_nms, int64_t max_det, size_t* workspace_bytes);
int ymi_detect_nms(const float* y, int64_t batch, int64_t nc, int64_t anchors, float conf_thres, float iou_thres, int32_t multi_label,
                   int32_t agnostic, const int32_t* host_classes, int32_t n_classes, int64_t max_det, int64_t max_nms, float max_wh, float* det,
                   int32_t* count, void* workspace, size_t workspace_bytes, void* stream);
int ymi_detect_nms_seg(const float* y, int64_t batch, int64_t nc, int64_t nm, int64_t anchors, float conf_thres, float iou_thres, int32_t multi_label,
                       int32_t agnostic, const int32_t* host_classes, int32_t n_classes, int64_t max_det, int64_t max_nms, float max_wh, float* det,
                       int32_t* count, float* coef, void* workspace, size_t workspace_bytes, void* stream);

#define YMI_MASK_NM 32
#define YMI_MASK_MAX_BINS 256
int ymi_process_mask(const ymi_tensor* proto, const float* box, const float* coef, const int32_t* img, int64_t n, int64_t ih, int64_t iw,
                     int32_t upsample, uint8_t* mask, int32_t* area, void* stream);
int ymi_mask_overlap(const float* det, const float* coef, const int32_t* count, int64_t batch, int64_t max_det, const ymi_tensor* proto, int64_t ih,
                     int64_t iw, const void* masks, int32_t masks_f32, int64_t masks_h, int64_t masks_w, int64_t n_bins, int32_t* inter,
                     int32_t* area_pred, int32_t* area_gt, void* stream);

int ymi_scale_image(const void* src, int32_t src_uint8, int64_t planes, int64_t h, int64_t w, float* dst, int64_t hp, int64_t wp, int64_t hs,
                    int64_t ws, float pad_value, int32_t normalize, int32_t flip_lr, int32_t flip_ud, void* stream);
int ymi_tta_merge(int32_t n, const float* const* src, const int64_t* anchors, const int64_t* lo, const int64_t* hi, const float* scale,
                  const int32_t* flip, const int64_t* img_h, const int64_t* img_w, int64_t batch, int64_t rows, float* out, void* stream);

#define YMI_LETTERBOX_MAX 32
typedef struct ymi_letterbox_image {
    const uint8_t* src;
    int32_t h, w, hs, ws, top, left;
} ymi_letterbox_image;
int ymi_letterbox_batch(const ymi_letterbox_image* images, int64_t n, float* dst, int64_t H, int64_t W, int32_t pad_value, int32_t normalize,
                        int32_t bgr, void* stream);
int ymi_scale_boxes(const float* det, int64_t det_ld, const int32_t* count, const float* params, int64_t batch, int64_t max_det, int64_t cols,
                    int32_t padding, int32_t xywh, float* out, int64_t out_ld, void* stream);

#define YMI_AUGMENT_MAX 32
#define YMI_AUGMENT_MAX_SRC 4
typedef struct ymi_augment_source {
    const uint8_t* src;
    int32_t h, w;
    int32_t x1a, y1a, x2a, y2a, x1b, y1b;
} ymi_augment_source;
typedef struct ymi_augment_image {
    ymi_augment_source s[YMI_AUGMENT_MAX_SRC];
    double A[6];
    const uint8_t* lut;
    int32_t n_src, canvas_h, canvas_w, flip_ud, flip_lr, _pad;
} ymi_augment_image;
int ymi_augment_batch(const ymi_augment_image* table, const ymi_augment_image* table_d, int64_t n, float* dst, int64_t size, int32_t border,
                      int32_t normalize, int32_t bgr, void* stream);
typedef struct ymi_augment_label_image {
    float src_w[YMI_AUGMENT_MAX_SRC], src_h[YMI_AUGMENT_MAX_SRC], ratio_w[YMI_AUGMENT_MAX_SRC], ratio_h[YMI_AUGMENT_MAX_SRC];
    float padw[YMI_AUGMENT_MAX_SRC], padh[YMI_AUGMENT_MAX_SRC];
    float M[6];
    float scale, size_w, size_h, canvas;
    int32_t flip_ud, flip_lr, row_start, row_end;
} ymi_augment_label_image;
int ymi_augment_boxes(const float* rows, int64_t n, const ymi_augment_label_image* images, int64_t batch, float area_thr, float* batch_idx,
                      float* cls, float* bboxes, int32_t* keep, int32_t* count, int32_t* total, void* stream);

#define YMI_VALMATCH_CHUNK 1024
#define YMI_VALMATCH_MAX_LEVELS 16
int ymi_val_match(const float* det, const int32_t* count, int64_t batch, int64_t max_det, const int32_t* lab_img, const float* lab_cls,
                  const float* lab_box, int64_t n_labels, float img_w, float img_h, const float* native, const float* levels, int32_t n_levels,
                  int32_t single_cls, uint8_t* tp, int32_t* cm, int64_t nc, float cm_conf, float cm_iou, void* stream);
int ymi_val_match_masks(const float* det, const int32_t* count, int64_t batch, int64_t max_det, const int32_t* lab_img, const float* lab_cls,
                        int64_t n_labels, const int32_t* inter, const int32_t* area_pred, const int32_t* area_gt, int64_t n_bins, const float* levels,
                        int32_t n_levels, int32_t single_cls, uint8_t* tp_m, void* stream);

#define YMI_OPT_MAX_GRADS 448
typedef struct ymi_opt_entry {
    float* param;
    float* momentum;
    float* ema;
    int64_t numel;
    int32_t group;
    int32_t _pad;
    float* second;
    float* acc;
} ymi_opt_entry;
int64_t ymi_opt_chunk_elems(void);
int ymi_opt_grad_norm(const ymi_opt_entry* table, const int32_t* chunk_map, int32_t first_tensor, int32_t n_tensors, int64_t n_chunks,
                      const float* const* host_grads, const float* hyper, float* partials, int64_t partials_offset, int64_t partials_total,
                      void* state, int32_t finalize, void* stream);
int ymi_opt_update(const ymi_opt_entry* table, const int32_t* chunk_map, int32_t first_tensor, int32_t n_tensors, int64_t n_chunks,
                   const float* const* host_grads, const float* hyper, const void* state, int32_t rule, void* stream);
int ymi_opt_grad_accumulate(const ymi_opt_entry* table, const int32_t* chunk_map, int32_t first_tensor, int32_t n_tensors, int64_t n_chunks,
                            const float* const* host_grads, void* stream);

int ymi_swin_mlp_fwd(const ymi_tensor* u, const void* w1_packed, const float* b1, int64_t hidden, const void* w2_packed, const float* b2,
                     const ymi_tensor* residual, const ymi_tensor* pre, const ymi_tensor* post, const ymi_tensor* out, void* stream);
int ymi_swin_mlp_bwd_data(const ymi_tensor* dout, const void* w2_dgrad_packed, const ymi_tensor* pre, const ymi_tensor* dpre,
                          const void* w1_dgrad_packed, const ymi_tensor* add1, const ymi_tensor* add2, const ymi_tensor* du, void* stream);

int ymi_swin_ln_mlp_supported(int64_t c, int64_t hidden, int32_t dtype);
int64_t ymi_swin_ln_mlp_pack_elems(int64_t c, int64_t hidden);
int64_t ymi_swin_ln_mlp_pre_elems(int64_t tokens, int64_t hidden);
int ymi_swin_ln_mlp_pack(const float* w1, const float* w2, int64_t c, int64_t hidden, void* packed, void* stream);
int ymi_swin_ln_mlp_fwd(const ymi_tensor* x, const float* gamma, const float* beta, float eps, const void* packed, const float* b1, const float* b2,
                        int64_t hidden, const ymi_tensor* u, float* mean, float* rstd, void* pre, const ymi_tensor* out, void* stream);
int ymi_swin_ln_mlp_bwd_data(const ymi_tensor* dout, const void* packed, const void* pre, int64_t hidden, const ymi_tensor* post, const ymi_tensor* dpre,
                             const ymi_tensor* du, void* stream);

#ifdef __cplusplus
}
#endif
#endif
```

Before: 2776 images/sec.

## Fuse BN-act backward apply, 1x1 dgrad and wgrad into one kernel

```diff
diff --git a/improving_yolov8_cbam_swinblock_amd/_lib.py b/improving_yolov8_cbam_swinblock_amd/_lib.py
--- a/improving_yolov8_cbam_swinblock_amd/_lib.py
+++ b/improving_yolov8_cbam_swinblock_amd/_lib.py
@@ -101,6 +101,9 @@
     "ymi_conv2d_bwd_weight_workspace": (_sz, [_c_i64, _c_i64, _c_i64, _c_i64, _c_i64]),
     "ymi_conv2d_bwd_weight_deferred": (_c_i32, [_TP, _TP, _c_i64, _c_i64, _c_i64, _c_i64, _c_i64, _vp, _vp, _vp, _sz, _vp, _vp]),
     "ymi_wgrad_hold": (_c_i32, [_c_i32]),
+    "ymi_conv1x1_bn_act_bwd_ok": (_c_i32, [_TP, _TP, _TP, _TP, _TP, _TP]),
+    "ymi_conv1x1_bn_act_bwd_workspace": (_sz, [_c_i64, _c_i64, _c_i64]),
+    "ymi_conv1x1_bn_act_bwd": (_c_i32, [_TP, _TP, _vp, _vp, _vp, _vp, _c_i32, _TP, _vp, _TP, _TP, _TP, _vp, _vp, _vp, _vp, _sz, _vp, _vp]),
     "ymi_wgrad_reduce_batch": (_c_i32, [_vp, _c_i32, _vp, _vp]),
     "ymi_sppf_pool3_fwd": (_c_i32, [_TP, _c_i64, _TP, _TP, _TP, _vp]),
     "ymi_sppf_pool3_bwd_workspace": (_c_i64, [_c_i64, _c_i64, _c_i64, _c_i64, _c_i32]),
diff --git a/improving_yolov8_cbam_swinblock_amd/csrc/common.h b/improving_yolov8_cbam_swinblock_amd/csrc/common.h
--- a/improving_yolov8_cbam_swinblock_amd/csrc/common.h
+++ b/improving_yolov8_cbam_swinblock_amd/csrc/common.h
@@ -330,6 +330,10 @@
     float* coef;
     GammaBeta2 g2;
 };
+template <int ACT> __device__ __forceinline__ float bn_bwd_apply_one(float d, float x, float a0, float a1, float c0, float c1, float c2) {
+    const float dz = d * act_grad<ACT>(x * a0 + a1);
+    return dz * c0 - (x * c1 + c2);
+}
 struct BnFinal {
     const float* part;
     int blocks, C;
@@ -445,6 +449,9 @@
 int ymi_bn_bwd_final(const float* part, int blocks, int C, const float* gamma, const float* beta, const float* mean, const float* inv, float inv_count,
                      float* dgamma, float* dbeta, float* coef, hipStream_t stream);
 
+int ymi_bn_act_bwd_coef(const ymi_tensor* dout, const ymi_tensor* raw, const float* gamma, const float* save_mean, const float* save_invstd, const float* beta,
+                        GammaBeta2 g2, int32_t act, float* dgamma, float* dbeta, void* workspace, size_t workspace_bytes, hipStream_t stream, const float** coef);
+
 ymi_wgrad_pending ymi_wgrad_record(const void* slab, float* dw, int64_t elems, int splits, int ng, int cin, int cout_real, int cin_real, int ntaps,
                                    bool slab_bf16, const float* bias_slab, float* dbias);
 
diff --git a/improving_yolov8_cbam_swinblock_amd/csrc/reduce_bwd.hip b/improving_yolov8_cbam_swinblock_amd/csrc/reduce_bwd.hip
--- a/improving_yolov8_cbam_swinblock_amd/csrc/reduce_bwd.hip
+++ b/improving_yolov8_cbam_swinblock_amd/csrc/reduce_bwd.hip
@@ -265,8 +265,7 @@
             float o[G];
 #pragma unroll
             for (int r = 0; r < G; ++r) {
-                const float dz = d[r] * act_grad<ACT>(x[r] * a0[r] + a1[r]);
-                o[r] = dz * c0[r] - (x[r] * c1[r] + c2[r]);
+                o[r] = bn_bwd_apply_one<ACT>(d[r], x[r], a0[r], a1[r], c0[r], c1[r], c2[r]);
             }
             Pack<T, G>::store(op + p * draw.ld + g * G, o);
         };
@@ -285,8 +284,7 @@
 #pragma unroll
             for (int r = 0; r < G; ++r) {
                 const int c = g * G + r;
-                const float dz = d[r] * act_grad<ACT>(x[r] * coef[c] + coef[C + c]);
-                o[r] = dz * coef[2 * C + c] - (x[r] * coef[3 * C + c] + coef[4 * C + c]);
+                o[r] = bn_bwd_apply_one<ACT>(d[r], x[r], coef[c], coef[C + c], coef[2 * C + c], coef[3 * C + c], coef[4 * C + c]);
             }
             Pack<T, G>::store(op + p * draw.ld + g * G, o);
         }
@@ -327,14 +325,11 @@
     YMI_CHECK_ARG(dout && split > 0 && split < dout->c && split % 4 == 0 && gamma2 && beta2, "bn_act_bwd_pair: split");
     return bn_act_bwd_impl(dout, raw, gamma, save_mean, save_invstd, beta, GammaBeta2{gamma2, beta2, (int)split}, act, draw, dgamma, dbeta, workspace, workspace_bytes, stream);
 }
-static int bn_act_bwd_impl(const ymi_tensor* dout, const ymi_tensor* raw, const float* gamma, const float* save_mean,
-                           const float* save_invstd, const float* beta, GammaBeta2 g2, int32_t act, const ymi_tensor* draw, float* dgamma,
-                           float* dbeta, void* workspace, size_t workspace_bytes, void* stream) {
-    YMI_CHECK_ARG(ymi_tensor_ok(dout) && ymi_tensor_ok(raw) && ymi_tensor_ok(draw) && ymi_same_shape(dout, raw) && ymi_same_shape(dout, draw),
-                  "bn_act_bwd: shapes");
-    YMI_CHECK_ARG(dout->dtype == raw->dtype && raw->dtype == draw->dtype, "bn_act_bwd: dtypes");
+int ymi_bn_act_bwd_coef(const ymi_tensor* dout, const ymi_tensor* raw, const float* gamma, const float* save_mean, const float* save_invstd, const float* beta,
+                        GammaBeta2 g2, int32_t act, float* dgamma, float* dbeta, void* workspace, size_t workspace_bytes, hipStream_t s, const float** coef_out) {
+    YMI_CHECK_ARG(ymi_tensor_ok(dout) && ymi_tensor_ok(raw) && ymi_same_shape(dout, raw), "bn_act_bwd: shapes");
+    YMI_CHECK_ARG(dout->dtype == raw->dtype, "bn_act_bwd: dtypes");
     YMI_CHECK_ARG(save_mean && save_invstd && dgamma && dbeta && workspace, "bn_act_bwd: null argument");
-    YMI_CHECK_ARG(draw->ld % 4 == 0, "bn_act_bwd: draw ld");
     const int64_t P = ymi_pixels(dout);
     const int C = (int)dout->c;
     const int rblocks = reduce_blocks(P, C);
@@ -343,25 +338,35 @@
         ymi_set_error("bn_act_bwd: workspace %zu < %zu", workspace_bytes, need);
         return YMI_EWORKSPACE;
     }
-    hipStream_t s = (hipStream_t)stream;
     int blocks = 0;
     float* coef = (float*)workspace + (size_t)rblocks * 2 * C;
     double* xrows = reinterpret_cast<double*>(coef + 6 * (size_t)C);
     const BnCoefArgs bn{gamma, beta, save_mean, save_invstd, 1.0f / (float)P, coef, g2};
+    *coef_out = coef;
     if (bn_tail_on() && C <= 1024) {
         unsigned* tickets = ymi_ticket_slot();
         YMI_CHECK_ARG(tickets, "bn_act_bwd: ticket counters");
-        int rc = launch_chan_reduce<1>(dout, raw, gamma, beta, save_mean, save_invstd, act, (float*)workspace, &blocks, s, "bn_act_bwd(reduce)", g2,
-                                       ReduceTail{tickets, rblocks % 32 == 0 ? 32 : 8, xrows, dbeta, dgamma, bn});
-        if (rc) return rc;
-        return launch_bn_apply(dout, raw, draw, act, coef, s);
+        return launch_chan_reduce<1>(dout, raw, gamma, beta, save_mean, save_invstd, act, (float*)workspace, &blocks, s, "bn_act_bwd(reduce)", g2,
+                                     ReduceTail{tickets, rblocks % 32 == 0 ? 32 : 8, xrows, dbeta, dgamma, bn});
     }
     int rc = launch_chan_reduce<1>(dout, raw, gamma, beta, save_mean, save_invstd, act, (float*)workspace, &blocks, s, "bn_act_bwd(reduce)", g2);
     if (rc) return rc;
     const BnFinal f{(const float*)workspace, blocks, C, dbeta, dgamma, bn};
     if (C <= 1024 && ymi_wgrad_issue_held(&f, s)) YMI_CHECK_LAUNCH("bn_act_bwd(final, riding)");
     else if ((rc = launch_final(f, s, "bn_act_bwd(final)")) != YMI_OK) return rc;
-    return launch_bn_apply(dout, raw, draw, act, coef, s);
+    return YMI_OK;
+}
+static int bn_act_bwd_impl(const ymi_tensor* dout, const ymi_tensor* raw, const float* gamma, const float* save_mean,
+                           const float* save_invstd, const float* beta, GammaBeta2 g2, int32_t act, const ymi_tensor* draw, float* dgamma,
+                           float* dbeta, void* workspace, size_t workspace_bytes, void* stream) {
+    YMI_CHECK_ARG(ymi_tensor_ok(dout) && ymi_tensor_ok(raw) && ymi_tensor_ok(draw) && ymi_same_shape(dout, raw) && ymi_same_shape(dout, draw),
+                  "bn_act_bwd: shapes");
+    YMI_CHECK_ARG(dout->dtype == raw->dtype && raw->dtype == draw->dtype, "bn_act_bwd: dtypes");
+    YMI_CHECK_ARG(draw->ld % 4 == 0, "bn_act_bwd: draw ld");
+    const float* coef = nullptr;
+    const int rc = ymi_bn_act_bwd_coef(dout, raw, gamma, save_mean, save_invstd, beta, g2, act, dgamma, dbeta, workspace, workspace_bytes, (hipStream_t)stream, &coef);
+    if (rc) return rc;
+    return launch_bn_apply(dout, raw, draw, act, coef, (hipStream_t)stream);
 }
 
 template <typename T>
diff --git a/improving_yolov8_cbam_swinblock_amd/csrc/wgrad.hip b/improving_yolov8_cbam_swinblock_amd/csrc/wgrad.hip
--- a/improving_yolov8_cbam_swinblock_amd/csrc/wgrad.hip
+++ b/improving_yolov8_cbam_swinblock_amd/csrc/wgrad.hip
@@ -330,6 +330,21 @@
     }
 }
 
+__device__ __forceinline__ bool wg_tile_of_block(const WgradArgs& a, int first, int& bx, int& by, int& bz) {
+    if (a.xcd_map) {
+        const int id = (int)blockIdx.x - first, xcd = id & 7, seq = id >> 3, nxy = a.nx * a.ny;
+        const int zi = seq / nxy, t = seq - zi * nxy;
+        const int spx = (a.splits + 7) >> 3;
+        bz = xcd * spx + zi;
+        if (zi >= spx || bz >= a.splits) return false;
+        by = t / a.nx;
+        bx = t - by * a.nx;
+    } else {
+        bx = blockIdx.x; by = blockIdx.y; bz = blockIdx.z;
+    }
+    return true;
+}
+
 template <typename T, int BM, bool BIAS, bool PATCH>
 __global__ __launch_bounds__(256, (BM == 128 ? 3 : WG_WAVES)) void wgrad_kernel(WgradArgs a, BnRider rider) {
     using G = WgTile<T, BM>;
@@ -348,17 +363,7 @@
         if ((int)blockIdx.x * 32 < rider.f.C) bn_final_block<NT, false>(rider.f, (int)blockIdx.x, reinterpret_cast<double*>(smem));
         return;
     }
-    if (a.xcd_map) {
-        const int id = (int)blockIdx.x - rider.nwg, xcd = id & 7, seq = id >> 3, nxy = a.nx * a.ny;
-        const int zi = seq / nxy, t = seq - zi * nxy;
-        const int spx = (a.splits + 7) >> 3;
-        bz = xcd * spx + zi;
-        if (zi >= spx || bz >= a.splits) return;
-        by = t / a.nx;
-        bx = t - by * a.nx;
-    } else {
-        bx = blockIdx.x; by = blockIdx.y; bz = blockIdx.z;
-    }
+    if (!wg_tile_of_block(a, rider.nwg, bx, by, bz)) return;
     const int j0 = bx * WG_BN, co0 = by * BM;
     const int m_begin = bz * a.pix_per_split;
     const int m_end = min(a.Mpix, m_begin + a.pix_per_split);
@@ -414,6 +419,201 @@
     }
 }
 
+struct Conv1x1BwdArgs {
+    WgradArgs w;
+    const void* dout;
+    const void* raw;
+    int64_t ld_dout, ld_raw;
+    const float* coef;
+    const void* wd;
+    void* dx;
+    const void* add1;
+    const void* add2;
+    int64_t ld_dx, ld_a1, ld_a2;
+};
+constexpr int C1_DROW = WG_BN * 4 + 16;
+template <int BM> constexpr size_t conv1x1_bwd_lds_bytes() { return wgrad_lds_bytes<bf16_t, BM>() + (size_t)WG_BK * C1_DROW; }
+
+__device__ __forceinline__ u32x4 c1_lds_read16(const char* p) {
+    u32x4 v;
+    asm volatile("ds_read_b128 %0, %1" : "=v"(v) : "v"((uint32_t)(uintptr_t)(lptr_t)p));
+    return v;
+}
+__device__ __forceinline__ void c1_lds_write16_mfma(char* p, f32x4 v) {
+    asm volatile("s_nop 15\n\ts_nop 3\n\tds_write_b128 %0, %1" ::"v"((uint32_t)(uintptr_t)(lptr_t)p), "v"(v) : "memory");
+}
+
+template <int BM, int ACT>
+__global__ __launch_bounds__(256, (BM == 128 ? 2 : 3)) void conv1x1_bwd_kernel(Conv1x1BwdArgs p) {
+    using T = bf16_t;
+    using G = WgTile<T, BM>;
+    constexpr int NT = G::NT, TR = G::TR, TC = G::TC, WM = G::WM, STAGE = G::STAGE, NS = WG_NS, NY = G::NY, NX = G::NX;
+    constexpr int RING = NS * STAGE;
+    constexpr int KK = BM / 32;
+    static_assert(G::YT == NT && WG_BK == 32 && NS == 2, "every thread owns NY chunks of the dY image; two stages");
+    static_assert(RING >= (NT / 64) * SlabStage<bf16_t, TR>::BYTES && RING >= (NT / 64) * SlabStage<float, TR>::BYTES, "the staged slab stores use the ring");
+    extern __shared__ __attribute__((aligned(16))) char smem[];
+    char* dxs = smem + RING;
+
+    const WgradArgs& a = p.w;
+    const int tid = threadIdx.x, lane = tid & 63;
+    const int wave = __builtin_amdgcn_readfirstlane(tid >> 6);
+    const int wr = wave / G::WCOLS, wc = wave % G::WCOLS;
+    int bx, by, bz;
+    if (!wg_tile_of_block(a, 0, bx, by, bz)) return;
+    const int j0 = bx * WG_BN;
+    const int m_begin = bz * a.pix_per_split;
+    const int m_end = min(a.Mpix, m_begin + a.pix_per_split);
+    const G ld(a, tid, j0, 0);
+
+    float k0[8], k1[8], k2[8], k3[8], k4[8];
+#pragma unroll
+    for (int r = 0; r < 8; ++r) {
+        const int c = ld.ych + r;
+        k0[r] = p.coef[c];
+        k1[r] = p.coef[BM + c];
+        k2[r] = p.coef[2 * BM + c];
+        k3[r] = p.coef[3 * BM + c];
+        k4[r] = p.coef[4 * BM + c];
+    }
+    bf16x8 wf[2][KK];
+#pragma unroll
+    for (int ct = 0; ct < 2; ++ct) {
+        const int ci = j0 + (2 * wave + ct) * 16 + (lane & 15);
+#pragma unroll
+        for (int kk = 0; kk < KK; ++kk) {
+            u32x4 v = {0u, 0u, 0u, 0u};
+            if (ci < a.Cin) v = *reinterpret_cast<const u32x4*>(reinterpret_cast<const T*>(p.wd) + (int64_t)ci * BM + kk * 32 + (lane >> 4) * 8);
+            wf[ct][kk] = __builtin_bit_cast(bf16x8, v);
+        }
+    }
+    const bool patch = a.pw_shift >= 0;
+    const int pw = patch ? 1 << a.pw_shift : WG_BK, ph = WG_BK / pw;
+    auto row_off = [&](int row) { return patch ? (row >> a.pw_shift) * a.W + (row & (pw - 1)) : row; };
+    struct { int m, wo, ho; } org, nxt;
+    org.m = m_begin; org.wo = org.ho = 0;
+    if (patch) {
+        const int pidx = m_begin / WG_BK, npw = a.W >> a.pw_shift, nph = a.H / ph;
+        const int t = pidx / npw, wp = pidx - t * npw;
+        const int n = t / nph, hp = t - n * nph;
+        org.wo = wp * pw; org.ho = hp * ph;
+        org.m = (n * a.H + org.ho) * a.W + org.wo;
+    }
+    auto advance = [&](auto o) {
+        if (!patch) { o.m += WG_BK; return o; }
+        o.wo += pw; o.m += pw;
+        if (o.wo == a.W) {
+            o.wo = 0; o.ho += ph; o.m += (ph - 1) * a.W;
+            if (o.ho == a.H) o.ho = 0;
+        }
+        return o;
+    };
+    uint32_t xv[NX];
+#pragma unroll
+    for (int i = 0; i < NX; ++i) xv[i] = ld.x_cok ? (uint32_t)((row_off(ld.x_row(i)) * (int)a.ldx + ld.ci) * 2) : 0x80000000u;
+    int yo[NY];
+#pragma unroll
+    for (int i = 0; i < NY; ++i) yo[i] = row_off(ld.y_row(i));
+    const int dch = tid & 15, drow = tid >> 4;
+    const bool d_cok = j0 + dch * 8 < a.Cin;
+    const int dro[2] = {row_off(drow), row_off(drow + 16)};
+
+    f32x4 acc[TR][TC];
+#pragma unroll
+    for (int r = 0; r < TR; ++r)
+#pragma unroll
+        for (int c = 0; c < TC; ++c) acc[r][c] = f32x4{0.f, 0.f, 0.f, 0.f};
+    f32x4 accb[1] = {f32x4{0.f, 0.f, 0.f, 0.f}};
+
+    const int nk = (m_end - m_begin + WG_BK - 1) / WG_BK;
+    u32x4 rd[NY], rr[NY];
+    auto load_rows = [&](int mo) {
+#pragma unroll
+        for (int i = 0; i < NY; ++i) {
+            const int m = mo + yo[i];
+            rd[i] = rr[i] = u32x4{0u, 0u, 0u, 0u};
+            if (patch || m < m_end) {
+                rd[i] = *reinterpret_cast<const u32x4*>(reinterpret_cast<const T*>(p.dout) + (int64_t)m * p.ld_dout + ld.ych);
+                rr[i] = *reinterpret_cast<const u32x4*>(reinterpret_cast<const T*>(p.raw) + (int64_t)m * p.ld_raw + ld.ych);
+            }
+        }
+    };
+    auto issue_x = [&](int s, int mo) {
+        char* Xs = smem + s * STAGE + G::YBYTES;
+        const uint32_t soff = __builtin_amdgcn_readfirstlane((uint32_t)mo * (uint32_t)a.ldx * 2u);
+#pragma unroll
+        for (int i = 0; i < NX; ++i) wg_buffer_to_lds(a.x, a.x_bytes, G::x_slot(Xs, i, wave), xv[i], soff);
+    };
+    load_rows(org.m);
+    issue_x(0, org.m);
+    for (int kt = 0; kt < nk; ++kt, org = nxt) {
+        const int mk = org.m;
+        nxt = advance(org);
+        char* Ys = smem + (kt & 1) * STAGE;
+#pragma unroll
+        for (int i = 0; i < NY; ++i) {
+            const bf16x8 d = __builtin_bit_cast(bf16x8, rd[i]), x = __builtin_bit_cast(bf16x8, rr[i]);
+            const bool ok = patch || mk + yo[i] < m_end;
+            bf16x8 o;
+#pragma unroll
+            for (int r = 0; r < 8; ++r) {
+                const float v = bn_bwd_apply_one<ACT>((float)d[r], (float)x[r], k0[r], k1[r], k2[r], k3[r], k4[r]);
+                o[r] = (bf16_t)(ok ? v : 0.0f);
+            }
+            *reinterpret_cast<bf16x8*>(Ys + (i * NT + tid) * 16) = o;
+        }
+        asm volatile("s_waitcnt vmcnt(0) lgkmcnt(0)\n\ts_barrier" ::: "memory");
+        if (kt + 1 < nk) {
+            issue_x((kt + 1) & 1, nxt.m);
+            load_rows(nxt.m);
+        }
+        WFrag<T>::template step<BM, TR, TC, false>(Ys, Ys + G::YBYTES, wr * WM, wc * 64, lane, acc, false, accb);
+#pragma unroll
+        for (int pt = 0; pt < 2; ++pt) {
+            u32x4 bq[KK];
+            const int px = pt * 16 + (lane & 15);
+            const int sw = tr_swz<tr_swz_mode(BM * 2)>(px) << 1;
+#pragma unroll
+            for (int kk = 0; kk < KK; ++kk) bq[kk] = c1_lds_read16(Ys + px * (BM * 2) + (((kk * 4 + (lane >> 4)) ^ sw) << 4));
+            asm volatile("s_waitcnt lgkmcnt(0)" ::: "memory");
+#pragma unroll
+            for (int kk = 0; kk < KK; ++kk) asm volatile("" : "+v"(bq[kk]));
+#pragma unroll
+            for (int ct = 0; ct < 2; ++ct) {
+                f32x4 d = {0.f, 0.f, 0.f, 0.f};
+#pragma unroll
+                for (int kk = 0; kk < KK; ++kk) d = __builtin_amdgcn_mfma_f32_16x16x32_bf16(wf[ct][kk], __builtin_bit_cast(bf16x8, bq[kk]), d, 0, 0, 0);
+                c1_lds_write16_mfma(dxs + px * C1_DROW + ((2 * wave + ct) * 16 + 4 * (lane >> 4)) * 4, d);
+            }
+        }
+        asm volatile("s_waitcnt lgkmcnt(0)\n\ts_barrier" ::: "memory");
+#pragma unroll
+        for (int h = 0; h < 2; ++h) {
+            const int row = drow + 16 * h, m = mk + dro[h];
+            const bool ok = (patch || m < m_end) && d_cok;
+            u32x4 ra[2] = {u32x4{0u, 0u, 0u, 0u}, u32x4{0u, 0u, 0u, 0u}};
+            if (ok && p.add1) ra[0] = *reinterpret_cast<const u32x4*>(reinterpret_cast<const T*>(p.add1) + (int64_t)m * p.ld_a1 + j0 + dch * 8);
+            if (ok && p.add2) ra[1] = *reinterpret_cast<const u32x4*>(reinterpret_cast<const T*>(p.add2) + (int64_t)m * p.ld_a2 + j0 + dch * 8);
+            u32x4 lo = c1_lds_read16(dxs + row * C1_DROW + dch * 32), hi = c1_lds_read16(dxs + row * C1_DROW + dch * 32 + 16);
+            asm volatile("s_waitcnt lgkmcnt(0)" ::: "memory");
+            asm volatile("" : "+v"(lo), "+v"(hi));
+            const f32x4 flo = __builtin_bit_cast(f32x4, lo), fhi = __builtin_bit_cast(f32x4, hi);
+            float v[8] = {flo[0], flo[1], flo[2], flo[3], fhi[0], fhi[1], fhi[2], fhi[3]};
+#pragma unroll
+            for (int q = 0; q < 2; ++q) {
+                const bf16x8 t = __builtin_bit_cast(bf16x8, ra[q]);
+#pragma unroll
+                for (int r = 0; r < 8; ++r) v[r] += (float)t[r];
+            }
+            if (ok) Pack<T, 8>::store(reinterpret_cast<T*>(p.dx) + (int64_t)m * p.ld_dx + j0 + dch * 8, v);
+        }
+    }
+
+    const int64_t slab_off = (int64_t)bz * a.CoutP * a.NG;
+    const int row0 = wr * WM, col0 = j0 + wc * 64;
+    if (a.slab_bf16) wg_store_slab_staged<bf16_t>(smem, wave, lane, acc, reinterpret_cast<bf16_t*>(a.slab) + slab_off, row0, col0, a.CoutP, a.NG);
+    else wg_store_slab_staged<float>(smem, wave, lane, acc, reinterpret_cast<float*>(a.slab) + slab_off, row0, col0, a.CoutP, a.NG);
+}
 
 template <typename S> __device__ __forceinline__ float wg_split_sum(const S* __restrict__ p, int64_t e, int64_t stride, int splits) {
     float s0 = 0.f, s1 = 0.f, s2 = 0.f, s3 = 0.f;
@@ -560,6 +760,18 @@
 
 static int wgrad_impl(const ymi_tensor* x, const ymi_tensor* dy, int64_t cout_real, int64_t cin_real, int64_t kh, int64_t kw, int64_t stride,
                       float* dw_oihw, float* dbias, void* workspace, size_t workspace_bytes, ymi_wgrad_pending* pending, void* stream);
+static int wgrad_slab_sum(const WgradArgs& a, int64_t cout_real, int64_t cin_real, int64_t ntaps, float* dw_oihw, float* dbias, ymi_wgrad_pending* pending,
+                          hipStream_t s);
+static int wgrad_patch_shift(const ymi_tensor* x, const ymi_tensor* dy) {
+    const int64_t xb = ymi_pixels(x) * x->ld * ymi_esize(x->dtype), yb = ymi_pixels(dy) * dy->ld * ymi_esize(dy->dtype);
+    const int64_t margin = (x->w + 2) * x->ld * (int64_t)ymi_esize(x->dtype);
+    if (!(x->dtype == YMI_BF16 && ymi_opt(OPT_WGRAD_PATCH) && xb + margin < (1ll << 31) && yb < (1ll << 31) && ymi_pixels(dy) % WG_BK == 0)) return -1;
+    for (int sh = 5; sh >= 0; --sh) {
+        const int pw = 1 << sh, ph = WG_BK >> sh;
+        if (dy->w % pw == 0 && dy->h % ph == 0) return sh;
+    }
+    return -1;
+}
 
 struct WgradLaunch {
     WgradArgs a;
@@ -722,21 +934,10 @@
     wg_find_divisor(a.Wo, &a.wo_mul, &a.wo_shr);
     wg_find_divisor(a.Ho, &a.ho_mul, &a.ho_shr);
     a.nx = (int)((ng + bn - 1) / bn); a.ny = (int)((dy->c + bm - 1) / bm); a.splits = p.splits;
-    a.pw_shift = -1;
-    {
-        const int64_t xb = ymi_pixels(x) * x->ld * ymi_esize(x->dtype), yb = ymi_pixels(dy) * dy->ld * ymi_esize(dy->dtype);
-        const int64_t margin = (x->w + 2) * x->ld * (int64_t)ymi_esize(x->dtype);
-        if (bf16 && ymi_opt(OPT_WGRAD_PATCH) && xb + margin < (1ll << 31) && yb < (1ll << 31) && mpix % WG_BK == 0) {
-            for (int sh = 5; sh >= 0; --sh) {
-                const int pw = 1 << sh, ph = WG_BK >> sh;
-                if (dy->w % pw == 0 && dy->h % ph == 0) {
-                    a.pw_shift = sh;
-                    break;
-                }
-            }
-            a.x_bytes = (uint32_t)xb;
-            a.y_bytes = (uint32_t)yb;
-        }
+    a.pw_shift = wgrad_patch_shift(x, dy);
+    if (a.pw_shift >= 0) {
+        a.x_bytes = (uint32_t)(ymi_pixels(x) * x->ld * ymi_esize(x->dtype));
+        a.y_bytes = (uint32_t)(ymi_pixels(dy) * dy->ld * ymi_esize(dy->dtype));
     }
     a.xcd_map = p.splits >= 8 ? 1 : 0;
     dim3 grid((unsigned)a.nx, (unsigned)a.ny, (unsigned)p.splits);
@@ -757,20 +958,97 @@
         }
     }
     YMI_CHECK_LAUNCH("wgrad");
+    return wgrad_slab_sum(a, cout_real, cin_real, kh * kw, dw_oihw, dbias, pending, s);
+}
+
+static int wgrad_slab_sum(const WgradArgs& a, int64_t cout_real, int64_t cin_real, int64_t ntaps, float* dw_oihw, float* dbias, ymi_wgrad_pending* pending,
+                          hipStream_t s) {
     if (pending) {
-        *pending = ymi_wgrad_record(a.slab, dw_oihw, (int64_t)a.CoutP * a.NG, p.splits, a.NG, a.Cin, (int)cout_real, (int)cin_real, (int)(kh * kw), slab_bf16,
+        *pending = ymi_wgrad_record(a.slab, dw_oihw, (int64_t)a.CoutP * a.NG, a.splits, a.NG, a.Cin, (int)cout_real, (int)cin_real, (int)ntaps, a.slab_bf16 != 0,
                                     a.bias_slab, dbias);
     } else {
-        const int64_t total = cout_real * kh * kw * cin_real;
+        const int64_t total = cout_real * ntaps * cin_real;
         int64_t gb = (total + 255) / 256;
         if (gb > 2048) gb = 2048;
-        hipLaunchKernelGGL(slab_bf16 ? wgrad_reduce_kernel<true> : wgrad_reduce_kernel<false>, dim3((unsigned)gb), dim3(256), 0, s, (const void*)a.slab, p.splits,
-                           a.CoutP, a.NG, a.Cin, (int)cout_real, (int)cin_real, (int)(kh * kw), dw_oihw);
+        hipLaunchKernelGGL(a.slab_bf16 ? wgrad_reduce_kernel<true> : wgrad_reduce_kernel<false>, dim3((unsigned)gb), dim3(256), 0, s, (const void*)a.slab, a.splits,
+                           a.CoutP, a.NG, a.Cin, (int)cout_real, (int)cin_real, (int)ntaps, dw_oihw);
     }
     YMI_CHECK_LAUNCH("wgrad_reduce");
     if (dbias && !pending) {
-        hipLaunchKernelGGL(wgrad_bias_reduce_kernel, dim3((unsigned)((dy->c + 255) / 256)), dim3(256), 0, s, (const float*)a.bias_slab, p.splits, (int)dy->c, dbias);
+        hipLaunchKernelGGL(wgrad_bias_reduce_kernel, dim3((unsigned)((a.CoutP + 255) / 256)), dim3(256), 0, s, (const float*)a.bias_slab, a.splits, a.CoutP, dbias);
         YMI_CHECK_LAUNCH("wgrad_bias_reduce");
     }
     return YMI_OK;
 }
+
+static bool conv1x1_bwd_scope(const ymi_tensor* dout, const ymi_tensor* raw, const ymi_tensor* x, const ymi_tensor* add1, const ymi_tensor* add2,
+                              const ymi_tensor* dx) {
+    if (!(ymi_tensor_ok(dout) && ymi_tensor_ok(raw) && ymi_tensor_ok(x) && ymi_tensor_ok(dx))) return false;
+    if (add2 && !add1) return false;
+    const ymi_tensor* all[6] = {dout, raw, x, dx, add1, add2};
+    for (const ymi_tensor* t : all)
+        if (t && !(ymi_tensor_ok(t) && t->dtype == YMI_BF16 && t->c % 8 == 0 && t->ld % 8 == 0 && (uintptr_t)t->data % 16 == 0 && ymi_pixels(t) * t->ld < (1ll << 30))) return false;
+    if (!(ymi_same_shape(dout, raw) && (dout->c == 64 || dout->c == 128))) return false;
+    if (!(x->n == dout->n && x->h == dout->h && x->w == dout->w && x->c <= 512 && ymi_same_shape(x, dx))) return false;
+    return (!add1 || ymi_same_shape(add1, dx)) && (!add2 || ymi_same_shape(add2, dx));
+}
+extern "C" int ymi_conv1x1_bn_act_bwd_ok(const ymi_tensor* dout, const ymi_tensor* raw, const ymi_tensor* x, const ymi_tensor* add1, const ymi_tensor* add2,
+                                         const ymi_tensor* dx) {
+    return conv1x1_bwd_scope(dout, raw, x, add1, add2, dx) ? 1 : 0;
+}
+extern "C" size_t ymi_conv1x1_bn_act_bwd_workspace(int64_t m_rows, int64_t cout, int64_t cin) {
+    const int rblocks = 2048;
+    const size_t bn = (((size_t)rblocks * 2 * cout + 6 * (size_t)cout) * sizeof(float) + 64 * (size_t)cout * sizeof(double) + 255) / 256 * 256;
+    return bn + ymi_conv2d_bwd_weight_workspace(m_rows, cout, cin, 1, 1);
+}
+extern "C" int ymi_conv1x1_bn_act_bwd(const ymi_tensor* dout, const ymi_tensor* raw, const float* gamma, const float* save_mean, const float* save_invstd,
+                                      const float* beta, int32_t act, const ymi_tensor* x, const void* w_dgrad_packed, const ymi_tensor* add1,
+                                      const ymi_tensor* add2, const ymi_tensor* dx, float* dgamma, float* dbeta, float* dw_oihw, void* workspace,
+                                      size_t workspace_bytes, ymi_wgrad_pending* pending, void* stream) {
+    YMI_CHECK_ARG(conv1x1_bwd_scope(dout, raw, x, add1, add2, dx), "conv1x1_bn_act_bwd: outside the fused kernel's scope (ymi_conv1x1_bn_act_bwd_ok)");
+    YMI_CHECK_ARG(w_dgrad_packed && (uintptr_t)w_dgrad_packed % 16 == 0 && dw_oihw && workspace, "conv1x1_bn_act_bwd: bad argument");
+    const int64_t mpix = ymi_pixels(dout);
+    const int bm = (int)dout->c, cin = (int)x->c;
+    const size_t need = ymi_conv1x1_bn_act_bwd_workspace(mpix, bm, cin);
+    if (workspace_bytes < need) {
+        ymi_set_error("conv1x1_bn_act_bwd: workspace %zu < %zu bytes", workspace_bytes, need);
+        return YMI_EWORKSPACE;
+    }
+    hipStream_t s = (hipStream_t)stream;
+    const size_t bn_bytes = need - ymi_conv2d_bwd_weight_workspace(mpix, bm, cin, 1, 1);
+    const float* coef = nullptr;
+    int rc = ymi_bn_act_bwd_coef(dout, raw, gamma, save_mean, save_invstd, beta, GammaBeta2{nullptr, nullptr, 0}, act, dgamma, dbeta, workspace, bn_bytes, s, &coef);
+    if (rc) return rc;
+    WgradPlan p = wgrad_plan(mpix, bm, cin, bm, 2);
+    const bool slab_bf16 = p.splits >= 16;
+    if (!slab_bf16) p = wgrad_plan(mpix, bm, cin, bm, 4);
+    Conv1x1BwdArgs k{};
+    WgradArgs& a = k.w;
+    a.x = x->data; a.slab = reinterpret_cast<char*>(workspace) + bn_bytes; a.slab_bf16 = slab_bf16 ? 1 : 0;
+    a.ldx = x->ld; a.Mpix = (int)mpix; a.H = a.Ho = (int)x->h; a.W = a.Wo = (int)x->w;
+    a.stride = 1; a.pad = 0; a.KW = 1;
+    a.CoutP = bm; a.Cin = cin; a.NG = cin; a.pix_per_split = p.pix_per_split;
+    a.nx = (cin + WG_BN - 1) / WG_BN; a.ny = 1; a.splits = p.splits;
+    a.x_bytes = (uint32_t)(((mpix - 1) * x->ld + x->c) * 2);
+    a.xcd_map = p.splits >= 8 ? 1 : 0;
+    a.pw_shift = wgrad_patch_shift(x, dout);
+    k.dout = dout->data; k.raw = raw->data; k.ld_dout = dout->ld; k.ld_raw = raw->ld;
+    k.coef = coef; k.wd = w_dgrad_packed;
+    k.dx = dx->data; k.ld_dx = dx->ld;
+    k.add1 = add1 ? add1->data : nullptr; k.ld_a1 = add1 ? add1->ld : 0;
+    k.add2 = add2 ? add2->data : nullptr; k.ld_a2 = add2 ? add2->ld : 0;
+    dim3 grid((unsigned)a.nx, 1, (unsigned)p.splits);
+    if (a.xcd_map) grid = dim3((unsigned)(8 * ((p.splits + 7) / 8) * a.nx), 1, 1);
+    int prof = -1;
+    if (ymi_prof_enabled())
+        prof = ymi_prof_start(s, 1, 4.0 * (double)mpix * bm * cin, ((double)mpix * (2.0 * bm + (2.0 + (add1 ? 1 : 0) + (add2 ? 1 : 0)) * cin)) * 2.0 + (double)bm * cin * 4.0,
+                              2500.0);
+    dispatch_dtype_act(YMI_BF16, act, [&](auto, auto ac) {
+        constexpr int ACT = decltype(ac)::value;
+        if (bm == 128) hipLaunchKernelGGL((conv1x1_bwd_kernel<128, ACT>), grid, dim3(256), conv1x1_bwd_lds_bytes<128>(), s, k);
+        else hipLaunchKernelGGL((conv1x1_bwd_kernel<64, ACT>), grid, dim3(256), conv1x1_bwd_lds_bytes<64>(), s, k);
+    });
+    ymi_prof_stop(s, prof);
+    YMI_CHECK_LAUNCH("conv1x1_bn_act_bwd");
+    return wgrad_slab_sum(a, bm, cin, 1, dw_oihw, nullptr, pending, s);
+}
diff --git a/improving_yolov8_cbam_swinblock_amd/ops/base.py b/improving_yolov8_cbam_swinblock_amd/ops/base.py
--- a/improving_yolov8_cbam_swinblock_amd/ops/base.py
+++ b/improving_yolov8_cbam_swinblock_amd/ops/base.py
@@ -20,6 +20,7 @@
     "first_conv": True,
     "stat_atomics": True,
     "wgrad_rider": True,
+    "fused_bwd_1x1": True,
 }
 
 
diff --git a/improving_yolov8_cbam_swinblock_amd/ops/conv.py b/improving_yolov8_cbam_swinblock_amd/ops/conv.py
--- a/improving_yolov8_cbam_swinblock_amd/ops/conv.py
+++ b/improving_yolov8_cbam_swinblock_amd/ops/conv.py
@@ -159,6 +159,31 @@
         check(L().ymi_bn_act_bwd_pair(_byref(as_ymi(dout)), _byref(as_ymi(raw)), ptr(gamma), ptr(beta), ptr(gamma_b), ptr(beta_b), oa, ptr(stats[0]), ptr(stats[1]),
                                       act, _byref(as_ymi(draw)), ptr(dgamma), ptr(dbeta), ptr(ws), ws.numel(), stream_ptr()), "bn_act_bwd_pair")
     return draw, dgamma, dbeta
+
+
+def _conv1x1_bwd_fused(dout, raw, stats, act, gamma, beta, x, weight, job):
+    lib = L()
+    o, cin = weight.shape[0], weight.shape[1]
+    dev = x.device
+    a1 = _byref(as_ymi(job.fused[0])) if len(job.fused) > 0 else None
+    a2 = _byref(as_ymi(job.fused[1])) if len(job.fused) > 1 else None
+    tdo, traw, tx, tdx = as_ymi(dout), as_ymi(raw), as_ymi(x), as_ymi(job.dxv)
+    if not lib.ymi_conv1x1_bn_act_bwd_ok(_byref(tdo), _byref(traw), _byref(tx), a1, a2, _byref(tdx)):
+        return None
+    dgamma = torch.empty(o, dtype=torch.float32, device=dev)
+    dbeta = torch.empty(o, dtype=torch.float32, device=dev)
+    params = (weight,)
+    defer = RUN.defer and _in_backward() and _adoptable(params)
+    dw = _new_dw(o, cin, 1, dev, params, None)
+    need = int(lib.ymi_conv1x1_bn_act_bwd_workspace(tdo.n * tdo.h * tdo.w, o, cin))
+    ws = torch.empty(need, dtype=torch.uint8, device=dev) if defer else workspace(need, dev, "conv1x1bwd")
+    rec = _lib.WgradPending() if defer else None
+    if defer:
+        _defer_wgrad(rec, (ws, x, dout, raw), weight)
+    check(lib.ymi_conv1x1_bn_act_bwd(_byref(tdo), _byref(traw), ptr(gamma), ptr(stats[0]), ptr(stats[1]), ptr(beta), act, _byref(tx), ptr(job.wd), a1, a2,
+                                     _byref(tdx), ptr(dgamma), ptr(dbeta), ptr(dw), ptr(ws), ws.numel(), _byref(rec) if defer else None, stream_ptr()),
+          "conv1x1_bn_act_bwd")
+    return dgamma, dbeta, dw
 
 
 class _ConvBnAct(torch.autograd.Function):
@@ -208,14 +233,29 @@
         dtype = x.dtype
         o, _, k, _ = weight.shape
         dout = grad_nhwc(dout, dtype)
+        join, res_join = ctx.joins
+        want_dx, want_dw = ctx.needs_input_grad[0], ctx.needs_input_grad[1]
+        hand_res = has_res and ctx.needs_input_grad[10]
+        if (HOOKS["fused_bwd_1x1"] and want_dx and want_dw and k == 1 and stride == 1 and dtype == torch.bfloat16 and o in (64, 128)
+                and x.shape[1] == cin and cin <= 128 and not _deferred_twice((weight,))):
+            dres = _join_plain(res_join, dout) if hand_res else None
+            job, deposit = _dgrad_joined_prepare(join, dout, weight, k, stride, x.shape, dtype)
+            done = _conv1x1_bwd_fused(dout, raw, stats, act, gamma, beta, x, weight, job)
+            if done is None:
+                draw, dgamma, dbeta = _bn_act_bwd(dout, raw, stats, act, gamma, beta)
+                dx = _dgrad_joined_finish(join, _dgrad_launch(job._replace(dy=draw, ty=as_ymi(draw))), deposit)
+                dw, _ = _wgrad_maybe_async(x, draw, o, cin, k, stride, False, (weight,))
+            else:
+                dgamma, dbeta, dw = done
+                dx = _dgrad_joined_finish(join, _dgrad_finish(job), deposit)
+            return dx, dw, dgamma, dbeta, None, None, None, None, None, None, dres, None, None, None
         draw, dgamma, dbeta = _bn_act_bwd(dout, raw, stats, act, gamma, beta)
-        join, res_join = ctx.joins
-        dres = _join_plain(res_join, dout) if (has_res and ctx.needs_input_grad[10]) else None
+        dres = _join_plain(res_join, dout) if hand_res else None
         dx = None
-        if ctx.needs_input_grad[0]:
+        if want_dx:
             dx = _dgrad_joined(join, draw, weight, k, stride, x.shape, dtype)
         dw = None
-        if ctx.needs_input_grad[1]:
+        if want_dw:
             dw, _ = _wgrad_maybe_async(x, draw, o, cin, k, stride, False, (weight,))
         return dx, dw, dgamma, dbeta, None, None, None, None, None, None, dres, None, None, None
 
diff --git a/include/ymi.h b/include/ymi.h
--- a/include/ymi.h
+++ b/include/ymi.h
@@ -145,6 +145,14 @@
 int ymi_wgrad_hold(int32_t mode);
 int ymi_wgrad_reduce_batch(const ymi_wgrad_pending* host_records, int32_t n, ymi_wgrad_pending* device_table, void* stream);
 
+int ymi_conv1x1_bn_act_bwd_ok(const ymi_tensor* dout, const ymi_tensor* raw, const ymi_tensor* x, const ymi_tensor* add1, const ymi_tensor* add2,
+                              const ymi_tensor* dx);
+size_t ymi_conv1x1_bn_act_bwd_workspace(int64_t m_rows, int64_t cout, int64_t cin);
+int ymi_conv1x1_bn_act_bwd(const ymi_tensor* dout, const ymi_tensor* raw, const float* gamma, const float* save_mean, const float* save_invstd,
+                           const float* beta, int32_t act, const ymi_tensor* x, const void* w_dgrad_packed, const ymi_tensor* add1,
+                           const ymi_tensor* add2, const ymi_tensor* dx, float* dgamma, float* dbeta, float* dw_oihw, void* workspace,
+                           size_t workspace_bytes, ymi_wgrad_pending* pending, void* stream);
+
 int64_t ymi_first_conv_stat_blocks(int64_t n, int64_t h, int64_t w);
 int ymi_first_conv_bn_act_fwd(const float* img_nchw, int64_t n, int64_t c, int64_t h, int64_t w, const float* weight_oihw, int64_t cout,
                               const float* gamma, const float* beta, float* running_mean, float* running_var, float momentum, float eps,
```

Measured after the change: 2817 images/sec (median of 6 runs). 1.01x the previous value.
